# PlanNoa/video_super_resolution

Hardware: AMD Instinct MI355X
Metric: HR frames/sec, 1080p->4K x4 VSR (LR 540x960 -> 2160x3840), VSR.forward end-to-end (higher is better)
Workload: dtype f16

## Files before the change

### __graft_entry__.py

```python
import os

os.environ.setdefault("MIOPEN_FIND_MODE", "2")
os.environ.setdefault("MIOPEN_DEBUG_ENABLE_AI_IMMED_MODE_FALLBACK", "0")
os.environ.setdefault("MIOPEN_LOG_LEVEL", "2")
import subprocess
import sys

ROOT = os.path.dirname(os.path.abspath(__file__))
if ROOT not in sys.path:
    sys.path.insert(0, ROOT)


def build() -> None:
    from video_super_resolution_amd import _lib
    _lib.build(verbose=True)
    subprocess.check_call(["make", "-s", "-C", os.path.join(ROOT, "oracle"), "_build/liboracle_native.so"])
    import video_super_resolution_amd
    missing = [s for s in _lib.declared_symbols() if not hasattr(_lib.load(), s)]
    if missing:
        raise RuntimeError(f"libvsr_hip.so lacks {missing}")
    xmissing = [s for s in _lib.declared_symbols() + _lib.declared_symbols(xcheck=True) if not hasattr(_lib.load_xcheck(), s)]
    if xmissing:
        raise RuntimeError(f"libvsr_hip_xcheck.so lacks {xmissing}")
    s3missing = [s for s in _lib.declared_symbols(s3=True) if not hasattr(_lib.load_s3(), s)]
    if s3missing:
        raise RuntimeError(f"libvsr_hip_s3.so lacks {s3missing}")
    s3tmissing = [s for s in _lib.declared_symbols(s3t=True) if not hasattr(_lib.load_s3t(), s)]
    if s3tmissing:
        raise RuntimeError(f"libvsr_hip_s3t.so lacks {s3tmissing}")
    s3pmissing = [s for s in _lib.declared_symbols(s3p=True) if not hasattr(_lib.load_s3p(), s)]
    if s3pmissing:
        raise RuntimeError(f"libvsr_hip_s3p.so lacks {s3pmissing}")
    s3fmissing = [s for s in _lib.declared_symbols(s3f=True) if not hasattr(_lib.load_s3f(), s)]
    if s3fmissing:
        raise RuntimeError(f"libvsr_hip_s3f.so lacks {s3fmissing}")
    yuvmissing = [s for s in _lib.declared_symbols(yuv=True) if not hasattr(_lib.load_yuv(), s)]
    if yuvmissing:
        raise RuntimeError(f"libvsr_hip_yuv.so lacks {yuvmissing}")
    metricmissing = [s for s in _lib.declared_symbols(metric=True) if not hasattr(_lib.load_metric(), s)]
    if metricmissing:
        raise RuntimeError(f"libvsr_hip_metric.so lacks {metricmissing}")
    optmissing = [s for s in _lib.declared_symbols(opt=True) if not hasattr(_lib.load_opt(), s)]
    if optmissing:
        raise RuntimeError(f"libvsr_hip_opt.so lacks {optmissing}")
    lossmissing = [s for s in _lib.declared_symbols(loss=True) if not hasattr(_lib.load_loss(), s)]
    if lossmissing:
        raise RuntimeError(f"libvsr_hip_loss.so lacks {lossmissing}")
    resizemissing = [s for s in _lib.declared_symbols(resize=True) if not hasattr(_lib.load_resize(), s)]
    if resizemissing:
        raise RuntimeError(f"libvsr_hip_resize.so lacks {resizemissing}")
    warpmissing = [s for s in _lib.declared_symbols(warp=True) if not hasattr(_lib.load_warp(), s)]
    if warpmissing:
        raise RuntimeError(f"libvsr_hip_warp.so lacks {warpmissing}")
    scenemissing = [s for s in _lib.declared_symbols(scene=True) if not hasattr(_lib.load_scene(), s)]
    if scenemissing:
        raise RuntimeError(f"libvsr_hip_scene.so lacks {scenemissing}")
    hgimissing = [s for s in _lib.declared_symbols(hgi=True) if not hasattr(_lib.load_hgi(), s)]
    if hgimissing:
        raise RuntimeError(f"libvsr_hip_hgi.so lacks {hgimissing}")
    msssimmissing = [s for s in _lib.declared_symbols(msssim=True) if not hasattr(_lib.load_msssim(), s)]
    if msssimmissing:
        raise RuntimeError(f"libvsr_hip_msssim.so lacks {msssimmissing}")


def smoke() -> None:
    import numpy as np
    import torch
    from oracle import native, vsr_oracle
    from video_super_resolution_amd import SRProjectionModule, ops
    from video_super_resolution_amd.weights import fill_module_

    assert torch.cuda.is_available(), "smoke() needs cuda:0"
    torch.cuda.set_device(0)
    rs = np.random.RandomState(0)
    img = rs.randn(1, 3, 32, 48).astype(np.float32)
    flow = (rs.randn(1, 2, 32, 48) * 4).astype(np.float32)
    got = ops.resample2d(torch.from_numpy(img).cuda(), torch.from_numpy(flow).cuda()).cpu().numpy()
    assert np.array_equal(got, native.resample2d(img, flow)), "flow warp differs from the oracle"

    sr = fill_module_(SRProjectionModule().eval(), seed=0, prefix="model.")
    x = torch.from_numpy(rs.randint(0, 256, (8, 3, 10, 12)).astype(np.float32))
    with torch.no_grad():
        ref = vsr_oracle.sr_forward({k: v for k, v in sr.state_dict().items()}, x).numpy()
    sr = sr.cuda()
    errs = {}
    for precision, bar in (("fp32", 1e-3), ("fp16", 5e-3)):
        sr.precision = precision
        out = sr(x.cuda()).cpu().numpy()
        errs[precision] = np.abs(out - ref).max() / np.abs(ref).max()
        assert errs[precision] < bar, f"SR forward ({precision}) differs from the oracle: {errs[precision]}"
    print(f"smoke ok: warp bit-exact, SR forward rel err fp32 {errs['fp32']:.2e}, fp16/MFMA {errs['fp16']:.2e}")


if __name__ == "__main__":
    build()
    if len(sys.argv) > 1 and sys.argv[1] == "smoke":
        smoke()
```

### video_super_resolution_amd/_lib.py

```python
from __future__ import annotations

import ctypes
import os
import re
import subprocess

import torch

_PKG = os.path.dirname(os.path.abspath(__file__))
_ROOT = os.path.dirname(_PKG)
LIB_PATH = os.path.join(_PKG, "libvsr_hip.so")
XLIB_PATH = os.path.join(_PKG, "libvsr_hip_xcheck.so")
HEADER_PATH = os.path.join(_ROOT, "include", "vsr_hip.h")
XHEADER_PATH = os.path.join(_ROOT, "include", "vsr_hip_xcheck.h")
_lib = None
_xlib = None


def _side(name: str, prefix: str, abi: int, has_query: bool) -> tuple:
    return (os.path.join(_PKG, f"libvsr_hip_{name}.so"), os.path.join(_ROOT, "include", f"vsr_hip_{name}.h"), prefix, abi, has_query)


_SIDE = {"grad": _side("grad", "vsr_grad", 1, False), "s3": _side("s3", "vsr_s3", 1, True), "s3t": _side("s3t", "vsr_s3t", 1, True),
         "s3p": _side("s3p", "vsr_s3p", 1, True), "s3f": _side("s3f", "vsr_s3f", 1, True), "yuv": _side("yuv", "vsr_yuv", 1, False),
         "metric": _side("metric", "vsr_metric", 1, False), "opt": _side("opt", "vsr_opt", 1, False), "loss": _side("loss", "vsr_loss", 1, False),
         "resize": _side("resize", "vsr_resize", 1, False), "warp": _side("warp", "vsr_warp", 1, False),
         "scene": _side("scene", "vsr_scene", 1, False), "hgi": _side("hgi", "vsr_hgi", 1, False),
         "msssim": _side("msssim", "vsr_msssim", 1, False)}
(GLIB_PATH, GHEADER_PATH), (S3LIB_PATH, S3HEADER_PATH), (S3TLIB_PATH, S3THEADER_PATH), (S3PLIB_PATH, S3PHEADER_PATH), \
    (S3FLIB_PATH, S3FHEADER_PATH), (YUVLIB_PATH, YUVHEADER_PATH), (METRICLIB_PATH, METRICHEADER_PATH), (OPTLIB_PATH, OPTHEADER_PATH), \
    (LOSSLIB_PATH, LOSSHEADER_PATH), (RESIZELIB_PATH, RESIZEHEADER_PATH), (WARPLIB_PATH, WARPHEADER_PATH), (SCENELIB_PATH, SCENEHEADER_PATH), \
    (HGILIB_PATH, HGIHEADER_PATH), (MSSSIMLIB_PATH, MSSSIMHEADER_PATH) = (row[:2] for row in _SIDE.values())
_gradlib = _s3lib = _s3tlib = _s3plib = _s3flib = _yuvlib = _metriclib = _optlib = _losslib = _resizelib = _warplib = _scenelib = _hgilib = _msssimlib = None
_use_x = os.environ.get("VSR_USE_XCHECK", "0") == "1" or bool(os.environ.get("VSR_TUNING", "").strip())


class VsrHipError(RuntimeError):
    pass


def build(verbose: bool = False) -> str:
    cmd = ["make", "-j4", "-C", os.path.join(_PKG, "csrc")]
    if not verbose:
        cmd.insert(1, "-s")
    subprocess.check_call(cmd)
    return LIB_PATH


def declared_symbols(xcheck: bool = False, grad: bool = False, s3: bool = False, s3t: bool = False, s3p: bool = False, s3f: bool = False,
                     yuv: bool = False, metric: bool = False, opt: bool = False, loss: bool = False, resize: bool = False,
                     warp: bool = False, scene: bool = False, hgi: bool = False, msssim: bool = False) -> list:
    side = [name for name, on in (("grad", grad), ("s3", s3), ("s3t", s3t), ("s3p", s3p), ("s3f", s3f), ("yuv", yuv), ("metric", metric),
                                  ("opt", opt), ("loss", loss), ("resize", resize), ("warp", warp), ("scene", scene), ("hgi", hgi),
                                  ("msssim", msssim)) if on]
    with open(_SIDE[side[-1]][1] if side else XHEADER_PATH if xcheck else HEADER_PATH) as f:
        text = re.sub(r"/\*.*?\*/", "", f.read(), flags=re.S)
    return sorted(set(re.findall(r"\b(vsr_[a-z0-9_]+)\s*\(", text)))


def _dlopen(path: str) -> ctypes.CDLL:
    if not os.path.exists(path):
        raise VsrHipError(
            f"{path} is missing: build it with `python -c 'import __graft_entry__ as g; g.build()'` "
            "(there is no CPU fallback for the device path)")
    return ctypes.CDLL(path)


def _open(path: str) -> ctypes.CDLL:
    lib = _dlopen(path)
    lib.vsr_last_error.restype = ctypes.c_char_p
    lib.vsr_last_route.restype = ctypes.c_char_p
    for fn in ("vsr_sr_query", "vsr_train_corr_dw_ws_floats", "vsr_train_prelu_bwd_ws_floats"):
        getattr(lib, fn).restype = ctypes.c_size_t
    if lib.vsr_abi_version() != 3:
        raise VsrHipError(f"{os.path.basename(path)}: ABI version mismatch")
    return lib


def load_xcheck() -> ctypes.CDLL:
    global _xlib
    if _xlib is None:
        lib = _open(XLIB_PATH)
        for t in os.environ.get("VSR_TUNING", "").split(","):
            if t.strip():
                lib.vsr_conv2d_tuning(int(t))
        _xlib = lib
    return _xlib


def _load_side(name: str) -> ctypes.CDLL:
    cache = f"_{name}lib"
    if globals()[cache] is None:
        path, _, prefix, abi, has_query = _SIDE[name]
        lib = _dlopen(path)
        getattr(lib, prefix + "_last_error").restype = ctypes.c_char_p
        lib.vsr_last_error = getattr(lib, prefix + "_last_error")
        if has_query:
            getattr(lib, prefix + "_query").restype = ctypes.c_size_t
        if getattr(lib, prefix + "_abi_version")() != abi:
            raise VsrHipError(f"{os.path.basename(path)}: ABI version mismatch")
        globals()[cache] = lib
    return globals()[cache]


def load_grad() -> ctypes.CDLL:
    return _load_side("grad")


def load_s3() -> ctypes.CDLL:
    return _load_side("s3")


def load_s3t() -> ctypes.CDLL:
    return _load_side("s3t")


def load_s3p() -> ctypes.CDLL:
    return _load_side("s3p")


def load_s3f() -> ctypes.CDLL:
    return _load_side("s3f")


def load_yuv() -> ctypes.CDLL:
    return _load_side("yuv")


def load_metric() -> ctypes.CDLL:
    lib = _load_side("metric")
    lib.vsr_metric_ws_bytes.restype = ctypes.c_size_t
    return lib


class OptTensor(ctypes.Structure):
    _fields_ = [("p", ctypes.c_void_p), ("g", ctypes.c_void_p), ("m", ctypes.c_void_p), ("v", ctypes.c_void_p), ("n", ctypes.c_ulonglong)]


def load_opt() -> ctypes.CDLL:
    lib = _load_side("opt")
    lib.vsr_opt_plan_bytes.restype = lib.vsr_opt_norm_ws_bytes.restype = ctypes.c_size_t
    lib.vsr_opt_plan_bytes.argtypes = [ctypes.c_int, ctypes.POINTER(ctypes.c_ulonglong)]
    lib.vsr_opt_plan_fill.argtypes = [ctypes.c_void_p, ctypes.c_size_t, ctypes.c_int, ctypes.POINTER(OptTensor)]
    lib.vsr_opt_norm_ws_bytes.argtypes = [ctypes.c_void_p]
    lib.vsr_opt_adam_f32.argtypes = [ctypes.c_void_p] * 3 + [ctypes.c_float] * 7 + [ctypes.c_void_p]
    lib.vsr_opt_grad_norm.argtypes = [ctypes.c_void_p, ctypes.c_void_p, ctypes.c_double, ctypes.c_void_p, ctypes.c_void_p, ctypes.c_void_p]
    return lib


def load_loss() -> ctypes.CDLL:
    lib = _load_side("loss")
    lib.vsr_loss_ws_bytes.restype = ctypes.c_size_t
    lib.vsr_loss_ws_bytes.argtypes = [ctypes.c_int, ctypes.c_int]
    lib.vsr_loss_pixel_terms.argtypes = [ctypes.c_void_p] * 3 + [ctypes.c_int] * 2 + [ctypes.c_void_p] * 6
    return lib


def load_resize() -> ctypes.CDLL:
    lib = _load_side("resize")
    lib.vsr_resize_frames.argtypes = [ctypes.c_void_p] * 2 + [ctypes.c_int] * 5 + [ctypes.c_void_p, ctypes.c_void_p, ctypes.c_int] * 2 + \
        [ctypes.c_int, ctypes.c_void_p]
    return lib


def load_warp() -> ctypes.CDLL:
    lib = _load_side("warp")
    lib.vsr_warp_ws_bytes.restype = ctypes.c_size_t
    lib.vsr_warp_ws_bytes.argtypes = [ctypes.c_int] * 4
    lib.vsr_warp_error.argtypes = [ctypes.c_void_p] * 2 + [ctypes.c_int] * 7 + [ctypes.c_void_p] * 2 + [ctypes.c_int] + [ctypes.c_longlong] * 3 + \
        [ctypes.c_int] * 3 + [ctypes.c_void_p] * 5
    return lib


def load_scene() -> ctypes.CDLL:
    lib = _load_side("scene")
    lib.vsr_scene_ws_bytes.restype = ctypes.c_size_t
    lib.vsr_scene_ws_bytes.argtypes = [ctypes.c_int] * 3
    lib.vsr_scene_pair_sums.argtypes = [ctypes.c_void_p] * 2 + [ctypes.c_int] * 3 + [ctypes.c_void_p] * 4
    lib.vsr_scene_decide.argtypes = [ctypes.c_void_p, ctypes.c_int, ctypes.c_void_p, ctypes.c_double, ctypes.c_double, ctypes.c_void_p, ctypes.c_void_p]
    lib.vsr_scene_window.argtypes = [ctypes.c_void_p] * 4 + [ctypes.c_int] * 2 + [ctypes.c_void_p] * 4 + [ctypes.c_int] * 2 + [ctypes.c_void_p]
    return lib


def load_hgi() -> ctypes.CDLL:
    lib = _load_side("hgi")
    lib.vsr_hgi_workgroups.restype = ctypes.c_longlong
    lib.vsr_hgi_inception_f16.argtypes = [ctypes.c_void_p] + [ctypes.c_int] * 3 + [ctypes.c_void_p] * 2 + [ctypes.c_int] * 3 + \
        [ctypes.c_void_p, ctypes.c_void_p, ctypes.c_int] * 3 + [ctypes.c_int, ctypes.c_void_p] + [ctypes.c_int] * 4 + [ctypes.c_void_p]
    return lib


def load_msssim() -> ctypes.CDLL:
    lib = _load_side("msssim")
    lib.vsr_msssim_ws_bytes.restype = ctypes.c_size_t
    lib.vsr_msssim_ws_bytes.argtypes = [ctypes.c_int] * 5
    lib.vsr_msssim_frames.argtypes = [ctypes.c_void_p] * 2 + [ctypes.c_int] * 6 + [ctypes.c_void_p] * 5
    return lib


def load() -> ctypes.CDLL:
    global _lib
    if _use_x:
        return load_xcheck()
    if _lib is None:
        _lib = _open(LIB_PATH)
    return _lib


class xcheck:

    def __enter__(self):
        global _use_x
        self._old, _use_x = _use_x, True
        return load_xcheck()

    def __exit__(self, *exc):
        global _use_x
        _use_x = self._old
        return False


Q_UTD_BLOB_BYTES, Q_UTD_STRIP_WIDTH, Q_UTD_S2_BLOB_BYTES, Q_UTD_S2_STRIP_WIDTH, Q_TAIL_S2_BLOB_BYTES = range(5)
Q_S3_BLOB_BYTES, Q_S3_STRIP_WIDTH = range(2)
Q_S3T_BLOB_BYTES, Q_S3T_BLOB_FOLD_BYTES, Q_S3T_STRIP_WIDTH = range(3)
Q_S3P_BLOB_BYTES, Q_S3P_STRIP_WIDTH = range(2)
Q_S3F_BLOB_BYTES, Q_S3F_STRIP_WIDTH = range(2)


def check(rc: int, what: str = "", lib=None) -> None:
    if rc != 0:
        libs = [lib] if lib is not None else [l for l in (load(), _lib, _xlib) if l is not None]
        msgs = []
        for l in libs:
            m = l.vsr_last_error().decode("utf-8", "replace")
            if m and m not in msgs:
                msgs.append(m)
        raise VsrHipError(f"{what or 'vsr'} failed ({rc}): {' | '.join(msgs)}")


def dptr(t: torch.Tensor, dtype=torch.float32) -> ctypes.c_void_p:
    if not t.is_cuda:
        raise VsrHipError("device path called with a CPU tensor (no CPU fallback exists)")
    if t.dtype != dtype:
        raise VsrHipError(f"expected {dtype}, got {t.dtype}")
    if not t.is_contiguous():
        raise VsrHipError("tensor must be contiguous")
    return ctypes.c_void_p(t.data_ptr())


def optr(t, dtype=torch.float32):
    return ctypes.c_void_p(0) if t is None else dptr(t, dtype)


_raw_stream = getattr(torch._C, "_cuda_getCurrentRawStream", None)


def raw_stream(index=None) -> int:
    if _raw_stream is not None:
        return _raw_stream(torch._C._cuda_getDevice() if index is None else index)
    return torch.cuda.current_stream(index).cuda_stream


def stream() -> ctypes.c_void_p:
    return ctypes.c_void_p(raw_stream())


def _first_cuda_tensor(objs):
    for o in objs:
        if isinstance(o, torch.Tensor):
            if o.is_cuda:
                return o
        elif isinstance(o, (list, tuple)):
            t = _first_cuda_tensor(o)
            if t is not None:
                return t
    return None


def on_device(fn):
    import functools

    @functools.wraps(fn)
    def wrapped(*args, **kwargs):
        t = _first_cuda_tensor(args)
        if t is None:
            t = _first_cuda_tensor(tuple(kwargs.values()))
        if t is None or t.device.index == torch.cuda.current_device():
            return fn(*args, **kwargs)
        with torch.cuda.device(t.device):
            return fn(*args, **kwargs)
    return wrapped


def cf(v: float) -> ctypes.c_float:
    return ctypes.c_float(float(v))


class _ChainStage(ctypes.Structure):
    _fields_ = [("inp", ctypes.c_void_p * 2), ("w", ctypes.c_void_p * 2), ("ldw", ctypes.c_int * 2), ("w_prev", ctypes.c_void_p),
                ("ldw_prev", ctypes.c_int), ("bias", ctypes.c_void_p), ("cmap", ctypes.c_void_p), ("slope", ctypes.c_float),
                ("out", ctypes.c_void_p)]


class Chain1x1(ctypes.Structure):
    _fields_ = [("nstages", ctypes.c_int), ("stage", _ChainStage * 3)]


_ROUTE_BATCH = os.environ.get("VSR_ROUTE_BATCH", "1") != "0"


class route_batch:

    def __init__(self, num: int, den: int):
        self.num, self.den = int(num), int(den)
        self.on = self.den > 0 and self.num > 0 and self.num != self.den and _ROUTE_BATCH

    def __enter__(self):
        if self.on:
            check(load().vsr_conv2d_route_batch(self.num, self.den), "conv2d_route_batch")
        return self

    def __exit__(self, *exc):
        if self.on:
            load().vsr_conv2d_route_batch(0, 0)
        return False


class serial_streams:
    on = False

    def __init__(self, enable: bool = True):
        self.enable = bool(enable)

    def __enter__(self):
        self._old, serial_streams.on = serial_streams.on, serial_streams.on or self.enable
        return self

    def __exit__(self, *exc):
        serial_streams.on = self._old
        return False


class EventTimer:

    def __init__(self):
        self.enabled = False
        self.only = None
        self._pairs = {}

    def reset(self):
        self._pairs = {}

    def start(self, name: str):
        if not self.enabled or (self.only is not None and name not in self.only):
            return None
        a = torch.cuda.Event(enable_timing=True)
        b = torch.cuda.Event(enable_timing=True)
        a.record()
        self._pairs.setdefault(name, []).append((a, b))
        return b

    @staticmethod
    def stop(tok):
        if tok is not None:
            tok.record()

    def summary(self):
        return {k: (len(v), sum(a.elapsed_time(b) for a, b in v) / len(v)) for k, v in self._pairs.items()}


TIMER = EventTimer()


class RouteLog:

    def __init__(self):
        self.enabled = False
        self.calls = []

    def note(self, label: str):
        if self.enabled:
            self.calls.append((label, load().vsr_last_route().decode()))

    def note_as(self, label: str, route: str):
        if self.enabled:
            self.calls.append((label, route))

    def last(self) -> str:
        return load().vsr_last_route().decode()

    def histogram(self):
        h = {}
        for _, r in self.calls:
            h[r] = h.get(r, 0) + 1
        return h


ROUTES = RouteLog()
```

### video_super_resolution_amd/csrc/sr_f16.hip

```cpp
#include "sr_f16_common.h"

namespace {

#if VSR_X
__device__ unsigned long long* g_stamp_ptr = nullptr;

template <int MODE, bool ALLMAX, int DIAG = 0>
__global__ void __launch_bounds__(512, 2)
k_utd(const _Float16* __restrict__ in, const unsigned char* __restrict__ blob, _Float16* __restrict__ out, int h, int w,
      int rows_per_seg) {
    extern __shared__ __attribute__((aligned(16))) unsigned char smem[];
    unsigned char* const ring = smem;
    unsigned char* const part = smem + RING_BYTES;
    unsigned char* const lrr = smem + RING_BYTES + PART_BYTES;
    float* const bias_s = reinterpret_cast<float*>(smem + RING_BYTES + PART_BYTES + LR_BYTES);

    const int tid = threadIdx.x;
    const int lane = tid & 63;
    const int wv = __builtin_amdgcn_readfirstlane(tid >> 6);
    const int l15 = lane & 15, g = lane >> 4;
    const int x0 = blockIdx.x * TX;
    const int n = blockIdx.z;
    const int r0 = blockIdx.y * rows_per_seg;
    const int r1 = min(h, r0 + rows_per_seg);
    if (r0 >= r1) return;

    h8 Aup[2][4][2];
    h8 Adn[2][8];
#pragma unroll
    for (int c = 0; c < 2; ++c)
#pragma unroll
        for (int t = 0; t < 4; ++t)
#pragma unroll
            for (int mt = 0; mt < 2; ++mt)
                Aup[c][t][mt] = *reinterpret_cast<const h8*>(blob + BLOB_UP + ((((wv * 2 + c) * 4 + t) * 2 + mt) * 64 + lane) * 16);
    if (MODE == 0) {
#pragma unroll
        for (int hl = 0; hl < 2; ++hl)
#pragma unroll
            for (int kx = 0; kx < 8; ++kx)
                Adn[hl][kx] = *reinterpret_cast<const h8*>(blob + BLOB_DN + (((wv * 2 + hl) * 8 + kx) * 64 + lane) * 16);
        if (tid < 128) *reinterpret_cast<uint4*>(smem + RING_BYTES + PART_BYTES + LR_BYTES + 256 + tid * 16) =
            *reinterpret_cast<const uint4*>(blob + BLOB_DT + tid * 16);
    }
    const unsigned char* const adt_s = smem + RING_BYTES + PART_BYTES + LR_BYTES + 256 + lane * 16;
    const float* fpar = reinterpret_cast<const float*>(blob + BLOB_F32);
    if (tid < 64) bias_s[tid] = fpar[tid];
    auto bias_up = [&](int mt) __attribute__((always_inline)) { return *reinterpret_cast<const f4*>(bias_s + 16 * mt + 4 * g); };
    auto bias_dt = [&](int mt) __attribute__((always_inline)) { return *reinterpret_cast<const f4*>(bias_s + 32 + 16 * mt + 4 * g); };
    const float a_up = fpar[96], a_dt = fpar[97], a_dn = fpar[98];
    const h2 a_up2 = {(_Float16)a_up, (_Float16)a_up}, a_dt2 = {(_Float16)a_dt, (_Float16)a_dt};
    const bool up_max = ALLMAX || a_up <= 1.0f, dt_max = ALLMAX || a_dt <= 1.0f;
    const bool edge_strip = (x0 == 0) || (4 * (x0 + 32) - 2 >= 4 * w);
    int ring_lo[2], ring_hi[2], lr_b[2][2];
#pragma unroll
    for (int nt = 0; nt < 2; ++nt) {
        const int j = 16 * nt + l15;
        ring_lo[nt] = j * (4 * COL_PITCH) + ((g ^ ((j >> 1) & 3)) << 4);
        ring_hi[nt] = j * (4 * COL_PITCH) + ((g ^ (((j + 1) >> 1) & 3)) << 4);
        lr_b[0][nt] = lr_off(j + 1, g);
        lr_b[1][nt] = lr_off(j, g);
    }
    const int py = wv >> 1, pxb = (wv & 1) * 2;
    const int rr = wv & 3, mth = wv >> 2;
    const int rj = tid >> 4, rcp = tid & 15;
    const float bdn0 = fpar[64 + 2 * rcp], bdn1 = fpar[64 + 2 * rcp + 1];
    const bool red_ok = (rj < TX) && (x0 + rj < w);
    const int part_wr = rr * PART_W_PITCH + l15 * PART_PX_PITCH + (16 * mth + 4 * g) * 4;
    const int part_rd = rj * PART_PX_PITCH + rcp * 8;

    const _Float16* in_n = in + (size_t)n * h * w * NF;
    const bool lr_loader = tid < LR_COLS * 4;
    const int lr_px = tid >> 2, lr_ch = tid & 3, lr_col = x0 - 1 + lr_px;
    const bool lr_col_ok = lr_loader && lr_col >= 0 && lr_col < w;
    const int lr_st = lr_off(lr_px, lr_ch);

    auto fetch_lr = [&](int r) __attribute__((always_inline)) -> uint4 {
        uint4 v = make_uint4(0, 0, 0, 0);
        if (lr_col_ok && r >= 0 && r < h) v = *reinterpret_cast<const uint4*>(in_n + ((size_t)r * w + lr_col) * NF + lr_ch * 8);
        return v;
    };
    auto lr_slot = [&](int r) __attribute__((always_inline)) { return ((r + 1) % 3) * LR_SLOT; };

    f4 carry[2] = {f4{0.0f, 0.0f, 0.0f, 0.0f}, f4{0.0f, 0.0f, 0.0f, 0.0f}};

    auto p1_load = [&](int s_i, int s_i1, h8 (&Bf)[4][2]) __attribute__((always_inline)) {
#pragma unroll
        for (int t = 0; t < 4; ++t) {
            const int dy = t >> 1, dx = t & 1;
            const unsigned char* base = lrr + (dy ? s_i : s_i1);
#pragma unroll
            for (int nt = 0; nt < 2; ++nt) Bf[t][nt] = *reinterpret_cast<const h8*>(base + lr_b[dx][nt]);
        }
    };
    auto phase1 = [&](int i, int s_i, int s_i1, unsigned char* rbase, auto checkc, auto edgec) __attribute__((always_inline)) {
        constexpr bool CHECK = decltype(checkc)::value;
        constexpr bool EDGE = decltype(edgec)::value;
        const int r_hr = 4 * i + 2 + py;
        unsigned char* const rowbase = rbase + py * ROW_PITCH;
        const bool row_ok = !CHECK || ((r_hr >= 0) && (r_hr < 4 * h));
        if (row_ok) {
            h8 Bf[4][2];
            p1_load(s_i, s_i1, Bf);
            f4 acc2c[2][2][2];
#pragma unroll
            for (int c = 0; c < 2; ++c) {
#pragma unroll
                for (int mt = 0; mt < 2; ++mt)
#pragma unroll
                    for (int nt = 0; nt < 2; ++nt) acc2c[c][mt][nt] = bias_up(mt);
#pragma unroll
                for (int t = 0; t < 4; ++t)
#pragma unroll
                    for (int mt = 0; mt < 2; ++mt)
#pragma unroll
                        for (int nt = 0; nt < 2; ++nt) acc2c[c][mt][nt] = mfma16(Aup[c][t][mt], Bf[t][nt], acc2c[c][mt][nt]);
            }
            h8 adt_r[2];
            f4 bdt_r[2];
            if (MODE == 0) {
#pragma unroll
                for (int mt = 0; mt < 2; ++mt) {
                    adt_r[mt] = *reinterpret_cast<const h8*>(adt_s + mt * 1024);
                    bdt_r[mt] = bias_dt(mt);
                }
            }
#pragma unroll
            for (int c = 0; c < 2; ++c) {
                const int px = pxb + c;
                f4 (&acc)[2][2] = acc2c[c];
#pragma unroll
                for (int nt = 0; nt < 2; ++nt) {
                    const h8 hb = act_pack(acc[0][nt], acc[1][nt], a_up2, up_max);
                    const int c_hr = 4 * (x0 + 16 * nt + l15) + px - 2;
                    if (MODE == 0) {
                        f4 a2[2];
#pragma unroll
                        for (int mt = 0; mt < 2; ++mt) a2[mt] = mfma16(adt_r[mt], hb, bdt_r[mt]);
                        h8 ob = act_pack(a2[0], a2[1], a_dt2, dt_max);
                        if (EDGE) {
                            const bool col_ok = (c_hr >= 0) && (c_hr < 4 * w);
#pragma unroll
                            for (int e = 0; e < 8; ++e) ob[e] = col_ok ? ob[e] : (_Float16)0.0f;
                        }
                        *reinterpret_cast<h8*>(rowbase + ring_lo[nt] + px * COL_PITCH) = ob;
                    } else if ((c_hr >= 0) && (c_hr < 4 * w)) {
                        _Float16* dst = out + (((size_t)n * 4 * h + r_hr) * (size_t)(4 * w) + c_hr) * NF;
                        typedef _Float16 h4 __attribute__((ext_vector_type(4)));
                        h4 lo = {hb[0], hb[1], hb[2], hb[3]}, hi = {hb[4], hb[5], hb[6], hb[7]};
                        *reinterpret_cast<h4*>(dst + 4 * g) = lo;
                        *reinterpret_cast<h4*>(dst + 16 + 4 * g) = hi;
                    }
                }
            }
        } else if (MODE == 0) {
            h8 z;
#pragma unroll
            for (int e = 0; e < 8; ++e) z[e] = (_Float16)0.0f;
#pragma unroll
            for (int c = 0; c < 2; ++c)
#pragma unroll
                for (int nt = 0; nt < 2; ++nt) *reinterpret_cast<h8*>(rowbase + ring_lo[nt] + (pxb + c) * COL_PITCH) = z;
        }
    };

    auto phase2 = [&](const unsigned char* rbase, unsigned char* pbase) __attribute__((always_inline)) {
        const unsigned char* const rowbase = rbase + rr * ROW_PITCH;
        f4 acc[2] = {carry[0], carry[1]};
        f4 nc[2] = {f4{0.0f, 0.0f, 0.0f, 0.0f}, f4{0.0f, 0.0f, 0.0f, 0.0f}};
#pragma unroll
        for (int kk = 0; kk < 8; ++kk)
#pragma unroll
            for (int nt = 0; nt < 2; ++nt) {
                const int kx = (kk >> 1) + 4 * (kk & 1);
                const h8 b = *reinterpret_cast<const h8*>(rowbase + (kx < 4 ? ring_lo[nt] : ring_hi[nt]) + kx * COL_PITCH);
                acc[nt] = mfma16(Adn[1][kx], b, acc[nt]);
                nc[nt] = mfma16(Adn[0][kx], b, nc[nt]);
            }
        __builtin_amdgcn_sched_group_barrier(0x100, 8, 0);
#pragma unroll
        for (int k = 0; k < 4; ++k) {
            __builtin_amdgcn_sched_group_barrier(0x008, 4, 0);
            __builtin_amdgcn_sched_group_barrier(0x100, 2, 0);
        }
        __builtin_amdgcn_sched_group_barrier(0x008, 16, 0);
        carry[0] = nc[0];
        carry[1] = nc[1];
#pragma unroll
        for (int nt = 0; nt < 2; ++nt) *reinterpret_cast<f4*>(pbase + part_wr + 16 * nt * PART_PX_PITCH) = acc[nt];
    };

    auto reduce_store = [&](int i, const unsigned char* pbase) __attribute__((always_inline)) {
        f2 s = {0.0f, 0.0f};
#pragma unroll
        for (int k = 0; k < 4; ++k) {
            const f2 v = *reinterpret_cast<const f2*>(pbase + part_rd + k * PART_W_PITCH);
            s[0] += v[0];
            s[1] += v[1];
        }
        const h2 o = {(_Float16)prelu(s[0] + bdn0, a_dn), (_Float16)prelu(s[1] + bdn1, a_dn)};
        if (red_ok) *reinterpret_cast<h2*>(out + (((size_t)n * h + i) * w + x0 + rj) * NF + 2 * rcp) = o;
    };

    if (lr_loader) {
        *reinterpret_cast<uint4*>(lrr + lr_slot(r0 - 1) + lr_st) = fetch_lr(r0 - 1);
        *reinterpret_cast<uint4*>(lrr + lr_slot(r0) + lr_st) = fetch_lr(r0);
        if (MODE == 0) *reinterpret_cast<uint4*>(lrr + lr_slot(r0 + 1) + lr_st) = fetch_lr(r0 + 1);
    }
    __syncthreads();

    if (MODE == 0) {
        phase1(r0 - 1, lr_slot(r0 - 1), lr_slot(r0), ring + ((r0 - 1) & 1) * SLOT_PITCH, BoolC<true>{}, BoolC<true>{});
        __syncthreads();
        __builtin_amdgcn_s_waitcnt(0);
        int s_im1 = lr_slot(r0 - 1), s_i = lr_slot(r0), s_i1 = lr_slot(r0 + 1);
        int ring_cur = (r0 & 1) * SLOT_PITCH, part_cur = (r0 & 1) * PART_BUF;
        unsigned long long stamp[4] = {0, 0, 0, 0};
        const unsigned long long rt0 = DIAG ? __builtin_amdgcn_s_memrealtime() : 0, ct0 = DIAG ? __builtin_amdgcn_s_memtime() : 0;
        auto march = [&](auto edgec) __attribute__((always_inline)) {
            for (int i = r0; i < r1; ++i) {
                uint4 nxt = make_uint4(0, 0, 0, 0);
                if (wv < 3) nxt = fetch_lr(i + 2);
                const unsigned char* ring_prev = ring + (ring_cur ^ SLOT_PITCH);
                unsigned char* part_prev = part + (part_cur ^ PART_BUF);
                if (DIAG) {
                    const unsigned long long t0 = __builtin_amdgcn_s_memtime();
                    phase2(ring_prev, part_prev);
                    const unsigned long long t1 = __builtin_amdgcn_s_memtime();
                    phase1(i, s_i, s_i1, ring + ring_cur, BoolC<true>{}, edgec);
                    const unsigned long long t2 = __builtin_amdgcn_s_memtime();
                    if (i - 2 >= r0) reduce_store(i - 2, part + part_cur);
                    if (wv < 3 && lr_loader) *reinterpret_cast<uint4*>(lrr + s_im1 + lr_st) = nxt;
                    const unsigned long long t3 = __builtin_amdgcn_s_memtime();
                    __syncthreads();
                    const unsigned long long t4 = __builtin_amdgcn_s_memtime();
                    stamp[0] += t1 - t0; stamp[1] += t2 - t1; stamp[2] += t3 - t2; stamp[3] += t4 - t3;
                } else {
                    phase2(ring_prev, part_prev);
                    phase1(i, s_i, s_i1, ring + ring_cur, BoolC<true>{}, edgec);
                    if (i - 2 >= r0) reduce_store(i - 2, part + part_cur);
                    if (wv < 3 && lr_loader) *reinterpret_cast<uint4*>(lrr + s_im1 + lr_st) = nxt;
                    __syncthreads();
                }
                const int t = s_im1; s_im1 = s_i; s_i = s_i1; s_i1 = t;
                ring_cur ^= SLOT_PITCH;
                part_cur ^= PART_BUF;
            }
        };
        if (edge_strip) march(BoolC<true>{}); else march(BoolC<false>{});
        if (DIAG && g_stamp_ptr && (tid & 63) == 0) {
            unsigned long long* d = g_stamp_ptr + ((size_t)((blockIdx.z * gridDim.y + blockIdx.y) * gridDim.x + blockIdx.x) * 8 + wv) * 8;
            for (int k = 0; k < 4; ++k) d[k] = stamp[k];
            d[4] = __builtin_amdgcn_s_memtime() - ct0;
            d[5] = __builtin_amdgcn_s_memrealtime() - rt0;
        }
        phase2(ring + (ring_cur ^ SLOT_PITCH), part + (part_cur ^ PART_BUF));
        if (r1 - 2 >= r0) reduce_store(r1 - 2, part + part_cur);
        __syncthreads();
        reduce_store(r1 - 1, part + (part_cur ^ PART_BUF));
    } else {
        for (int i = r0 - 1; i < r1; ++i) {
            const uint4 nxt = fetch_lr(i + 2);
            const int r_hr = 4 * i + 2 + py;
            if (r_hr >= 4 * r0 && r_hr < 4 * r1) phase1(i, lr_slot(i), lr_slot(i + 1), ring, BoolC<true>{}, BoolC<true>{});
            __syncthreads();
            if (lr_loader) *reinterpret_cast<uint4*>(lrr + lr_slot(i + 2) + lr_st) = nxt;
            __syncthreads();
        }
    }
}

#endif

__global__ void __launch_bounds__(256)
k_conv1x1_h(const _Float16* __restrict__ in0, const float* __restrict__ w0, int ld0, const _Float16* __restrict__ in1,
            const float* __restrict__ w1, int ld1, const _Float16* __restrict__ in2, const float* __restrict__ w2, int ld2,
            const float* __restrict__ bias, const float* __restrict__ cmap, float slope, _Float16* __restrict__ out,
            size_t P, size_t total_px) {
    const int lane = threadIdx.x & 63;
    const int l15 = lane & 15, g = lane >> 4;
    const _Float16* ins[3] = {in0, in1, in2};
    const float* ws[3] = {w0, w1, w2};
    const int lds_[3] = {ld0, ld1, ld2};
    h8 A[3][2];
#pragma unroll
    for (int t = 0; t < 3; ++t)
#pragma unroll
        for (int mt = 0; mt < 2; ++mt) {
            h8 a;
#pragma unroll
            for (int e = 0; e < 8; ++e) a[e] = (_Float16)0.0f;
            if (ins[t]) {
                const float* wr = ws[t] + (size_t)(16 * mt + l15) * lds_[t] + 8 * g;
#pragma unroll
                for (int e = 0; e < 8; ++e) a[e] = (_Float16)wr[e];
            }
            A[t][mt] = a;
        }
    f4 bz[2];
#pragma unroll
    for (int mt = 0; mt < 2; ++mt)
#pragma unroll
        for (int r = 0; r < 4; ++r) bz[mt][r] = bias[16 * mt + 4 * g + r];
    const h2 a2 = {(_Float16)slope, (_Float16)slope};
    const bool use_max = slope <= 1.0f;
    const size_t ntiles = (total_px + 15) / 16;
    const size_t wave0 = (size_t)blockIdx.x * 4 + (threadIdx.x >> 6), nwaves = (size_t)gridDim.x * 4;
    for (size_t tile = wave0; tile < ntiles; tile += nwaves) {
        const size_t px = tile * 16 + l15;
        const size_t pc = px < total_px ? px : total_px - 1;
        f4 acc[2] = {bz[0], bz[1]};
        if (cmap) {
            const size_t pp = pc % P;
#pragma unroll
            for (int mt = 0; mt < 2; ++mt) {
                const f4 c = *reinterpret_cast<const f4*>(cmap + pp * NF + 16 * mt + 4 * g);
                acc[mt] += c;
            }
        }
#pragma unroll
        for (int t = 0; t < 3; ++t) {
            if (!ins[t]) continue;
            const h8 bfrag = *reinterpret_cast<const h8*>(ins[t] + pc * NF + 8 * g);
#pragma unroll
            for (int mt = 0; mt < 2; ++mt) acc[mt] = mfma16(A[t][mt], bfrag, acc[mt]);
        }
        if (px < total_px) {
            typedef float f2v __attribute__((ext_vector_type(2)));
            typedef _Float16 h4 __attribute__((ext_vector_type(4)));
#pragma unroll
            for (int mt = 0; mt < 2; ++mt) {
                const h2 p0 = prelu_h2(__builtin_convertvector(f2v{acc[mt][0], acc[mt][1]}, h2), a2, use_max);
                const h2 p1 = prelu_h2(__builtin_convertvector(f2v{acc[mt][2], acc[mt][3]}, h2), a2, use_max);
                *reinterpret_cast<h4*>(out + px * NF + 16 * mt + 4 * g) = h4{p0[0], p0[1], p1[0], p1[1]};
            }
        }
    }
}

struct ChainStage {
    const _Float16* in[2];
    const float* w[2];
    int ld[2];
    const float* w_prev;
    int ld_prev;
    const float* bias;
    const float* cmap;
    float slope;
    _Float16* out;
};
struct ChainP {
    int nstages;
    ChainStage st[3];
};

__global__ void __launch_bounds__(256)
k_chain1x1_h(const ChainP cp, size_t P, size_t total_px) {
    const int lane = threadIdx.x & 63;
    const int l15 = lane & 15, g = lane >> 4;
    h8 A[3][3][2];
    f4 bz[3][2];
    h2 a2[3];
    bool use_max[3];
#pragma unroll
    for (int s = 0; s < 3; ++s) {
        const ChainStage& st = cp.st[s];
        const bool on = s < cp.nstages;
#pragma unroll
        for (int t = 0; t < 3; ++t)
#pragma unroll
            for (int mt = 0; mt < 2; ++mt) {
                h8 a;
#pragma unroll
                for (int e = 0; e < 8; ++e) a[e] = (_Float16)0.0f;
                const float* wp = !on ? nullptr : (t < 2 ? (st.in[t] ? st.w[t] : nullptr) : st.w_prev);
                if (wp) {
                    const int ld = t < 2 ? st.ld[t] : st.ld_prev;
                    const float* wr = wp + (size_t)(16 * mt + l15) * ld;
#pragma unroll
                    for (int e = 0; e < 8; ++e)
                        a[e] = (_Float16)wr[t < 2 ? 8 * g + e : (e < 4 ? 4 * g + e : 16 + 4 * g + (e - 4))];
                }
                A[s][t][mt] = a;
            }
#pragma unroll
        for (int mt = 0; mt < 2; ++mt)
#pragma unroll
            for (int r = 0; r < 4; ++r) bz[s][mt][r] = on ? st.bias[16 * mt + 4 * g + r] : 0.0f;
        const float sl = on ? st.slope : 1.0f;
        a2[s] = h2{(_Float16)sl, (_Float16)sl};
        use_max[s] = sl <= 1.0f;
    }
    const size_t ntiles = (total_px + 15) / 16;
    const size_t wave0 = (size_t)blockIdx.x * 4 + (threadIdx.x >> 6), nwaves = (size_t)gridDim.x * 4;
    for (size_t tile = wave0; tile < ntiles; tile += nwaves) {
        const size_t px = tile * 16 + l15;
        const size_t pc = px < total_px ? px : total_px - 1;
        h8 prev;
#pragma unroll
        for (int e = 0; e < 8; ++e) prev[e] = (_Float16)0.0f;
#pragma unroll
        for (int s = 0; s < 3; ++s) {
            if (s >= cp.nstages) break;
            const ChainStage& st = cp.st[s];
            f4 acc[2] = {bz[s][0], bz[s][1]};
            if (st.cmap) {
                const size_t pp = pc % P;
#pragma unroll
                for (int mt = 0; mt < 2; ++mt) acc[mt] += *reinterpret_cast<const f4*>(st.cmap + pp * NF + 16 * mt + 4 * g);
            }
#pragma unroll
            for (int t = 0; t < 2; ++t) {
                if (!st.in[t]) continue;
                const h8 bfrag = *reinterpret_cast<const h8*>(st.in[t] + pc * NF + 8 * g);
#pragma unroll
                for (int mt = 0; mt < 2; ++mt) acc[mt] = mfma16(A[s][t][mt], bfrag, acc[mt]);
            }
            if (s > 0 && st.w_prev) {
#pragma unroll
                for (int mt = 0; mt < 2; ++mt) acc[mt] = mfma16(A[s][2][mt], prev, acc[mt]);
            }
            prev = act_pack(acc[0], acc[1], a2[s], use_max[s]);
            if (st.out && px < total_px) {
                typedef _Float16 h4 __attribute__((ext_vector_type(4)));
                *reinterpret_cast<h4*>(st.out + px * NF + 4 * g) = h4{prev[0], prev[1], prev[2], prev[3]};
                *reinterpret_cast<h4*>(st.out + px * NF + 16 + 4 * g) = h4{prev[4], prev[5], prev[6], prev[7]};
            }
        }
    }
}

template <int NS, int MIN, bool CMAP0>
__global__ void __launch_bounds__(256)
k_chain1x1_s(const ChainP cp, unsigned P, unsigned total_px) {
    const int lane = threadIdx.x & 63, wv = threadIdx.x >> 6;
    const int l15 = lane & 15, g = lane >> 4;
    __shared__ __attribute__((aligned(16))) h8 As[NS][3][2][64];
    __shared__ __attribute__((aligned(16))) float bs[NS][32];
    __shared__ __attribute__((aligned(16))) unsigned char ost[4 * 1024];
    for (int q = wv; q < NS * 6; q += 4) {
        const int s = q / 6, t = (q % 6) >> 1, mt = q & 1;
        const ChainStage& st = cp.st[s];
        h8 a;
#pragma unroll
        for (int e = 0; e < 8; ++e) a[e] = (_Float16)0.0f;
        const float* wp = t < 2 ? (st.in[t] ? st.w[t] : nullptr) : st.w_prev;
        if (wp) {
            const int ld = t < 2 ? st.ld[t] : st.ld_prev;
            const float* wr = wp + (size_t)(16 * mt + l15) * ld;
#pragma unroll
            for (int e = 0; e < 8; ++e)
                a[e] = (_Float16)wr[t < 2 ? 8 * g + e : (e < 4 ? 4 * g + e : 16 + 4 * g + (e - 4))];
        }
        As[s][t][mt][lane] = a;
    }
    if (threadIdx.x < NS * 32) bs[threadIdx.x >> 5][threadIdx.x & 31] = cp.st[threadIdx.x >> 5].bias[threadIdx.x & 31];
    __syncthreads();
    h2 a2[NS];
    bool use_max[NS];
#pragma unroll
    for (int s = 0; s < NS; ++s) {
        a2[s] = h2{(_Float16)cp.st[s].slope, (_Float16)cp.st[s].slope};
        use_max[s] = cp.st[s].slope <= 1.0f;
    }
    constexpr int NIN = ((MIN >> 0) & 1) + ((MIN >> 1) & 1) + ((MIN >> 2) & 1) + ((MIN >> 3) & 1) + ((MIN >> 4) & 1) + ((MIN >> 5) & 1);
    struct Ops { h8 in[NIN > 0 ? NIN : 1]; f4 cm[2]; };
    auto fetch = [&](unsigned tile, Ops& o) __attribute__((always_inline)) {
        const unsigned px = tile * 16 + l15;
        const unsigned pc = px < total_px ? px : total_px - 1;
        int k = 0;
#pragma unroll
        for (int q = 0; q < 2 * NS; ++q)
            if ((MIN >> q) & 1) o.in[k++] = *reinterpret_cast<const h8*>(cp.st[q >> 1].in[q & 1] + (size_t)pc * NF + 8 * g);
        if (CMAP0) {
            const unsigned pp = pc - (pc / P) * P;
#pragma unroll
            for (int mt = 0; mt < 2; ++mt) o.cm[mt] = *reinterpret_cast<const f4*>(cp.st[0].cmap + (size_t)pp * NF + 16 * mt + 4 * g);
        }
    };
    const unsigned ntiles = (total_px + 15) / 16;
    const unsigned wave0 = blockIdx.x * 4 + wv, nwaves = gridDim.x * 4;
    if (wave0 >= ntiles) return;
    Ops cur;
    fetch(wave0, cur);
    for (unsigned tile = wave0; tile < ntiles; tile += nwaves) {
        Ops nxt;
        fetch(tile + nwaves < ntiles ? tile + nwaves : tile, nxt);
        unsigned loff = lane * 16, boff = g * 16;
        asm volatile("" : "+v"(loff), "+v"(boff));
        const unsigned char* const ap = reinterpret_cast<const unsigned char*>(&As[0][0][0][0]) + loff;
        const unsigned char* const bp = reinterpret_cast<const unsigned char*>(&bs[0][0]) + boff;
        const unsigned px = tile * 16 + l15;
        h8 prev = cur.in[0];
        int k = 0;
#pragma unroll
        for (int s = 0; s < NS; ++s) {
            f4 acc[2];
#pragma unroll
            for (int mt = 0; mt < 2; ++mt) acc[mt] = *reinterpret_cast<const f4*>(bp + s * 128 + mt * 64);
            if (CMAP0 && s == 0) { acc[0] += cur.cm[0]; acc[1] += cur.cm[1]; }
#pragma unroll
            for (int t = 0; t < 2; ++t) {
                if (!((MIN >> (2 * s + t)) & 1)) continue;
                const h8 bfrag = cur.in[k++];
#pragma unroll
                for (int mt = 0; mt < 2; ++mt)
                    acc[mt] = mfma16(*reinterpret_cast<const h8*>(ap + ((s * 3 + t) * 2 + mt) * 1024), bfrag, acc[mt]);
            }
            if (s > 0) {
#pragma unroll
                for (int mt = 0; mt < 2; ++mt)
                    acc[mt] = mfma16(*reinterpret_cast<const h8*>(ap + ((s * 3 + 2) * 2 + mt) * 1024), prev, acc[mt]);
            }
            prev = act_pack(acc[0], acc[1], a2[s], use_max[s]);
            if (cp.st[s].out) {
                typedef _Float16 h4 __attribute__((ext_vector_type(4)));
                unsigned char* const o = ost + wv * 1024;
                const int sw = (l15 >> 1) & 3;
                *reinterpret_cast<h4*>(o + l15 * 64 + (((g >> 1) ^ sw) << 4) + ((g & 1) << 3)) = h4{prev[0], prev[1], prev[2], prev[3]};
                *reinterpret_cast<h4*>(o + l15 * 64 + (((2 + (g >> 1)) ^ sw) << 4) + ((g & 1) << 3)) = h4{prev[4], prev[5], prev[6], prev[7]};
                asm volatile("" ::: "memory");
                const int opx = lane >> 2, opc = (lane & 3) ^ ((opx >> 1) & 3);
                const h8 ov = *reinterpret_cast<const h8*>(o + lane * 16);
                asm volatile("" ::: "memory");
                const unsigned gpx = tile * 16 + opx;
                if (gpx < total_px) *reinterpret_cast<h8*>(cp.st[s].out + (size_t)gpx * NF + 8 * opc) = ov;
            }
        }
        cur = nxt;
    }
}

__global__ void __launch_bounds__(256, 4)
k_head_h(const float* __restrict__ x, const float* __restrict__ sub_scale, const float* __restrict__ sub_bias,
         const float* __restrict__ w_in, const float* __restrict__ b_in, float slope_in, int nmid,
         const float* __restrict__ w_feat, const float* __restrict__ b_feat, float slope_feat, _Float16* __restrict__ out,
         int N, int h, int w) {
    const int lane = threadIdx.x & 63;
    const int l15 = lane & 15, g = lane >> 4;
    const size_t hw = (size_t)h * w;
    __shared__ __attribute__((aligned(16))) float bias_in[128];
    if (threadIdx.x < 128) bias_in[threadIdx.x] = b_in[threadIdx.x];
    __shared__ __attribute__((aligned(16))) h8 A1s[8][64], A2s[4][2][64];
    {
        const int wv = threadIdx.x >> 6;
#pragma unroll
        for (int q = 0; q < 2; ++q) {
            const int mt = 2 * wv + q;
            h8 a;
#pragma unroll
            for (int j = 0; j < 8; ++j) {
                const int k = 8 * g + j;
                a[j] = k < 27 ? (_Float16)w_in[(16 * mt + l15) * 27 + k] : (_Float16)0.0f;
            }
            A1s[mt][lane] = a;
        }
#pragma unroll
        for (int mt2 = 0; mt2 < 2; ++mt2) {
            h8 a;
#pragma unroll
            for (int j = 0; j < 8; ++j) {
                const int mid = 32 * wv + (j < 4 ? 4 * g + j : 16 + 4 * g + (j - 4));
                a[j] = (_Float16)w_feat[(16 * mt2 + l15) * nmid + mid];
            }
            A2s[wv][mt2][lane] = a;
        }
    }
    __syncthreads();
    const h2 a1 = {(_Float16)slope_in, (_Float16)slope_in}, a2 = {(_Float16)slope_feat, (_Float16)slope_feat};
    const bool max1 = slope_in <= 1.0f, max2 = slope_feat <= 1.0f;
    constexpr int SROW = 20, SCH = 3 * SROW, SWAVE = 3 * SCH;
    __shared__ __attribute__((aligned(16))) float stg[4 * SWAVE];
    __shared__ __attribute__((aligned(16))) unsigned char ost[4 * 1024];
    const int wvi = threadIdx.x >> 6;
    float* const my = stg + wvi * SWAVE;
    int toff[8];
#pragma unroll
    for (int j = 0; j < 8; ++j) {
        const int k = 8 * g + j, kk = k < 27 ? k : 0;
        toff[j] = (kk / 9) * SCH + ((kk % 9) / 3) * SROW + (kk % 3) + l15;
    }
    int ec[3], er[3], ecol[3], eoff[3];
    float es[3], eb[3];
#pragma unroll
    for (int q = 0; q < 3; ++q) {
        const int e0 = lane + 64 * q, ee = e0 < 162 ? e0 : 0;
        ec[q] = ee / 54; er[q] = (ee % 54) / 18; ecol[q] = ee % 18;
        eoff[q] = e0 < 162 ? ec[q] * SCH + er[q] * SROW + ecol[q] : -1;
        es[q] = sub_scale[ec[q]]; eb[q] = sub_bias[ec[q]];
    }
    const unsigned tpr = (unsigned)(w + 15) >> 4;
    const unsigned ntiles = (unsigned)N * (unsigned)h * tpr;
    const unsigned wave0 = __builtin_amdgcn_readfirstlane(blockIdx.x * 4 + (threadIdx.x >> 6)), nwaves = gridDim.x * 4;
    auto fetch = [&](unsigned tile, float (&raw)[3], unsigned& okmask, unsigned& row_out) __attribute__((always_inline)) {
        const unsigned row = tile / tpr, xt = tile - row * tpr;
        const unsigned n = row / (unsigned)h;
        const int y = (int)(row - n * (unsigned)h), x0 = (int)(16 * xt);
        const float* const img = x + (size_t)n * 3 * hw;
        unsigned m = 0;
#pragma unroll
        for (int q = 0; q < 3; ++q) {
            const int yy = y - 1 + er[q], xc = x0 - 1 + ecol[q];
            const bool ok = yy >= 0 && yy < h && xc >= 0 && xc < w;
            const int yc = yy < 0 ? 0 : (yy >= h ? h - 1 : yy), xl = xc < 0 ? 0 : (xc >= w ? w - 1 : xc);
            raw[q] = img[(size_t)ec[q] * hw + (size_t)yc * w + xl];
            m |= ok ? (1u << q) : 0u;
        }
        okmask = m;
        row_out = row;
    };
    float cur[3];
    unsigned curm = 0, cur_row = 0;
    if (wave0 < ntiles) fetch(wave0, cur, curm, cur_row);
    for (unsigned tile = wave0; tile < ntiles; tile += nwaves) {
        float nxr[3];
        unsigned nxm, nx_row;
        const unsigned tnext = tile + nwaves < ntiles ? tile + nwaves : tile;
        fetch(tnext, nxr, nxm, nx_row);
        const unsigned xt = tile - cur_row * tpr;
        const int xx = (int)(16 * xt) + l15;
#pragma unroll
        for (int q = 0; q < 3; ++q) {
            const float t = cur[q] * es[q] + eb[q];
            if (eoff[q] >= 0) my[eoff[q]] = (curm >> q) & 1u ? t : 0.0f;
        }
        asm volatile("" ::: "memory");
        h8 bfrag;
#pragma unroll
        for (int j = 0; j < 8; ++j) bfrag[j] = (_Float16)my[toff[j]];
        asm volatile("" ::: "memory");
        unsigned loff = lane * 16, boff = g * 16;
        asm volatile("" : "+v"(loff), "+v"(boff));
        const unsigned char* const a1p = reinterpret_cast<const unsigned char*>(&A1s[0][0]) + loff;
        const unsigned char* const a2p = reinterpret_cast<const unsigned char*>(&A2s[0][0][0]) + loff;
        const unsigned char* const bp = reinterpret_cast<const unsigned char*>(&bias_in[0]) + boff;
        f4 acc1[8];
#pragma unroll
        for (int mt = 0; mt < 8; ++mt)
            acc1[mt] = mfma16(*reinterpret_cast<const h8*>(a1p + mt * 1024), bfrag, *reinterpret_cast<const f4*>(bp + mt * 64));
        f4 acc2[2];
#pragma unroll
        for (int mt2 = 0; mt2 < 2; ++mt2)
#pragma unroll
            for (int r = 0; r < 4; ++r) acc2[mt2][r] = b_feat[16 * mt2 + 4 * g + r];
#pragma unroll
        for (int s4 = 0; s4 < 4; ++s4) {
            const h8 mid = act_pack(acc1[2 * s4], acc1[2 * s4 + 1], a1, max1);
#pragma unroll
            for (int mt2 = 0; mt2 < 2; ++mt2) acc2[mt2] = mfma16(*reinterpret_cast<const h8*>(a2p + (2 * s4 + mt2) * 1024), mid, acc2[mt2]);
        }
        {
            typedef float f2v __attribute__((ext_vector_type(2)));
            typedef _Float16 h4 __attribute__((ext_vector_type(4)));
            unsigned char* const o = ost + wvi * 1024;
            const int sw = (l15 >> 1) & 3;
#pragma unroll
            for (int mt2 = 0; mt2 < 2; ++mt2) {
                const h2 p0 = prelu_h2(__builtin_convertvector(f2v{acc2[mt2][0], acc2[mt2][1]}, h2), a2, max2);
                const h2 p1 = prelu_h2(__builtin_convertvector(f2v{acc2[mt2][2], acc2[mt2][3]}, h2), a2, max2);
                *reinterpret_cast<h4*>(o + l15 * 64 + (((2 * mt2 + (g >> 1)) ^ sw) << 4) + ((g & 1) << 3)) = h4{p0[0], p0[1], p1[0], p1[1]};
            }
            asm volatile("" ::: "memory");
            const int opx = lane >> 2, opc = (lane & 3) ^ ((opx >> 1) & 3);
            const h8 ov = *reinterpret_cast<const h8*>(o + lane * 16);
            asm volatile("" ::: "memory");
            const int ox = (int)(16 * xt) + opx;
            if (ox < w) *reinterpret_cast<h8*>(out + ((size_t)cur_row * w + ox) * NF + 8 * opc) = ov;
        }
        (void)xx;
#pragma unroll
        for (int q = 0; q < 3; ++q) cur[q] = nxr[q];
        curm = nxm;
        cur_row = nx_row;
    }
}

#if VSR_X
template <bool ALLMAX>
__global__ void __launch_bounds__(512, 2)
k_utd2(const _Float16* __restrict__ in, const unsigned char* __restrict__ blob, _Float16* __restrict__ out, int h, int w,
       int rows_per_seg) {
    extern __shared__ __attribute__((aligned(16))) unsigned char smem[];
    unsigned char* const ring = smem;
    unsigned char* const part = smem + RING_BYTES;
    unsigned char* const lrr = smem + RING_BYTES + PART_BYTES;
    float* const bias_s = reinterpret_cast<float*>(smem + RING_BYTES + PART_BYTES + LR_BYTES);
    const unsigned char* const adt_base = smem + RING_BYTES + PART_BYTES + LR_BYTES + 256;

    const int tid = threadIdx.x;
    const int lane = tid & 63;
    const int wv = __builtin_amdgcn_readfirstlane(tid >> 6);
    const int l15 = lane & 15, g = lane >> 4;
    const int x0 = blockIdx.x * TX;
    const int n = blockIdx.z;
    const int r0 = blockIdx.y * rows_per_seg;
    const int r1 = min(h, r0 + rows_per_seg);
    if (r0 >= r1) return;

    const float* fpar = reinterpret_cast<const float*>(blob + BLOB_F32);
    if (tid < 64) bias_s[tid] = fpar[tid];
    if (tid >= 64 && tid < 192) *reinterpret_cast<uint4*>(smem + RING_BYTES + PART_BYTES + LR_BYTES + 256 + (tid - 64) * 16) =
        *reinterpret_cast<const uint4*>(blob + BLOB_DT + (tid - 64) * 16);
    const float a_up = fpar[96], a_dt = fpar[97], a_dn = fpar[98];
    int ring_lo[2], ring_hi[2];
#pragma unroll
    for (int nt = 0; nt < 2; ++nt) {
        const int j = 16 * nt + l15;
        ring_lo[nt] = j * (4 * COL_PITCH) + ((g ^ ((j >> 1) & 3)) << 4);
        ring_hi[nt] = j * (4 * COL_PITCH) + ((g ^ (((j + 1) >> 1) & 3)) << 4);
    }
    const int t_first = r0 - 1, t_last = r1 + 1;

    if (wv < 4) {
        const int py = wv;
        h8 Aup[4][4][2];
#pragma unroll
        for (int c = 0; c < 4; ++c)
#pragma unroll
            for (int t = 0; t < 4; ++t)
#pragma unroll
                for (int mt = 0; mt < 2; ++mt)
                    Aup[c][t][mt] = *reinterpret_cast<const h8*>(blob + BLOB_UP + ((((py * 4 + c) * 4 + t) * 2 + mt) * 64 + lane) * 16);
        const h2 a_up2 = {(_Float16)a_up, (_Float16)a_up}, a_dt2 = {(_Float16)a_dt, (_Float16)a_dt};
        const bool up_max = ALLMAX || a_up <= 1.0f, dt_max = ALLMAX || a_dt <= 1.0f;
        const bool edge_strip = (x0 == 0) || (4 * (x0 + 32) - 2 >= 4 * w);
        int lr_b[2][2];
#pragma unroll
        for (int nt = 0; nt < 2; ++nt) {
            lr_b[0][nt] = lr_off(16 * nt + l15 + 1, g);
            lr_b[1][nt] = lr_off(16 * nt + l15, g);
        }
        const unsigned char* const adt_s = adt_base + lane * 16;
        const _Float16* in_n = in + (size_t)n * h * w * NF;
        const bool lr_loader = tid < LR_COLS * 4;
        const int lr_px = tid >> 2, lr_ch = tid & 3, lr_col = x0 - 1 + lr_px;
        const bool lr_col_ok = lr_loader && lr_col >= 0 && lr_col < w;
        const int lr_st = lr_off(lr_px, lr_ch);
        auto fetch_lr = [&](int r) __attribute__((always_inline)) -> uint4 {
            uint4 v = make_uint4(0, 0, 0, 0);
            if (lr_col_ok && r >= 0 && r < h) v = *reinterpret_cast<const uint4*>(in_n + ((size_t)r * w + lr_col) * NF + lr_ch * 8);
            return v;
        };
        auto lr_slot = [&](int r) __attribute__((always_inline)) { return ((r + 1) % 3) * LR_SLOT; };
        if (lr_loader) {
            *reinterpret_cast<uint4*>(lrr + lr_slot(r0 - 1) + lr_st) = fetch_lr(r0 - 1);
            *reinterpret_cast<uint4*>(lrr + lr_slot(r0) + lr_st) = fetch_lr(r0);
        }
        __syncthreads();
        for (int t = t_first; t <= t_last; ++t) {
            if (t <= r1 - 1) {
                uint4 nxt = make_uint4(0, 0, 0, 0);
                if (wv < 3) nxt = fetch_lr(t + 2);
                const int r_hr = 4 * t + 2 + py;
                unsigned char* const rowbase = ring + (t & 1) * SLOT_PITCH + py * ROW_PITCH;
                if (r_hr >= 0 && r_hr < 4 * h) {
                    h8 Bf[4][2];
#pragma unroll
                    for (int tp = 0; tp < 4; ++tp) {
                        const int dy = tp >> 1, dx = tp & 1;
                        const unsigned char* base = lrr + lr_slot(t + 1 - dy);
#pragma unroll
                        for (int nt = 0; nt < 2; ++nt) Bf[tp][nt] = *reinterpret_cast<const h8*>(base + lr_b[dx][nt]);
                    }
#pragma unroll
                    for (int c = 0; c < 4; ++c) {
                        f4 acc[2][2];
#pragma unroll
                        for (int mt = 0; mt < 2; ++mt)
#pragma unroll
                            for (int nt = 0; nt < 2; ++nt) acc[mt][nt] = *reinterpret_cast<const f4*>(bias_s + 16 * mt + 4 * g);
#pragma unroll
                        for (int tp = 0; tp < 4; ++tp)
#pragma unroll
                            for (int mt = 0; mt < 2; ++mt)
#pragma unroll
                                for (int nt = 0; nt < 2; ++nt) acc[mt][nt] = mfma16(Aup[c][tp][mt], Bf[tp][nt], acc[mt][nt]);
#pragma unroll
                        for (int nt = 0; nt < 2; ++nt) {
                            const h8 hb = act_pack(acc[0][nt], acc[1][nt], a_up2, up_max);
                            f4 a2[2] = {*reinterpret_cast<const f4*>(bias_s + 32 + 4 * g), *reinterpret_cast<const f4*>(bias_s + 48 + 4 * g)};
#pragma unroll
                            for (int mt = 0; mt < 2; ++mt) a2[mt] = mfma16(*reinterpret_cast<const h8*>(adt_s + mt * 1024), hb, a2[mt]);
                            h8 ob = act_pack(a2[0], a2[1], a_dt2, dt_max);
                            if (edge_strip) {
                                const int c_hr = 4 * (x0 + 16 * nt + l15) + c - 2;
                                const bool col_ok = (c_hr >= 0) && (c_hr < 4 * w);
#pragma unroll
                                for (int e = 0; e < 8; ++e) ob[e] = col_ok ? ob[e] : (_Float16)0.0f;
                            }
                            *reinterpret_cast<h8*>(rowbase + ring_lo[nt] + c * COL_PITCH) = ob;
                        }
                    }
                } else {
                    h8 z;
#pragma unroll
                    for (int e = 0; e < 8; ++e) z[e] = (_Float16)0.0f;
#pragma unroll
                    for (int c = 0; c < 4; ++c)
#pragma unroll
                        for (int nt = 0; nt < 2; ++nt) *reinterpret_cast<h8*>(rowbase + ring_lo[nt] + c * COL_PITCH) = z;
                }
                if (wv < 3 && lr_loader) *reinterpret_cast<uint4*>(lrr + lr_slot(t + 2) + lr_st) = nxt;
            }
            __syncthreads();
        }
    } else {
        const int q = wv - 4;
        h8 Adn[2][8][2];
#pragma unroll
        for (int hl = 0; hl < 2; ++hl)
#pragma unroll
            for (int kx = 0; kx < 8; ++kx)
#pragma unroll
                for (int mt = 0; mt < 2; ++mt)
                    Adn[hl][kx][mt] = *reinterpret_cast<const h8*>(blob + BLOB_DN + ((((q * 2 + hl) * 8 + kx) * 2 + mt) * 64 + lane) * 16);
        const int ctid = tid - 256;
        const int rj = ctid >> 3, rc4 = ctid & 7;
        const f4 bdn = *reinterpret_cast<const f4*>(fpar + 64 + 4 * rc4);
        const bool red_ok = (rj < TX) && (x0 + rj < w);
        f4 carry[2][2];
#pragma unroll
        for (int mt = 0; mt < 2; ++mt)
#pragma unroll
            for (int nt = 0; nt < 2; ++nt) carry[mt][nt] = f4{0.0f, 0.0f, 0.0f, 0.0f};
        __syncthreads();
        for (int t = t_first; t <= t_last; ++t) {
            if (t >= r0 && t <= r1) {
                const unsigned char* const rowbase = ring + ((t - 1) & 1) * SLOT_PITCH + q * ROW_PITCH;
                f4 acc[2][2], nc[2][2];
#pragma unroll
                for (int mt = 0; mt < 2; ++mt)
#pragma unroll
                    for (int nt = 0; nt < 2; ++nt) {
                        acc[mt][nt] = carry[mt][nt];
                        nc[mt][nt] = f4{0.0f, 0.0f, 0.0f, 0.0f};
                    }
#pragma unroll
                for (int kx = 0; kx < 8; ++kx)
#pragma unroll
                    for (int nt = 0; nt < 2; ++nt) {
                        const h8 b = *reinterpret_cast<const h8*>(rowbase + (kx < 4 ? ring_lo[nt] : ring_hi[nt]) + kx * COL_PITCH);
#pragma unroll
                        for (int mt = 0; mt < 2; ++mt) {
                            acc[mt][nt] = mfma16(Adn[1][kx][mt], b, acc[mt][nt]);
                            nc[mt][nt] = mfma16(Adn[0][kx][mt], b, nc[mt][nt]);
                        }
                    }
#pragma unroll
                for (int mt = 0; mt < 2; ++mt)
#pragma unroll
                    for (int nt = 0; nt < 2; ++nt) {
                        carry[mt][nt] = nc[mt][nt];
                        *reinterpret_cast<f4*>(part + ((t - 1) & 1) * PART_BUF + q * PART_W_PITCH + (16 * nt + l15) * PART_PX_PITCH +
                                               (16 * mt + 4 * g) * 4) = acc[mt][nt];
                    }
            }
            if (t - 2 >= r0 && t - 2 <= r1 - 1) {
                const unsigned char* pb = part + ((t - 2) & 1) * PART_BUF + rj * PART_PX_PITCH + rc4 * 16;
                f4 s4 = bdn;
#pragma unroll
                for (int k = 0; k < 4; ++k) s4 += *reinterpret_cast<const f4*>(pb + k * PART_W_PITCH);
                typedef _Float16 h4 __attribute__((ext_vector_type(4)));
                const h4 o = {(_Float16)prelu(s4[0], a_dn), (_Float16)prelu(s4[1], a_dn), (_Float16)prelu(s4[2], a_dn),
                              (_Float16)prelu(s4[3], a_dn)};
                if (red_ok) *reinterpret_cast<h4*>(out + (((size_t)n * h + (t - 2)) * w + x0 + rj) * NF + 4 * rc4) = o;
            }
            __syncthreads();
        }
    }
}


template <bool ALLMAX, bool DEC = false>
__global__ void __launch_bounds__(512, 2)
k_tail(const _Float16* __restrict__ in, const unsigned char* __restrict__ blob, const unsigned char* __restrict__ acv,
       const float* __restrict__ tpar, const float* __restrict__ x, float* __restrict__ prefc, int h, int w, int rows_per_seg) {
    extern __shared__ __attribute__((aligned(16))) unsigned char smem[];
    constexpr int RING3 = 3 * SLOT_PITCH;
    unsigned char* const ring = smem;
    unsigned char* const lrr = smem + RING3;
    float* const bias_s = reinterpret_cast<float*>(smem + RING3 + LR_BYTES);

    const int tid = threadIdx.x;
    const int lane = tid & 63;
    const int wv = __builtin_amdgcn_readfirstlane(tid >> 6);
    const int l15 = lane & 15, g = lane >> 4;
    const int x0 = blockIdx.x * TX;
    const int n = blockIdx.z;
    const int r0 = blockIdx.y * rows_per_seg;
    const int r1 = min(h, r0 + rows_per_seg);
    if (r0 >= r1) return;
    const int H = 4 * h, W = 4 * w;

    h8 Aup[2][4][2];
#pragma unroll
    for (int c = 0; c < 2; ++c)
#pragma unroll
        for (int t = 0; t < 4; ++t)
#pragma unroll
            for (int mt = 0; mt < 2; ++mt)
                Aup[c][t][mt] = *reinterpret_cast<const h8*>(blob + BLOB_UP + ((((wv * 2 + c) * 4 + t) * 2 + mt) * 64 + lane) * 16);
    h8 Acv[9];
#pragma unroll
    for (int t = 0; t < 9; ++t) Acv[t] = *reinterpret_cast<const h8*>(acv + (t * 64 + lane) * 16);
    const float* fpar = reinterpret_cast<const float*>(blob + BLOB_F32);
    if (tid < 32) bias_s[tid] = fpar[tid];
    auto bias_up = [&](int mt) __attribute__((always_inline)) { return *reinterpret_cast<const f4*>(bias_s + 16 * mt + 4 * g); };
    const float a_up = fpar[96];
    const h2 a_up2 = {(_Float16)a_up, (_Float16)a_up};
    const bool up_max = ALLMAX || a_up <= 1.0f;
    const int ch = g < 3 ? g : 0;
    const float b_out = tpar[ch], sub_s = tpar[3 + ch], sub_b = tpar[6 + ch], add_s = tpar[9 + ch], add_b = tpar[12 + ch];

    int ring_lo[2], lr_b[2][2];
#pragma unroll
    for (int nt = 0; nt < 2; ++nt) {
        const int j = 16 * nt + l15;
        ring_lo[nt] = j * (4 * COL_PITCH) + ((g ^ ((j >> 1) & 3)) << 4);
        lr_b[0][nt] = lr_off(j + 1, g);
        lr_b[1][nt] = lr_off(j, g);
    }
    const int py = wv >> 1, pxb = (wv & 1) * 2;
    const _Float16* in_n = in + (size_t)n * h * w * NF;
    const bool lr_loader = tid < LR_COLS * 4;
    const int lr_px = tid >> 2, lr_ch = tid & 3, lr_col = x0 - 1 + lr_px;
    const bool lr_col_ok = lr_loader && lr_col >= 0 && lr_col < w;
    const int lr_st = lr_off(lr_px, lr_ch);
    const __amdgpu_buffer_rsrc_t in_rsrc = __builtin_amdgcn_make_buffer_rsrc(const_cast<_Float16*>(in), 0, (int)((size_t)gridDim.z * h * w * NF * 2), 0x00020000);
    typedef unsigned int u4b __attribute__((ext_vector_type(4)));
    auto fetch_lr = [&](int r) __attribute__((always_inline)) -> u4b {
        const unsigned off = (lr_col_ok && r >= 0 && r < h) ? (unsigned)(((((size_t)n * h + r) * w + lr_col) * NF + lr_ch * 8) * 2) : 0xFFFFFFFFu;
        return __builtin_amdgcn_raw_buffer_load_b128(in_rsrc, off, 0, 0);
    };
    auto lr_slot = [&](int r) __attribute__((always_inline)) { return ((r + 1) % 3) * LR_SLOT; };
    auto ring_slot = [&](int gi) __attribute__((always_inline)) { return ring + ((gi + 3) % 3) * SLOT_PITCH; };

    auto phase1 = [&](int i) __attribute__((always_inline)) {
        const int r_hr = 4 * i + 2 + py;
        unsigned char* const rowbase = ring_slot(i) + py * ROW_PITCH;
        if (r_hr >= 0 && r_hr < H) {
            h8 Bf[4][2];
#pragma unroll
            for (int t = 0; t < 4; ++t) {
                const int dy = t >> 1, dx = t & 1;
                const unsigned char* base = lrr + lr_slot(i + 1 - dy);
#pragma unroll
                for (int nt = 0; nt < 2; ++nt) Bf[t][nt] = *reinterpret_cast<const h8*>(base + lr_b[dx][nt]);
            }
#pragma unroll
            for (int c = 0; c < 2; ++c) {
                const int px = pxb + c;
                f4 acc[2][2];
#pragma unroll
                for (int mt = 0; mt < 2; ++mt)
#pragma unroll
                    for (int nt = 0; nt < 2; ++nt) acc[mt][nt] = bias_up(mt);
#pragma unroll
                for (int t = 0; t < 4; ++t)
#pragma unroll
                    for (int mt = 0; mt < 2; ++mt)
#pragma unroll
                        for (int nt = 0; nt < 2; ++nt) acc[mt][nt] = mfma16(Aup[c][t][mt], Bf[t][nt], acc[mt][nt]);
#pragma unroll
                for (int nt = 0; nt < 2; ++nt) {
                    h8 hb = act_pack(acc[0][nt], acc[1][nt], a_up2, up_max);
                    const int c_hr = 4 * (x0 + 16 * nt + l15) + px - 2;
                    const bool col_ok = (c_hr >= 0) && (c_hr < W);
#pragma unroll
                    for (int e = 0; e < 8; ++e) hb[e] = col_ok ? hb[e] : (_Float16)0.0f;
                    *reinterpret_cast<h8*>(rowbase + ring_lo[nt] + px * COL_PITCH) = hb;
                }
            }
        } else {
            h8 z;
#pragma unroll
            for (int e = 0; e < 8; ++e) z[e] = (_Float16)0.0f;
#pragma unroll
            for (int c = 0; c < 2; ++c)
#pragma unroll
// ... 45 lines not shown
        }
    };

    if (lr_loader) {
        *reinterpret_cast<u4b*>(lrr + lr_slot(r0 - 1) + lr_st) = fetch_lr(r0 - 1);
        *reinterpret_cast<u4b*>(lrr + lr_slot(r0) + lr_st) = fetch_lr(r0);
        *reinterpret_cast<u4b*>(lrr + lr_slot(r0 + 1) + lr_st) = fetch_lr(r0 + 1);
    }
    __syncthreads();
    phase1(r0 - 1);
    __syncthreads();
    __builtin_amdgcn_s_waitcnt(0);
    for (int i = r0; i <= r1 + 1; ++i) {
        const bool produce = i <= r1 - 1;
        const u4b nxt = fetch_lr(i + 2);
        if (produce) phase1(i);
        if (i >= r0 + 1) phase3(i);
        if (produce && wv < 3 && lr_loader) *reinterpret_cast<u4b*>(lrr + lr_slot(i + 2) + lr_st) = nxt;
        __syncthreads();
    }
}

#endif

#if VSR_X
template <int NPL, int HID>
__global__ void __launch_bounds__(256)
k_fc_planes(const float* __restrict__ prefc, const float* __restrict__ w1, const float* __restrict__ b1,
            const float* __restrict__ w2, const float* __restrict__ b2, float* __restrict__ out, size_t P, int nhwc) {
    const int c = blockIdx.y;
    const size_t p = (size_t)blockIdx.x * 256 + threadIdx.x;
    if (p >= P) return;
    float v[NPL];
#pragma unroll
    for (int i = 0; i < NPL; ++i) v[i] = prefc[((size_t)i * 3 + c) * P + p];
    float o = b2[0];
#pragma unroll
    for (int j = 0; j < HID; ++j) {
        float hs = b1[j];
#pragma unroll
        for (int i = 0; i < NPL; ++i) hs += w1[j * NPL + i] * v[i];
        o += w2[j] * fmaxf(hs, 0.0f);
    }
    o = fmaxf(o, 0.0f);
    if (nhwc) out[p * 3 + c] = o; else out[(size_t)c * P + p] = o;
}

#pragma clang fp contract(off)
#endif

template <int NPL, int HID>
__global__ void __launch_bounds__(256)
k_fc_planes_skip(const float* __restrict__ raw, const float* __restrict__ x, const float* __restrict__ tpar,
                 const float* __restrict__ w1, const float* __restrict__ b1, const float* __restrict__ w2,
                 const float* __restrict__ b2, float* __restrict__ out, int h, int w, int dec) {
    const int c = blockIdx.y;
    const int Wo = dec ? w : 4 * w, Ho = dec ? h : 4 * h;
    const size_t P = (size_t)Ho * Wo;
    const size_t p = (size_t)blockIdx.x * 256 + threadIdx.x;
    if (p >= P) return;
    const int yo = (int)(p / Wo), xo = (int)(p - (size_t)yo * Wo);
    int y0, y1, x0i, x1i;
    float ly, lx;
    bil4(dec ? 4 * yo : yo, h, y0, y1, ly);
    bil4(dec ? 4 * xo : xo, w, x0i, x1i, lx);
    const float sub_s = tpar[3 + c], sub_b = tpar[6 + c], add_s = tpar[9 + c], add_b = tpar[12 + c];
    float v[NPL];
#pragma unroll
    for (int i = 0; i < NPL; ++i) {
        const float* xp = x + ((size_t)i * 3 + c) * (size_t)h * w;
        const float v00 = __builtin_fmaf(xp[(size_t)y0 * w + x0i], sub_s, sub_b), v01 = __builtin_fmaf(xp[(size_t)y0 * w + x1i], sub_s, sub_b);
        const float v10 = __builtin_fmaf(xp[(size_t)y1 * w + x0i], sub_s, sub_b), v11 = __builtin_fmaf(xp[(size_t)y1 * w + x1i], sub_s, sub_b);
        v[i] = __builtin_fmaf(lerp4(v00, v01, v10, v11, lx, ly) + raw[((size_t)i * 3 + c) * P + p], add_s, add_b);
    }
    float o = b2[0];
#pragma unroll
    for (int j = 0; j < HID; ++j) {
        float hs = b1[j];
#pragma unroll
        for (int i = 0; i < NPL; ++i) hs = __builtin_fmaf(w1[j * NPL + i], v[i], hs);
        o = __builtin_fmaf(w2[j], fmaxf(hs, 0.0f), o);
    }
    out[(size_t)c * P + p] = fmaxf(o, 0.0f);
}

template <int NPL, int HID>
__global__ void __launch_bounds__(256)
k_fc_planes_skip4(const float* __restrict__ raw, const float* __restrict__ x, const float* __restrict__ tpar,
                  const float* __restrict__ w1, const float* __restrict__ b1, const float* __restrict__ w2,
                  const float* __restrict__ b2, float* __restrict__ out, int h, int w) {
    typedef float f2 __attribute__((ext_vector_type(2)));
    const int c = blockIdx.y;
    const int Ho = 4 * h;
    const size_t P = (size_t)Ho * 4 * w;
    const size_t t = (size_t)blockIdx.x * 256 + threadIdx.x;
    if (t >= (size_t)Ho * w) return;
    const int yo = (int)(t / w), q = (int)(t - (size_t)yo * w);
    int y0, y1;
    float ly;
    bil4(yo, h, y0, y1, ly);
    int xa[4], xb[4];
    float lx[4];
#pragma unroll
    for (int j = 0; j < 4; ++j) bil4(4 * q + j, w, xa[j], xb[j], lx[j]);
    const int cm = q > 0 ? q - 1 : 0, cp = q < w - 1 ? q + 1 : q;
    const float sub_s = tpar[3 + c], sub_b = tpar[6 + c], add_s = tpar[9 + c], add_b = tpar[12 + c];
    const size_t p = (size_t)yo * 4 * w + 4 * q;
    float v[NPL][4];
#pragma unroll
    for (int i = 0; i < NPL; ++i) {
        const float* xp = x + ((size_t)i * 3 + c) * (size_t)h * w;
        const float* r0 = xp + (size_t)y0 * w;
        const float* r1 = xp + (size_t)y1 * w;
        const float a0 = __builtin_fmaf(r0[cm], sub_s, sub_b), a1 = __builtin_fmaf(r0[q], sub_s, sub_b), a2 = __builtin_fmaf(r0[cp], sub_s, sub_b);
        const float c0 = __builtin_fmaf(r1[cm], sub_s, sub_b), c1 = __builtin_fmaf(r1[q], sub_s, sub_b), c2 = __builtin_fmaf(r1[cp], sub_s, sub_b);
        const f4 rw = *reinterpret_cast<const f4*>(raw + ((size_t)i * 3 + c) * P + p);
#pragma unroll
        for (int j = 0; j < 4; ++j) {
            const float v00 = xa[j] == q ? a1 : (xa[j] == cm ? a0 : a2), v01 = xb[j] == q ? a1 : (xb[j] == cm ? a0 : a2);
            const float v10 = xa[j] == q ? c1 : (xa[j] == cm ? c0 : c2), v11 = xb[j] == q ? c1 : (xb[j] == cm ? c0 : c2);
            v[i][j] = __builtin_fmaf(lerp4(v00, v01, v10, v11, lx[j], ly) + rw[j], add_s, add_b);
        }
    }
    f2 o[2] = {f2{b2[0], b2[0]}, f2{b2[0], b2[0]}};
#pragma unroll
    for (int j = 0; j < HID; ++j) {
        f2 hs[2] = {f2{b1[j], b1[j]}, f2{b1[j], b1[j]}};
#pragma unroll
        for (int i = 0; i < NPL; ++i) {
            const float wv = w1[j * NPL + i];
            hs[0] = __builtin_elementwise_fma(f2{wv, wv}, f2{v[i][0], v[i][1]}, hs[0]);
            hs[1] = __builtin_elementwise_fma(f2{wv, wv}, f2{v[i][2], v[i][3]}, hs[1]);
        }
        const float w2j = w2[j];
        o[0] = __builtin_elementwise_fma(f2{w2j, w2j}, __builtin_elementwise_max(hs[0], f2{0.0f, 0.0f}), o[0]);
        o[1] = __builtin_elementwise_fma(f2{w2j, w2j}, __builtin_elementwise_max(hs[1], f2{0.0f, 0.0f}), o[1]);
    }
    *reinterpret_cast<f4*>(out + (size_t)c * P + p) = f4{fmaxf(o[0][0], 0.0f), fmaxf(o[0][1], 0.0f), fmaxf(o[1][0], 0.0f), fmaxf(o[1][1], 0.0f)};
}
#pragma clang fp contract(fast)

}

[[maybe_unused]] VSR_TUNABLE g_utd_variant = 0;

namespace vsr {
int launch_utd3(const void* in, const void* blob, void* out, int N, int h, int w, int rows_per_seg, int slopes_le_one,
                int diag, hipStream_t stream, void* out2 = nullptr);
int utd3_set_stamps(void* buf);
int tail3_set_stamps(void* buf, int totals_only);
size_t utd_s2_blob_bytes();
int utd_s2_strip_width();
size_t tail_s2_blob_bytes();
int launch_tail3(const void* hid_nhwc, const void* blob, const void* conv3_frags, const float* tail_params, float* prefc, int N,
                 int h, int w, int rows_per_seg, int slopes_le_one, int dec, hipStream_t stream, const void* in2 = nullptr,
                 const float* cmap = nullptr);
}

VSR_TUNABLE g_fc_one_pixel = 0;
VSR_TUNABLE g_chain_generic = 0;

extern "C" {

#if VSR_X
int vsr_sr_chain_variant(int generic) {
    const int old = g_chain_generic | (g_fc_one_pixel << 1);
    g_chain_generic = generic & 1;
    g_fc_one_pixel = (generic >> 1) & 1;
    return old;
}


int vsr_sr_utd_variant(int v) {
    VSR_REQUIRE(v >= 0 && v <= 4, "sr_utd_variant: 0 one wave per SIMD, 1 two waves per SIMD, 2 / 3 their stamped diagnostic builds, 4 build 0 with loop totals only");
    g_utd_variant = v;
    return VSR_OK;
}

int vsr_sr_tail_stamp_buffer(void* buf, int totals_only) { return vsr::tail3_set_stamps(buf, totals_only); }

int vsr_sr_utd_stamp_buffer(void* buf) {
    vsr::utd3_set_stamps(buf);
    return (int)hipMemcpyToSymbol(HIP_SYMBOL(g_stamp_ptr), &buf, sizeof(buf));
}

#endif

size_t vsr_sr_query(int what) {
    switch (what) {
        case VSR_Q_UTD_BLOB_BYTES: return BLOB_BYTES;
        case VSR_Q_UTD_STRIP_WIDTH: return TX;
        case VSR_Q_UTD_S2_BLOB_BYTES: return vsr::utd_s2_blob_bytes();
        case VSR_Q_UTD_S2_STRIP_WIDTH: return (size_t)vsr::utd_s2_strip_width();
        case VSR_Q_TAIL_S2_BLOB_BYTES: return vsr::tail_s2_blob_bytes();
        default: return 0;
    }
}

int vsr_sr_utd_f16(const void* in, const void* blob, void* out, int N, int h, int w, int rows_per_seg, int deconv_only,
                   int slopes_le_one, vsr_stream_t stream) {
    VSR_REQUIRE(in && blob && out, "sr_utd: null pointer");
    VSR_REQUIRE(N > 0 && h > 0 && w > 0 && rows_per_seg != 0 && rows_per_seg >= -65535 && N <= 65535, "sr_utd: bad shape");
    VSR_REQUIRE((reinterpret_cast<uintptr_t>(in) & 15) == 0 && (reinterpret_cast<uintptr_t>(blob) & 15) == 0 &&
                    (reinterpret_cast<uintptr_t>(out) & 15) == 0, "sr_utd: pointers must be 16-byte aligned");
#if !VSR_X
    if (deconv_only) return vsr::fail(VSR_E_UNSUPPORTED, "sr_utd: the deconv-only mode lives in the cross-check library (libvsr_hip_xcheck.so)");
    return vsr::launch_utd3(in, blob, out, N, h, w, rows_per_seg, slopes_le_one, 0, vsr::S(stream));
#else
    const bool one_wave_build = !deconv_only && (g_utd_variant == 0 || g_utd_variant == 2 || g_utd_variant == 4);
    if (rows_per_seg < 0 && !one_wave_build) rows_per_seg = h;
    const unsigned strips = vsr::cdiv(w, TX), segs = rows_per_seg > 0 ? vsr::cdiv(h, rows_per_seg) : 1;
    VSR_REQUIRE(segs <= 65535, "sr_utd: too many row segments");
    typedef void (*kern_t)(const _Float16*, const unsigned char*, _Float16*, int, int, int);
    static const kern_t kerns[4] = {k_utd<0, false>, k_utd<0, true>, k_utd<1, false>, k_utd<1, true>};
    static unsigned long long attr_devs = 0;
    if (!vsr::raise_lds_limit(attr_devs, kerns, 4, UTD_LDS)) return vsr::fail(VSR_E_LAUNCH, "sr_utd: cannot reserve %d bytes of LDS", UTD_LDS);
    if (!deconv_only && (g_utd_variant == 0 || g_utd_variant == 2 || g_utd_variant == 4))
        return vsr::launch_utd3(in, blob, out, N, h, w, rows_per_seg, slopes_le_one, g_utd_variant / 2, vsr::S(stream));
    kern_t k = kerns[(deconv_only ? 2 : 0) + (slopes_le_one ? 1 : 0)];
    if (!deconv_only && g_utd_variant == 3) {
        k = k_utd<0, true, 1>;
        (void)hipFuncSetAttribute(reinterpret_cast<const void*>(k), hipFuncAttributeMaxDynamicSharedMemorySize, UTD_LDS);
    }
    hipLaunchKernelGGL(k, dim3(strips, segs, N), dim3(512), UTD_LDS, vsr::S(stream), (const _Float16*)in,
                       (const unsigned char*)blob, (_Float16*)out, h, w, rows_per_seg);
    return vsr::launched("sr_utd");
#endif
}

int vsr_sr_utd_post_f16(const void* in, const void* blob, void* out, void* out_post, int N, int h, int w, int rows_per_seg, int slopes_le_one,
                        vsr_stream_t stream) {
    VSR_REQUIRE(in && blob && out && out_post, "sr_utd_post: null pointer");
    VSR_REQUIRE(N > 0 && h > 0 && w > 0 && rows_per_seg != 0 && rows_per_seg >= -65535 && N <= 65535, "sr_utd_post: bad shape");
    VSR_REQUIRE((reinterpret_cast<uintptr_t>(in) & 15) == 0 && (reinterpret_cast<uintptr_t>(blob) & 15) == 0 &&
                    (reinterpret_cast<uintptr_t>(out) & 15) == 0 && (reinterpret_cast<uintptr_t>(out_post) & 15) == 0,
                "sr_utd_post: pointers must be 16-byte aligned");
    VSR_REQUIRE(out_post != out && out_post != in, "sr_utd_post: out_post must be a tensor of its own");
    return vsr::launch_utd3(in, blob, out, N, h, w, rows_per_seg, slopes_le_one, 0, vsr::S(stream), out_post);
}

int vsr_sr_conv1x1_f16(const void* in0, const float* w0, int ldw0, const void* in1, const float* w1, int ldw1,
                       const void* in2, const float* w2, int ldw2, const float* bias, const float* cmap_nhwc, float slope,
                       void* out, int N, int P, vsr_stream_t stream) {
    VSR_REQUIRE(in0 && w0 && bias && out, "sr_conv1x1_f16: null pointer");
    VSR_REQUIRE((in1 == nullptr) == (w1 == nullptr) && (in2 == nullptr) == (w2 == nullptr), "sr_conv1x1_f16: input/weight mismatch");
    VSR_REQUIRE(N > 0 && P > 0 && N <= 65535, "sr_conv1x1_f16: bad shape");
    const size_t total = (size_t)N * P;
    const size_t tiles = (total + 15) / 16;
    const unsigned grid = (unsigned)(tiles / 4 + 1 < 2048 ? tiles / 4 + 1 : 2048);
    hipLaunchKernelGGL(k_conv1x1_h, dim3(grid), dim3(256), 0, vsr::S(stream), (const _Float16*)in0, w0, ldw0,
                       (const _Float16*)in1, w1, ldw1, (const _Float16*)in2, w2, ldw2, bias, cmap_nhwc, slope,
                       (_Float16*)out, (size_t)P, total);
    return vsr::launched("sr_conv1x1_f16");
}

int vsr_sr_chain1x1_f16(const vsr_chain1x1_t* chain, int N, int P, vsr_stream_t stream) {
    VSR_REQUIRE(chain && chain->nstages >= 1 && chain->nstages <= 3, "sr_chain1x1_f16: 1..3 stages");
    VSR_REQUIRE(N > 0 && P > 0 && N <= 65535, "sr_chain1x1_f16: bad shape");
    ChainP cp;
    cp.nstages = chain->nstages;
    for (int s = 0; s < 3; ++s) {
        ChainStage& d = cp.st[s];
        d = ChainStage{};
        if (s >= chain->nstages) continue;
        const auto& c = chain->stage[s];
        VSR_REQUIRE(c.bias, "sr_chain1x1_f16: stage %d has no bias", s);
        VSR_REQUIRE(c.in[0] || (s > 0 && c.w_prev), "sr_chain1x1_f16: stage %d has no input", s);
        VSR_REQUIRE(s > 0 || !c.w_prev, "sr_chain1x1_f16: the first stage has no previous stage");
        for (int t = 0; t < 2; ++t) {
            VSR_REQUIRE((c.in[t] == nullptr) == (c.w[t] == nullptr), "sr_chain1x1_f16: stage %d input/weight mismatch", s);
            d.in[t] = (const _Float16*)c.in[t]; d.w[t] = c.w[t]; d.ld[t] = c.ldw[t];
        }
        d.w_prev = c.w_prev; d.ld_prev = c.ldw_prev; d.bias = c.bias; d.cmap = c.cmap_nhwc; d.slope = c.slope;
        d.out = (_Float16*)c.out;
    }
    VSR_REQUIRE(cp.st[chain->nstages - 1].out, "sr_chain1x1_f16: the last stage must have an output");
    const size_t total = (size_t)N * P;
    const size_t tiles = (total + 15) / 16;
    const unsigned grid = (unsigned)(tiles / 4 + 1 < 2048 ? tiles / 4 + 1 : 2048);
    int min_mask = 0, cmap_late = 0, cmap0 = cp.st[0].cmap != nullptr;
    for (int s = 0; s < chain->nstages; ++s) {
        for (int t = 0; t < 2; ++t) min_mask |= cp.st[s].in[t] ? 1 << (2 * s + t) : 0;
        if (s > 0 && cp.st[s].cmap) cmap_late = 1;
    }
    const int key = g_chain_generic != 0 || cmap_late || total >= (1ull << 26) ? -1 : chain->nstages * 1000 + min_mask * 10 + cmap0;
#define VSR_CHAIN_CASE(NS_, MIN_, CM_)                                                                                   \
    case NS_ * 1000 + MIN_ * 10 + CM_:                                                                                   \
        hipLaunchKernelGGL((k_chain1x1_s<NS_, MIN_, (CM_ != 0)>), dim3(grid), dim3(256), 0, vsr::S(stream), cp, (unsigned)P, \
                           (unsigned)total);                                                                             \
        break;
    switch (key) {
        VSR_CHAIN_CASE(1, 1, 0) VSR_CHAIN_CASE(1, 3, 0) VSR_CHAIN_CASE(1, 1, 1) VSR_CHAIN_CASE(1, 3, 1)
        VSR_CHAIN_CASE(2, 3, 0) VSR_CHAIN_CASE(2, 1, 0) VSR_CHAIN_CASE(3, 7, 1) VSR_CHAIN_CASE(3, 5, 1) VSR_CHAIN_CASE(3, 7, 0)
        default: hipLaunchKernelGGL(k_chain1x1_h, dim3(grid), dim3(256), 0, vsr::S(stream), cp, (size_t)P, total);
    }
#undef VSR_CHAIN_CASE
    return vsr::launched("sr_chain1x1_f16");
}

int vsr_sr_head_f16(const float* x, const float* sub_scale3, const float* sub_bias3, const float* w_in, const float* b_in,
                    float slope_in, int nmid, const float* w_feat, const float* b_feat, float slope_feat, void* out_nhwc,
                    int N, int h, int w, vsr_stream_t stream) {
    VSR_REQUIRE(x && sub_scale3 && sub_bias3 && w_in && b_in && w_feat && b_feat && out_nhwc, "sr_head_f16: null pointer");
    VSR_REQUIRE(N > 0 && h > 0 && w > 0, "sr_head_f16: bad shape");
    if (nmid != 128) return vsr::fail(VSR_E_UNSUPPORTED, "sr_head_f16: %d mid channels (the reference has 4 x 32)", nmid);
    VSR_REQUIRE((long long)N * h * ((w + 15) / 16) < (1ll << 31), "sr_head_f16: too many pixels");
    const size_t tiles = (size_t)N * h * ((w + 15) / 16);
    const unsigned grid = (unsigned)(tiles / 4 + 1 < 2048 ? tiles / 4 + 1 : 2048);
    hipLaunchKernelGGL(k_head_h, dim3(grid), dim3(256), 0, vsr::S(stream), x, sub_scale3, sub_bias3, w_in, b_in, slope_in,
                       nmid, w_feat, b_feat, slope_feat, (_Float16*)out_nhwc, N, h, w);
    return vsr::launched("sr_head_f16");
}

#if VSR_X
int vsr_sr_utd2_f16(const void* in, const void* blob_v2, void* out, int N, int h, int w, int rows_per_seg, int slopes_le_one,
                    vsr_stream_t stream) {
    VSR_REQUIRE(in && blob_v2 && out, "sr_utd2: null pointer");
    VSR_REQUIRE(N > 0 && h > 0 && w > 0 && rows_per_seg > 0 && N <= 65535, "sr_utd2: bad shape");
    VSR_REQUIRE((reinterpret_cast<uintptr_t>(in) & 15) == 0 && (reinterpret_cast<uintptr_t>(blob_v2) & 15) == 0 &&
                    (reinterpret_cast<uintptr_t>(out) & 15) == 0, "sr_utd2: pointers must be 16-byte aligned");
    const unsigned strips = vsr::cdiv(w, TX), segs = vsr::cdiv(h, rows_per_seg);
    VSR_REQUIRE(segs <= 65535, "sr_utd2: too many row segments");
    typedef void (*kern_t)(const _Float16*, const unsigned char*, _Float16*, int, int, int);
    static const kern_t kerns[2] = {k_utd2<false>, k_utd2<true>};
    static unsigned long long attr_devs = 0;
    if (!vsr::raise_lds_limit(attr_devs, kerns, 2, UTD_LDS)) return vsr::fail(VSR_E_LAUNCH, "sr_utd2: cannot reserve %d bytes of LDS", UTD_LDS);
    if (slopes_le_one)
        hipLaunchKernelGGL(k_utd2<true>, dim3(strips, segs, N), dim3(512), UTD_LDS, vsr::S(stream), (const _Float16*)in,
                           (const unsigned char*)blob_v2, (_Float16*)out, h, w, rows_per_seg);
    else
        hipLaunchKernelGGL(k_utd2<false>, dim3(strips, segs, N), dim3(512), UTD_LDS, vsr::S(stream), (const _Float16*)in,
                           (const unsigned char*)blob_v2, (_Float16*)out, h, w, rows_per_seg);
    return vsr::launched("sr_utd2");
}

static int tail_launch(const void* hid_nhwc, const void* blob, const void* conv_out_frags, const float* tail_params,
                       const float* x, float* prefc, int N, int h, int w, int rows_per_seg, int slopes_le_one, bool dec,
                       vsr_stream_t stream) {
    VSR_REQUIRE(hid_nhwc && blob && conv_out_frags && tail_params && x && prefc, "sr_tail_f16: null pointer");
    VSR_REQUIRE(N > 0 && h > 0 && w > 0 && rows_per_seg > 0 && N <= 65535, "sr_tail_f16: bad shape");
    constexpr int LDS = 3 * SLOT_PITCH + LR_BYTES + 256;
    static_assert(LDS <= 160 * 1024, "LDS budget");
    const unsigned strips = vsr::cdiv(w, TX), segs = vsr::cdiv(h, rows_per_seg);
    VSR_REQUIRE(segs <= 65535, "sr_tail_f16: too many row segments");
    typedef void (*kern_t)(const _Float16*, const unsigned char*, const unsigned char*, const float*, const float*, float*, int, int, int);
    static const kern_t kerns[4] = {k_tail<false, false>, k_tail<true, false>, k_tail<false, true>, k_tail<true, true>};
    static unsigned long long attr_devs = 0;
    if (!vsr::raise_lds_limit(attr_devs, kerns, 4, LDS)) return vsr::fail(VSR_E_LAUNCH, "sr_tail_f16: cannot reserve %d bytes of LDS", LDS);
    hipLaunchKernelGGL(kerns[(dec ? 2 : 0) + (slopes_le_one ? 1 : 0)], dim3(strips, segs, N), dim3(512), LDS, vsr::S(stream),
                       (const _Float16*)hid_nhwc, (const unsigned char*)blob, (const unsigned char*)conv_out_frags, tail_params, x,
                       prefc, h, w, rows_per_seg);
    return vsr::launched("sr_tail_f16");
}

int vsr_sr_tail_f16(const void* hid_nhwc, const void* blob, const void* conv_out_frags, const float* tail_params,
                    const float* x, float* prefc, int N, int h, int w, int rows_per_seg, int slopes_le_one,
                    vsr_stream_t stream) {
    return tail_launch(hid_nhwc, blob, conv_out_frags, tail_params, x, prefc, N, h, w, rows_per_seg, slopes_le_one, false, stream);
}

int vsr_sr_tail_dec_f16(const void* hid_nhwc, const void* blob, const void* conv_out_frags, const float* tail_params,
                        const float* x, float* prefc_dec, int N, int h, int w, int rows_per_seg, int slopes_le_one,
                        vsr_stream_t stream) {
    return tail_launch(hid_nhwc, blob, conv_out_frags, tail_params, x, prefc_dec, N, h, w, rows_per_seg, slopes_le_one, true, stream);
}

#endif

int vsr_sr_tail3_f16(const void* hid_nhwc, const void* blob, const void* conv3_frags, const float* tail_params, float* raw,
                     int N, int h, int w, int rows_per_seg, int slopes_le_one, int decimate, vsr_stream_t stream) {
    VSR_REQUIRE(hid_nhwc && blob && conv3_frags && tail_params && raw, "sr_tail3_f16: null pointer");
    VSR_REQUIRE(N > 0 && h > 0 && w > 0 && rows_per_seg > 0 && N <= 65535, "sr_tail3_f16: bad shape");
    VSR_REQUIRE(vsr::cdiv(h, rows_per_seg) <= 65535, "sr_tail3_f16: too many row segments");
    return vsr::launch_tail3(hid_nhwc, blob, conv3_frags, tail_params, raw, N, h, w, rows_per_seg, slopes_le_one, decimate,
                             vsr::S(stream));
}

int vsr_sr_tail3_fold_f16(const void* lr_a, const void* lr_b, const float* cmap_nhwc, const void* blob_fold, const void* conv3_frags,
                          const float* tail_params, float* raw, int N, int h, int w, int rows_per_seg, int slopes_le_one, int decimate,
                          vsr_stream_t stream) {
    VSR_REQUIRE(lr_a && lr_b && cmap_nhwc && blob_fold && conv3_frags && tail_params && raw, "sr_tail3_fold_f16: null pointer");
    VSR_REQUIRE(N > 0 && h > 0 && w > 0 && rows_per_seg > 0 && N <= 65535, "sr_tail3_fold_f16: bad shape");
    VSR_REQUIRE(vsr::cdiv(h, rows_per_seg) <= 65535, "sr_tail3_fold_f16: too many row segments");
    return vsr::launch_tail3(lr_a, blob_fold, conv3_frags, tail_params, raw, N, h, w, rows_per_seg, slopes_le_one, decimate,
                             vsr::S(stream), lr_b, cmap_nhwc);
}

int vsr_sr_fc_planes_skip_f32(const float* raw, const float* x, const float* tail_params, const float* w1, const float* b1,
                              const float* w2, const float* b2, int nplanes, int hidden, float* out, int h, int w, int decimate,
                              vsr_stream_t stream) {
    VSR_REQUIRE(raw && x && tail_params && w1 && b1 && w2 && b2 && out, "sr_fc_planes_skip: null pointer");
    VSR_REQUIRE(h > 0 && w > 0, "sr_fc_planes_skip: bad shape");
    if (nplanes != 8 || hidden != 32)
        return vsr::fail(VSR_E_UNSUPPORTED, "sr_fc_planes_skip: %d planes / %d hidden units (the reference fuses 8 through 32)", nplanes, hidden);
    const size_t P = decimate ? (size_t)h * w : (size_t)16 * h * w;
    if (decimate != 0 || g_fc_one_pixel != 0)
        hipLaunchKernelGGL((k_fc_planes_skip<8, 32>), dim3(vsr::cdiv(P, 256), 3), dim3(256), 0, vsr::S(stream), raw, x, tail_params, w1, b1,
                           w2, b2, out, h, w, decimate);
    else
        hipLaunchKernelGGL((k_fc_planes_skip4<8, 32>), dim3(vsr::cdiv(P / 4, 256), 3), dim3(256), 0, vsr::S(stream), raw, x, tail_params,
                           w1, b1, w2, b2, out, h, w);
    return vsr::launched("sr_fc_planes_skip");
}

#if VSR_X
int vsr_sr_fc_planes_f32(const float* prefc, const float* w1, const float* b1, const float* w2, const float* b2,
                         int nplanes, int hidden, float* out, int P, int out_nhwc, vsr_stream_t stream) {
    VSR_REQUIRE(prefc && w1 && b1 && w2 && b2 && out, "sr_fc_planes: null pointer");
    VSR_REQUIRE(P > 0, "sr_fc_planes: bad shape");
    if (nplanes != 8 || hidden != 32)
        return vsr::fail(VSR_E_UNSUPPORTED, "sr_fc_planes: %d planes / %d hidden units (the reference fuses 8 through 32)", nplanes, hidden);
    hipLaunchKernelGGL((k_fc_planes<8, 32>), dim3(vsr::cdiv(P, 256), 3), dim3(256), 0, vsr::S(stream), prefc, w1, b1, w2, b2, out,
                       (size_t)P, out_nhwc);
    return vsr::launched("sr_fc_planes");
}
#endif

}
```

### video_super_resolution_amd/graph.py

```python
from __future__ import annotations

import os

import torch

from . import _lib
from .vsr import VSR

_RUNTIME_GRAPH_STREAMS = 4


def _hw_queue_limit() -> int:
    try:
        return int(os.environ.get("GPU_MAX_HW_QUEUES") or _RUNTIME_GRAPH_STREAMS)
    except ValueError:
        return _RUNTIME_GRAPH_STREAMS


class GraphedVSR:
    def __init__(self, model: VSR, clone_output: bool = True):
        self.model = model
        self.clone_output = clone_output
        self._graphs = {}

    def reset(self):
        self._graphs = {}

    def _key(self, data, est):
        m = self.model
        weights = (m.model._weights_key(), m._flow_exec.key(), m._depth_exec.key(), m._vos_exec.key())
        return (tuple(data.shape), data.dtype, data.device.index, None if est is None else (tuple(est.shape), est.dtype),
                m.precision, m.upscale_factor, m.share_planes, m.share_tail, m.overlap_shared, m.early_planes, m.depth_est_late, tuple(m.early_scales),
                m.model.fuse_uptran, m.model.fold_chain, tuple(m.model.fold_chain_modes), m.model.fold_tail, m.model.utd_build, m.model.tail_build, weights)

    def _capture(self, data, est):
        m = self.model
        sd = data.detach().clone()
        se = None if est is None else est.detach().clone()
        single = _hw_queue_limit() < _RUNTIME_GRAPH_STREAMS
        s = torch.cuda.Stream(device=data.device)
        s.wait_stream(torch.cuda.current_stream(data.device))
        with _lib.serial_streams(single):
            with torch.cuda.stream(s), torch.no_grad():
                want, _ = m(sd, None, None, se, train=False)
            torch.cuda.current_stream(data.device).wait_stream(s)
            torch.cuda.synchronize(data.device)
            g = torch.cuda.CUDAGraph()
            with torch.cuda.graph(g, stream=s if single else None), torch.no_grad():
                so, _ = m(sd, None, None, se, train=False)
        if single:
            g.replay()
            if not torch.equal(so, want):
                raise RuntimeError("GraphedVSR: the replayed graph does not reproduce the eager call's frame.  With fewer than four hardware "
                                   "queues (GPU_MAX_HW_QUEUES) the HIP runtime must run with DEBUG_CLR_GRAPH_PACKET_CAPTURE=0, set before its "
                                   "first call (importing this package first does it): graph.py")
        return g, sd, se, so

    def __call__(self, data, target, high_frames, estimated_image, train=False):
        m = self.model
        if train or target is not None or torch.is_grad_enabled() and m.training:
            raise ValueError("GraphedVSR replays inference calls only (train=False, target=None, under no_grad or in eval mode): "
                             "call the module itself for a training step")
        if m.temporal_cache:
            raise ValueError("VSR.temporal_cache keys on the identity of the frame tensors: not usable with the static buffers of a graph")
        if not data.is_cuda:
            raise RuntimeError("VSR runs on the GPU through hand-written HIP kernels; there is no CPU fallback")
        with torch.cuda.device(data.device):
            key = self._key(data, estimated_image)
            ent = self._graphs.get(key)
            if ent is None:
                if len(self._graphs) >= 8:
                    self._graphs.pop(next(iter(self._graphs)))
                ent = self._graphs[key] = self._capture(data, estimated_image)
            g, sd, se, so = ent
            sd.copy_(data)
            if se is not None:
                se.copy_(estimated_image)
            g.replay()
            out = so.clone() if self.clone_output else so
            if high_frames is not None:
                high_frames[1] = out.detach()
        return out, None
```

### video_super_resolution_amd/sr.py

```python
from __future__ import annotations

import ctypes
import os
from typing import Dict, List, Optional, Tuple

import torch
import torch.nn as nn

from . import _lib as L
from .sr_pack import (_append_post_s3, pack_conv_out_frags, pack_conv_out_frags3, pack_dt_frags, pack_tail_s2_blob, pack_tail_s3_blob,
                      pack_utd_blob, pack_utd_s2_blob, pack_utd_s3_blob, pack_utd_s3_pre_blob)

_NF = 32


def sr_geometry(upscale_factor: int):
    try:
        return {2: (6, 2, 2), 3: (7, 3, 2), 4: (8, 4, 2)}[int(upscale_factor)]
    except KeyError:
        raise NotImplementedError(f"upscale_factor {upscale_factor}: 4 (the reference's geometry), 2 or 3") from None


class MeanShift(nn.Conv2d):

    def __init__(self, rgb_mean, rgb_std, sign=-1):
        super().__init__(3, 3, kernel_size=1)
        std = torch.tensor(rgb_std, dtype=torch.float32)
        self.weight.data = torch.eye(3).view(3, 3, 1, 1) / std.view(3, 1, 1, 1)
        self.bias.data = sign * 255.0 * torch.tensor(rgb_mean, dtype=torch.float32) / std
        for p in self.parameters():
            p.requires_grad = False


def _conv_act(cin, cout, k, stride=1, padding=0, act=True) -> nn.Sequential:
    layers: List[nn.Module] = [nn.Conv2d(cin, cout, k, stride=stride, padding=padding)]
    if act:
        layers.append(nn.PReLU(num_parameters=1, init=0.2))
    return nn.Sequential(*layers)


def _deconv_act(cin, cout, k, stride, padding) -> nn.Sequential:
    return nn.Sequential(nn.ConvTranspose2d(cin, cout, k, stride, padding), nn.PReLU(num_parameters=1, init=0.2))


class FeedbackBlock(nn.Module):

    def __init__(self, num_features, num_groups, act_type="prelu", norm_type=None, upscale_factor=4):
        super().__init__()
        nf = num_features
        k, st, pd = sr_geometry(upscale_factor)
        self.num_groups = num_groups
        self.num_features = nf
        self.compress_in = _conv_act(2 * nf, nf, 1)
        self.upBlocks = nn.ModuleList()
        self.downBlocks = nn.ModuleList()
        self.uptranBlocks = nn.ModuleList()
        self.downtranBlocks = nn.ModuleList()
        for idx in range(num_groups):
            self.upBlocks.append(_deconv_act(nf, nf, k, st, pd))
            self.downBlocks.append(_conv_act(nf, nf, k, stride=st, padding=pd))
            if idx > 0:
                self.uptranBlocks.append(_conv_act(nf * (idx + 1), nf, 1))
                self.downtranBlocks.append(_conv_act(nf * (idx + 1), nf, 1))
        self.compress_out = _conv_act(num_groups * nf, nf, 1)

    def forward(self, x):
        raise RuntimeError("FeedbackBlock is a parameter container; call SRProjectionModule.forward")


class SRProjectionModule(nn.Module):
    def __init__(self, in_channels=3, out_channels=3, num_features=32, upscale_factor=4, num_steps=3, num_groups=6,
                 act_type="prelu", norm_type=None):
        super().__init__()
        if (in_channels, out_channels, num_features) != (3, 3, _NF):
            raise NotImplementedError("the gfx950 kernels implement the reference's widths: 3->3 channels, 32 features")
        k, st, pd = sr_geometry(upscale_factor)
        if not 3 <= num_groups <= 9:
            raise NotImplementedError("3 <= num_groups <= 9 (compress_out takes at most three live inputs per launch)")
        if act_type != "prelu" or norm_type is not None:
            raise NotImplementedError("only the reference configuration (PReLU, no norm) is implemented")
        self.num_steps = num_steps
        self.num_features = num_features
        self.upscale_factor = upscale_factor
        rgb_mean, rgb_std = (0.4488, 0.4371, 0.4040), (1.0, 1.0, 1.0)
        self.sub_mean = MeanShift(rgb_mean, rgb_std)
        self.conv_in = _conv_act(in_channels, 4 * num_features, 3, padding=1)
        self.feat_in = _conv_act(4 * num_features, num_features, 1)
        self.block = FeedbackBlock(num_features, num_groups, act_type, norm_type, upscale_factor)
        self.out = _deconv_act(num_features, num_features, k, st, pd)
        self.conv_out = _conv_act(num_features, out_channels, 3, padding=1, act=False)
        self.add_mean = MeanShift(rgb_mean, rgb_std, 1)
        self.fc = nn.Sequential(nn.Linear(8, 32), nn.ReLU(), nn.Linear(32, 1), nn.ReLU())
        self.precision = "fp16"
        self.tail_build = 3
        self.precompute_cus = int(os.environ.get("VSR_PRECOMPUTE_CUS", "128"))
        self.utd_flat_split = True
        self._pack: Optional[dict] = None
        self._pack_key = None
        self._const: Dict[Tuple[int, int], torch.Tensor] = {}
        self._const_nhwc: Dict[Tuple[int, int], torch.Tensor] = {}

    def _weights_key(self):
        mods = self.__dict__.get("_key_mods")
        if mods is None:
            mods = self.__dict__["_key_mods"] = [m for m in self.modules() if m._parameters or m._buffers]
        return tuple((t.data_ptr(), t._version) for m in mods for d in (m._parameters, m._buffers) for t in d.values() if t is not None)

    @staticmethod
    def _diag(ms: MeanShift):
        w = ms.weight.detach().reshape(3, 3)
        if torch.count_nonzero(w - torch.diag(torch.diagonal(w))):
            raise NotImplementedError("MeanShift weight must be diagonal (it is frozen to identity/std in the reference)")
        return torch.diagonal(w).contiguous().float(), ms.bias.detach().contiguous().float()

    def _packed(self) -> dict:
        key = self._weights_key()
        if self._pack is not None and key == self._pack_key:
            return self._pack
        b = self.block
        f = lambda t: t.detach().float().contiguous()
        P = {}
        P["sub_s"], P["sub_b"] = self._diag(self.sub_mean)
        P["add_s"], P["add_b"] = self._diag(self.add_mean)
        P["w_in"], P["b_in"], P["a_in"] = f(self.conv_in[0].weight), f(self.conv_in[0].bias), float(self.conv_in[1].weight.detach())
        P["w_feat"] = f(self.feat_in[0].weight.reshape(_NF, -1))
        P["b_feat"], P["a_feat"] = f(self.feat_in[0].bias), float(self.feat_in[1].weight.detach())
        wci = f(b.compress_in[0].weight.reshape(_NF, 2 * _NF))
        P["ci_w"], P["ci_b"], P["ci_a"] = wci, f(b.compress_in[0].bias), float(b.compress_in[1].weight.detach())
        P["up_w"] = [f(m[0].weight.permute(2, 3, 0, 1)) for m in b.upBlocks]
        P["up_b"] = [f(m[0].bias) for m in b.upBlocks]
        P["up_a"] = [float(m[1].weight.detach()) for m in b.upBlocks]
        P["dn_w"] = [f(m[0].weight.permute(2, 3, 1, 0)) for m in b.downBlocks]
        P["dn_b"] = [f(m[0].bias) for m in b.downBlocks]
        P["dn_a"] = [float(m[1].weight.detach()) for m in b.downBlocks]
        P["ut_w"] = [f(m[0].weight.reshape(_NF, -1)) for m in b.uptranBlocks]
        P["ut_b"] = [f(m[0].bias) for m in b.uptranBlocks]
        P["ut_a"] = [float(m[1].weight.detach()) for m in b.uptranBlocks]
        P["dt_w"] = [f(m[0].weight.reshape(_NF, -1)) for m in b.downtranBlocks]
        P["dt_b"] = [f(m[0].bias) for m in b.downtranBlocks]
        P["dt_a"] = [float(m[1].weight.detach()) for m in b.downtranBlocks]
        P["co_w"] = f(b.compress_out[0].weight.reshape(_NF, -1))
        P["co_b"], P["co_a"] = f(b.compress_out[0].bias), float(b.compress_out[1].weight.detach())
        P["out_w"] = f(self.out[0].weight.permute(2, 3, 0, 1))
        P["out_b"], P["out_a"] = f(self.out[0].bias), float(self.out[1].weight.detach())
        P["cv_w"], P["cv_b"] = f(self.conv_out[0].weight), f(self.conv_out[0].bias)
        P["fc_w1"], P["fc_b1"] = f(self.fc[0].weight), f(self.fc[0].bias)
        P["fc_w2"], P["fc_b2"] = f(self.fc[2].weight.reshape(-1)), f(self.fc[2].bias)
        P["zero_b"] = torch.zeros(_NF, dtype=torch.float32, device=wci.device)
        G = b.num_groups
        P["slopes_le_one"] = all(a <= 1.0 for a in P["up_a"] + P["dn_a"] + P["dt_a"] + [P["out_a"]])
        P["tail_par"] = torch.cat((P["cv_b"], P["sub_s"], P["sub_b"], P["add_s"], P["add_b"])).contiguous()
        post = {j: (P["ut_w"][j + 3], _NF * (j + 4), P["ut_b"][j + 3], P["ut_a"][j + 3]) for j in range(0, G - 5, 3)}
        fold_co = (P["co_w"], (_NF * 2, _NF * 5), P["co_b"], P["co_a"]) if G == 6 else None
        if self.upscale_factor != 4:
            def stage(j):
                args = (b.upBlocks[j + 1], P["dt_w"][j + 1], _NF * (j + 2), P["dt_b"][j + 1], P["dt_a"][j + 1], b.downBlocks[j + 2])
                if self.upscale_factor == 2 and self.fused_s2:
                    return _FusedStageS2(*args, slopes_le_one=P["slopes_le_one"], rows_fn=self._rows_per_segment, wide=self.utd_s2_build == 2, post=post.get(j))
                if self.upscale_factor == 3 and self.fused_s3:
                    return _FusedStageS3(*args, slopes_le_one=P["slopes_le_one"], rows_fn=self._rows_per_segment)
                return _UnfusedStage(*args, self.upscale_factor)
            P["stage"] = {j: stage(j) for j in range(0, G - 2, 3)}
            if self.upscale_factor == 3 and self.fused_s3:
                P["stage_post"] = {j: _FusedStageS3Post(P["stage"][j], post[j], rows_fn=self._rows_per_segment) for j in post}
                if G == 6:
                    P["stage_pre"] = {0: _FusedStageS3Pre(P["stage_post"][0], fold_co, (P["ci_w"], P["ci_b"], P["ci_a"]),
                                                          (P["ut_w"][0], _NF, P["ut_b"][0], P["ut_a"][0]), rows_fn=self._rows_per_segment)}
            P["out_deconv"] = _PhaseDeconv(self.out[0].weight, self.out[0].bias, P["out_a"], self.upscale_factor)
            if self.upscale_factor == 2 and self.fused_s2:
                P["tail_s2"] = pack_tail_s2_blob(self.out[0].weight, self.out[0].bias, P["out_a"], self.conv_out[0].weight,
                                                 self.conv_out[0].bias, fold_co=fold_co)
                P["tail_s2_fold"] = fold_co is not None
            if self.upscale_factor == 3 and self.fused_tail_s3:
                P["tail_s3"] = pack_tail_s3_blob(self.out[0].weight, self.out[0].bias, P["out_a"], self.conv_out[0].weight,
                                                 self.conv_out[0].bias, fold_co=fold_co)
                P["tail_s3_fold"] = fold_co is not None
            self._pack, self._pack_key = P, key
            self._const.clear()
            self._const_nhwc.clear()
            return P
        P["utd"], P["utd2"], P["utd_post"], P["utd4"] = {}, {}, {}, {}
        for j in range(0, G - 2, 3):
            args = (b.upBlocks[j + 1][0].weight, b.upBlocks[j + 1][0].bias, P["up_a"][j + 1], P["dt_w"][j + 1], _NF * (j + 2),
                    P["dt_b"][j + 1], P["dt_a"][j + 1], b.downBlocks[j + 2][0].weight, b.downBlocks[j + 2][0].bias, P["dn_a"][j + 2])
            P["utd"][j] = pack_utd_blob(*args)
            P["utd2"][j] = pack_utd_blob(*args, layout=2)
            P["utd4"][j] = pack_utd_blob(*args, layout=4, post=post.get(j))
            if j in post:
                P["utd_post"][j] = pack_utd_blob(*args, post=post[j])
        P["post_slopes_le_one"] = P["slopes_le_one"] and all(a <= 1.0 for a in P["ut_a"])
        P["utd_out"] = pack_utd_blob(self.out[0].weight, self.out[0].bias, P["out_a"], None, 0, None, 1.0, None, None, 1.0)
        if fold_co is not None:
            P["utd_out_fold"] = pack_utd_blob(self.out[0].weight, self.out[0].bias, P["out_a"], None, 0, None, 1.0, None, None, 1.0, fold_co=fold_co)
        P["cv_frags"] = pack_conv_out_frags(self.conv_out[0].weight)
        P["cv_frags3"] = pack_conv_out_frags3(self.conv_out[0].weight)
        self._pack, self._pack_key = P, key
        self._const.clear()
        self._const_nhwc.clear()
        return P

    @staticmethod
    def _c1(ins, bias, slope, N, P, cmap=None):
        lib = L.load()
        out = torch.empty((N, _NF, P), dtype=torch.float32, device=bias.device)
        args = []
        keep = []
        for k in range(3):
            if k < len(ins):
                t, w, col = ins[k]
                ws = w[:, col:col + _NF]
                keep.append(ws)
                args += [L.dptr(t), ctypes_ptr(ws), w.shape[1]]
            else:
                args += [L.optr(None), L.optr(None), 0]
        L.check(lib.vsr_sr_conv1x1_f32(*args, L.dptr(bias), L.optr(cmap), L.cf(slope), L.dptr(out), N, P, L.stream()),
                "sr_conv1x1")
        return out

    def _up(self, x, w, b, a, N, h, w_, dt=None):
        S = self.upscale_factor
        out = torch.empty((N, _NF, S * h, S * w_), dtype=torch.float32, device=x.device)
        tok = L.TIMER.start((("sr_deconv8s4_f32" if S == 4 else "sr_deconv_f32") if dt is None else "sr_deconv_dt_f32") + ("" if N == 8 else f"_p{N}"))
        fr, fb, fa = dt if dt is not None else (None, None, 0.0)
        L.check(L.load().vsr_sr_deconv_f32(L.dptr(x), L.dptr(w), L.dptr(b), L.cf(a), L.dptr(out), N, h, w_, S, L.optr(fr), L.optr(fb), L.cf(fa),
                                           L.stream()), "sr_deconv")
        L.TIMER.stop(tok)
        return out

    def _down(self, x, w, b, a, N, h, w_):
        S = self.upscale_factor
        out = torch.empty((N, _NF, h, w_), dtype=torch.float32, device=x.device)
        tok = L.TIMER.start(("sr_conv8s4_f32" if S == 4 else "sr_conv_f32") + ("" if N == 8 else f"_p{N}"))
        L.check(L.load().vsr_sr_conv_f32(L.dptr(x), L.dptr(w), L.dptr(b), L.cf(a), L.dptr(out), N, h, w_, S, L.stream()),
                "sr_conv")
        L.TIMER.stop(tok)
        return out

    def _hr_from(self, P, i, lr_prev, N, h, w, dt_for=None):
        a = self._c1([(lr_prev.view(N, _NF, h * w), P["ut_w"][i - 1], _NF * i)], P["ut_b"][i - 1], P["ut_a"][i - 1], N, h * w)
        dt = None
        if dt_for is not None:
            fr = P.setdefault("dt_frags", {})
            if dt_for not in fr:
                fr[dt_for] = pack_dt_frags(P["dt_w"][dt_for - 1], _NF * dt_for)
            dt = (fr[dt_for], P["dt_b"][dt_for - 1], P["dt_a"][dt_for - 1])
        return self._up(a.view(N, _NF, h, w), P["up_w"][i], P["up_b"][i], P["up_a"][i], N, h, w, dt=dt)

    def _lr_from(self, P, i, hr_prev, N, h, w, dt_done=False):
        S = self.upscale_factor
        b = hr_prev if dt_done else self._c1([(hr_prev.view(N, _NF, S * S * h * w), P["dt_w"][i - 1], _NF * i)], P["dt_b"][i - 1],
                                             P["dt_a"][i - 1], N, S * S * h * w)
        return self._down(b.view(N, _NF, S * h, S * w), P["dn_w"][i], P["dn_b"][i], P["dn_a"][i], N, h, w)

    def _const_map(self, P, h, w, dev) -> torch.Tensor:
        if (h, w) in self._const:
            return self._const[(h, w)]
        G = self.block.num_groups
        lr: Dict[int, torch.Tensor] = {}
        hr: Dict[int, torch.Tensor] = {}
        z = torch.zeros((1, _NF, h, w), dtype=torch.float32, device=dev)
        Z = torch.zeros((1, _NF, self.upscale_factor * h, self.upscale_factor * w), dtype=torch.float32, device=dev)
        hr[0] = self._up(z, P["up_w"][0], P["up_b"][0], P["up_a"][0], 1, h, w)
        lr[1] = self._down(Z, P["dn_w"][0], P["dn_b"][0], P["dn_a"][0], 1, h, w)
        del z, Z
        for i in range(1, G):
            if (i - 1) % 3 != 0 and i < G - 1:
                hr[i] = self._hr_from(P, i, lr[i - 1], 1, h, w)
            if (i + 1) % 3 != 0:
                lr[i + 1] = self._lr_from(P, i, hr[i - 1], 1, h, w)
            hr.pop(i - 2, None)
        cmap = None
        for j in sorted(lr):
            cmap = self._c1([(lr[j].view(1, _NF, h * w), P["co_w"], _NF * (j - 1))], P["zero_b"], 1.0, 1, h * w,
                            cmap=cmap).view(_NF, h * w)
        if cmap is None:
            cmap = torch.zeros((_NF, h * w), dtype=torch.float32, device=dev)
        self._const[(h, w)] = cmap
        return cmap

    def forward(self, x: torch.Tensor, taps: Optional[dict] = None, decimate: bool = False, shared: Optional[dict] = None) -> torch.Tensor:
        if torch.is_grad_enabled() and self.training and any(p.requires_grad for p in self.parameters()):
            if not getattr(self, "_warned_autograd", False):
                import warnings
                warnings.warn("SRProjectionModule: training mode with autograd enabled -> this call runs the differentiable "
                              "float32 train-step kernels (csrc/sr_train.hip; the train step of main.py:205-210), not the inference "
                              "kernels; call .eval() or wrap the call in torch.no_grad() for inference", stacklevel=2)
                self._warned_autograd = True
            from .sr_train import forward_train
            out = forward_train(self, x)
            S = self.upscale_factor
            return out[..., ::S, ::S] if decimate else out
        return self._forward_kernels(x, taps, decimate, shared)

    @L.on_device
    @torch.no_grad()
    def precompute_shared(self, x_first: torch.Tensor, shared: dict, live: dict) -> None:
        if self.precision == "fp32":
            n, _, h, w = x_first.shape
            if n != int(shared.get("n", 0)) or n <= 0:
                raise ValueError(f"precompute_shared: {n} planes given, shared['n'] = {shared.get('n')}")
            x = x_first.detach().float().contiguous()
            P = self._packed()
            S = self.upscale_factor
            kept = torch.empty((n, 3, S * h, S * w), dtype=torch.float32, device=x.device)
            self._f32_planes(x, P, self._const_map(P, h, w, x.device), None, kept)
            shared["prefc_f32"], shared["key_f32"] = kept, (self._pack_key, h, w, self.fc[0].in_features, S, n)
            return
        if self.precision != "fp16" or self.block.num_groups != 6:
            raise ValueError("precompute_shared: the fp16 configuration with six groups only (or the float32 configuration)")
        n, _, h, w = x_first.shape
        total = live[3].shape[0]
        if n != int(shared.get("n", 0)) or not 0 < n < total:
            raise ValueError(f"precompute_shared: {n} planes given, shared['n'] = {shared.get('n')}, {total} in all")
        x = x_first.detach().float().contiguous()
        P = self._packed()
        cmap = self._const_map(P, h, w, x.device)
        self._utd_cus, self._utd_side = int(getattr(self, "precompute_cus", 256)), True
        try:
            self._forward_f16(x, P, cmap, None, False, shared, precompute=live)
        finally:
            self._utd_cus, self._utd_side = 256, False

    @L.on_device
    @torch.no_grad()
    def precompute_rows(self, x_rows: torch.Tensor, live: dict, row0: int) -> None:
        if self.precision != "fp16" or self.block.num_groups != 6:
            raise ValueError("precompute_rows: the fp16 configuration with six groups only")
        n, _, h, w = x_rows.shape
        if not (0 <= row0 and row0 + n <= live[3].shape[0]):
            raise ValueError(f"precompute_rows: rows [{row0}, {row0 + n}) outside the {live[3].shape[0]} planes of the buffers")
        x = x_rows.detach().float().contiguous()
        P = self._packed()
        cmap = self._const_map(P, h, w, x.device)
        self._utd_cus, self._utd_side = int(getattr(self, "precompute_cus", 256)), True
        try:
            self._forward_f16(x, P, cmap, None, False, {}, precompute={k: live[k][row0:row0 + n] for k in (3, 6)})
        finally:
            self._utd_cus, self._utd_side = 256, False

    def _forward_autograd(self, x: torch.Tensor) -> torch.Tensor:
        import torch.nn.functional as F
        k, st, pd = sr_geometry(self.upscale_factor)
        b = self.block
        nf = self.num_features
        G = b.num_groups
        x = self.sub_mean(x.float())
        inter_res = F.interpolate(x, scale_factor=self.upscale_factor, mode="bilinear", align_corners=False)
        x = self.feat_in(self.conv_in(x))
        last = x
        h = None

        def tran(block, src, idx):
            conv, act = block[0], block[1]
            return act(F.conv2d(src, conv.weight[:, nf * idx:nf * (idx + 1)], conv.bias))

        for _ in range(self.num_steps):
            lr = [b.compress_in(torch.cat((x, last), 1))]
            hr = []
            for idx in range(G):
                if idx == 0:
                    ld_l = torch.zeros_like(lr[0])
                else:
                    ld_l = tran(b.uptranBlocks[idx - 1], lr[idx - 1], idx)
                hr.append(b.upBlocks[idx](ld_l))
                if idx == 0:
                    ld_h = torch.zeros_like(hr[0])
                else:
                    ld_h = tran(b.downtranBlocks[idx - 1], hr[idx - 1], idx)
                lr.append(b.downBlocks[idx](ld_h))
            last = b.compress_out(torch.cat(lr[1:], 1))
            h = self.add_mean(inter_res + self.conv_out(self.out(last)))
        v = self.fc(h.permute(1, 2, 3, 0))
        return v.permute(3, 0, 1, 2)

    @L.on_device
    @torch.no_grad()
    def _forward_kernels(self, x: torch.Tensor, taps: Optional[dict] = None, decimate: bool = False,
                         shared: Optional[dict] = None) -> torch.Tensor:
        if x.dim() != 4 or x.shape[1] != 3:
            raise ValueError(f"expected [planes,3,h,w], got {tuple(x.shape)}")
        N, _, h, w = x.shape
        if N != self.fc[0].in_features:
            raise ValueError(f"the fusion MLP is defined over {self.fc[0].in_features} planes, got {N}")
        lib = L.load()
        x = x.detach().float().contiguous()
        P = self._packed()
        dev = x.device
        G = self.block.num_groups
        cmap = self._const_map(P, h, w, dev)
        if self.precision == "fp16":
            return self._forward_f16(x, P, cmap, taps, decimate, shared)
        if self.precision != "fp32":
            raise ValueError(f"precision must be 'fp16' or 'fp32', got {self.precision!r}")
        S = self.upscale_factor
        n_sh = int(shared.get("n", 0)) if (shared is not None and taps is None) else 0
        skey32 = (self._pack_key, h, w, N, S, n_sh)
        kept = shared.get("prefc_f32") if (n_sh and shared.get("key_f32") == skey32) else None
        reuse = kept is not None and 0 < n_sh < N and tuple(kept.shape) == (n_sh, 3, S * h, S * w) and kept.device == dev
        prefc = torch.empty((N, 3, S * h, S * w), dtype=torch.float32, device=dev)
        if reuse:
            prefc[:n_sh].copy_(kept)
            self._f32_planes(x[n_sh:].contiguous(), P, cmap, None, prefc[n_sh:])
        else:
            self._f32_planes(x, P, cmap, taps, prefc)
            if 0 < n_sh < N:
                shared["prefc_f32"], shared["key_f32"] = prefc[:n_sh].clone(), skey32
        if taps is not None:
            taps[f"prefc{self.num_steps - 1}"] = prefc
        out = torch.empty((1, 3, S * h, S * w), dtype=torch.float32, device=dev)
        L.check(lib.vsr_sr_fc_fuse_f32(L.dptr(prefc), L.dptr(P["fc_w1"]), L.dptr(P["fc_b1"]), L.dptr(P["fc_w2"]),
                                       L.dptr(P["fc_b2"]), N, P["fc_w1"].shape[0], L.dptr(out), S * S * h * w, 0, L.stream()),
                "sr_fc_fuse")
        return out[..., ::S, ::S].contiguous() if decimate else out

    def _f32_planes(self, x, P, cmap, taps, prefc_out):
        lib = L.load()
        N, _, h, w = x.shape
        dev = x.device
        G = self.block.num_groups
        S = self.upscale_factor
        nmid = P["w_in"].shape[0]
        feat = torch.empty((N, _NF, h, w), dtype=torch.float32, device=dev)
        L.check(lib.vsr_sr_head_f32(L.dptr(x), L.dptr(P["sub_s"]), L.dptr(P["sub_b"]), L.dptr(P["w_in"]), L.dptr(P["b_in"]),
                                    L.cf(P["a_in"]), nmid, L.dptr(P["w_feat"]), L.dptr(P["b_feat"]), L.cf(P["a_feat"]),
                                    L.dptr(feat), N, h, w, L.stream()), "sr_head")
        if taps is not None:
            taps["feat_in"] = feat
        hp = h * w
        last = feat
        hid = None
        for step in range(self.num_steps):
            lr0 = self._c1([(feat.view(N, _NF, hp), P["ci_w"], 0), (last.view(N, _NF, hp), P["ci_w"], _NF)], P["ci_b"],
                           P["ci_a"], N, hp)
            live = {0: lr0.view(N, _NF, h, w)}
            j = 0
            while j + 3 <= G:
                fuse = bool(getattr(self, "fuse_dt_f32", True)) and taps is None
                hr = self._hr_from(P, j + 1, live[j], N, h, w, dt_for=j + 2 if fuse else None)
                live[j + 3] = self._lr_from(P, j + 2, hr, N, h, w, dt_done=fuse)
                del hr
                j += 3
            ins = [(live[k].view(N, _NF, hp), P["co_w"], _NF * (k - 1)) for k in sorted(live) if k > 0]
            if not ins:
                raise NotImplementedError("num_groups < 3 leaves compress_out without a live input")
            hid = self._c1(ins, P["co_b"], P["co_a"], N, hp, cmap=cmap)
            last = hid
            if taps is not None:
                taps[f"block{step}"] = hid.view(N, _NF, h, w)
                if step == self.num_steps - 1:
                    for k, v in live.items():
                        taps[f"lr{k}"] = v
        up = self._up(hid.view(N, _NF, h, w), P["out_w"], P["out_b"], P["out_a"], N, h, w)
        if bool(getattr(self, "tail_conv_mfma_f32", True)):
            from . import trunk_f32
            if "cv_wp" not in P:
                P["cv_wp"] = trunk_f32._pack(P["cv_w"].view(3, _NF, 3, 3).contiguous())
            trunk_f32.conv2d_fused(up, P["cv_wp"], None, P["cv_b"], False, 0.0, 3, 3, 3, 1, 1, 1, trunk_f32.SPATIAL_K, out=prefc_out)
            L.check(lib.vsr_sr_tail_scale_f32(L.optr(None), L.optr(None), L.optr(None), L.dptr(x), L.dptr(P["sub_s"]), L.dptr(P["sub_b"]),
                                              L.dptr(P["add_s"]), L.dptr(P["add_b"]), L.dptr(prefc_out), N, h, w, S, L.stream()), "sr_tail_skip")
            return
        L.check(lib.vsr_sr_tail_scale_f32(L.dptr(up), L.dptr(P["cv_w"]), L.dptr(P["cv_b"]), L.dptr(x), L.dptr(P["sub_s"]),
                                          L.dptr(P["sub_b"]), L.dptr(P["add_s"]), L.dptr(P["add_b"]), L.dptr(prefc_out), N, h, w, S,
                                          L.stream()), "sr_tail")

    @staticmethod
    def _c1h(ins, bias, slope, N, P, cmap=None):
        out = torch.empty((N, P, _NF), dtype=torch.float16, device=bias.device)
        args = []
        keep = []
        for k in range(3):
            if k < len(ins):
                t, w, col = ins[k]
                ws = w[:, col:col + _NF]
                keep.append(ws)
                args += [L.dptr(t, torch.float16), ctypes_ptr(ws), w.shape[1]]
            else:
                args += [L.optr(None), L.optr(None), 0]
        L.check(L.load().vsr_sr_conv1x1_f16(*args, L.dptr(bias), L.optr(cmap), L.cf(slope), L.dptr(out, torch.float16), N, P,
                                            L.stream()), "sr_conv1x1_f16")
        return out

    @staticmethod
    def _chain(stages, N, P, keep, outs=None):
        dev = stages[0]["bias"].device
        c = L.Chain1x1()
        c.nstages = len(stages)
        given, outs, hold = outs, [], []
        for s, st in enumerate(stages):
            d = c.stage[s]
            for t, (ten, wm, col) in enumerate(st["ins"]):
                ws = wm[:, col:col + _NF]
                hold.append(ws)
                d.inp[t] = L.dptr(ten, torch.float16).value
                d.w[t] = ctypes_ptr(ws).value
                d.ldw[t] = wm.shape[1]
            if st.get("prev") is not None:
                wm, col = st["prev"]
                ws = wm[:, col:col + _NF]
                hold.append(ws)
                d.w_prev = ctypes_ptr(ws).value
                d.ldw_prev = wm.shape[1]
            d.bias = L.dptr(st["bias"]).value
            if st.get("cmap") is not None:
                d.cmap = L.dptr(st["cmap"]).value
            d.slope = float(st["slope"])
            o = (given[s] if given is not None and given[s] is not None else
                 torch.empty((N, P, _NF), dtype=torch.float16, device=dev)) if keep[s] else None
            d.out = L.dptr(o, torch.float16).value if o is not None else None
            outs.append(o)
        tok = L.TIMER.start(f"sr_chain1x1_f16 x{len(stages)}") if L.TIMER.enabled else None
        L.check(L.load().vsr_sr_chain1x1_f16(ctypes.byref(c), N, P, L.stream()), "sr_chain1x1_f16")
        L.TIMER.stop(tok)
        return outs

    @staticmethod
    def _rows_per_segment(N, h, w, cus=256, strip=None, flat_ok=False):
        strips = -(-w // (strip or L.load().vsr_sr_query(L.Q_UTD_STRIP_WIDTH)))
        wgs = strips * N
        best, best_cost = 1, None
        for segs in range(1, max(1, min(-(-h // 8), 32)) + 1):
            rows = -(-h // segs)
            cost = -(-(wgs * (-(-h // rows))) // cus) * (rows + 6)
            if best_cost is None or cost < best_cost * 0.97:
                best, best_cost = segs, cost
        if flat_ok and wgs * h > cus:
            per = -(-(wgs * h) // cus)
            flat_cost = per + 6 * (2 if per < h else -(-per // h) + 1)
            if flat_cost < best_cost * 0.97:
                return -cus
        return -(-h // best)

    def _utd2(self, a, blob_v2, N, h, w):
        out = torch.empty((N, h, w, _NF), dtype=torch.float16, device=a.device)
        tok = L.TIMER.start("sr_utd2_f16")
        L.check(L.load_xcheck().vsr_sr_utd2_f16(L.dptr(a, torch.float16), L.dptr(blob_v2, torch.uint8), L.dptr(out, torch.float16), N, h, w,
                                         self._rows_per_segment(N, h, w), int(self._pack["slopes_le_one"]), L.stream()),
                "sr_utd2_f16")
        L.TIMER.stop(tok)
        return out

    fold_tail = os.environ.get("VSR_FOLD_TAIL", "1") != "0"
    fused_s2 = True
    fused_s3 = True
    fused_tail_s3 = True

    utd_s2_build = int(os.environ.get("VSR_UTD_S2_BUILD", "1"))
    fuse_uptran = os.environ.get("VSR_UTD_POST", "1") != "0"

    fold_chain = os.environ.get("VSR_FOLD_CHAIN", "0") != "0"
    fold_chain_modes = (2, 3)

    def _utd_timer_name(self, N):
        return ("sr_utd_f16" if N == 8 else f"sr_utd_f16_p{N}") + ("_side" if getattr(self, "_utd_side", False) else "")

    utd_build = int(os.environ.get("VSR_UTD_BUILD", "4"))

    def _utd4(self, a, blob, N, h, w, out=None, post=False, entry="vsr_sr_utd4_f16"):
        if out is None:
            out = torch.empty((N, h, w, _NF), dtype=torch.float16, device=a.device)
        out_post = torch.empty((N, h, w, _NF), dtype=torch.float16, device=a.device) if post else None
        tok = L.TIMER.start(self._utd_timer_name(N))
        L.check(getattr(L.load(), entry)(L.dptr(a, torch.float16), L.dptr(blob, torch.uint8), L.dptr(out, torch.float16), L.optr(out_post, torch.float16),
                                         N, h, w, self._rows_per_segment(N, h, w, cus=getattr(self, "_utd_cus", 256), flat_ok=getattr(self, "utd_flat_split", True)),
                                         int(self._pack["post_slopes_le_one"] if post else self._pack["slopes_le_one"]), L.stream()), entry[4:])
        L.TIMER.stop(tok)
        return (out, out_post) if post else out

    def _utd_post(self, a, blob, N, h, w, out=None):
        return self._utd4(a, blob, N, h, w, out=out, post=True, entry="vsr_sr_utd_post_f16")

    def _utd(self, a, blob, N, h, w, deconv_only=False, out=None):
        if out is None:
            out = torch.empty((N, 4 * h, 4 * w, _NF) if deconv_only else (N, h, w, _NF), dtype=torch.float16, device=a.device)
        tok = L.TIMER.start("sr_utd_f16_deconv" if deconv_only else self._utd_timer_name(N))
        L.check((L.load_xcheck() if deconv_only else L.load()).vsr_sr_utd_f16(L.dptr(a, torch.float16), L.dptr(blob, torch.uint8), L.dptr(out, torch.float16), N, h, w,
                                        self._rows_per_segment(N, h, w, cus=getattr(self, "_utd_cus", 256), flat_ok=not deconv_only and getattr(self, "utd_flat_split", True)),
                                        int(deconv_only), int(self._pack["slopes_le_one"]),
                                        L.stream()), "sr_utd_f16")
        L.TIMER.stop(tok)
        return out

    def _share_plan(self, N_all, h, w, taps, shared, precompute):
        if precompute is not None:
            return (self._pack_key, h, w, precompute[3].shape[0], self.upscale_factor), False, 0, 0, 0
        skey = (self._pack_key, h, w, N_all, self.upscale_factor)
        share_ok = shared is not None and taps is None and self.block.num_groups == 6 and 0 < int(shared.get("n", 0)) < N_all
        n0 = n_sh = m_done = 0
        if share_ok and shared.get("live") is not None and shared.get("key") == skey:
            n0 = n_sh = int(shared["n"])
            m_done = max(0, min(int(shared.get("done_last", 0)), N_all - n0))
            if shared.get("todo") is not None:
                a_, b_ = shared["todo"]
                if not (n0 <= a_ <= b_ <= N_all):
                    raise ValueError(f"shared['todo'] = {shared['todo']} outside the unshared planes [{n0}, {N_all})")
                n0, m_done = int(a_), N_all - int(b_)
        return skey, share_ok, n_sh, n0, m_done

    def _forward_f16(self, x, P, cmap, taps, decimate=False, shared=None, precompute=None):
        N_all, _, h, w = x.shape
        skey, share_ok, n_sh, n0, m_done = self._share_plan(N_all, h, w, taps, shared, precompute)
        N = N_all - n0 - m_done
        if (h, w) not in self._const_nhwc:
            self._const_nhwc[(h, w)] = cmap.t().contiguous()
        cmap_nhwc = self._const_nhwc[(h, w)]
        into = precompute if precompute is not None else shared["live"] if n0 else None
        dst = {k: into[k][n0:n0 + N].view(N, h, w, _NF) for k in (3, 6)} if into is not None else {}
        live = self._steps_f16(x[n0:N_all - m_done] if (n0 or m_done) else x, P, cmap_nhwc, taps, dst)
        if precompute is not None:
            shared.update(live={k: precompute[k] for k in (3, 6)}, key=skey)
            self._tail_ahead(P, precompute, shared, live, N, h, w, cmap_nhwc)
            return None
        if n_sh:
            live = {k: shared["live"][k] for k in (3, 6)}
        elif share_ok:
            shared.pop("prefc_all", None)
            shared.update(live={k: live[k] for k in (3, 6)}, key=skey)
        kept = shared is not None and shared.get("key") == skey and taps is None
        return self._tail_f16(x, live, P, cmap_nhwc, taps, decimate, shared.get("prefc_all") if (n_sh and kept) else None, n_sh)

    def _co(self, P, live, cmap_nhwc):
        return dict(ins=[(live[k], P["co_w"], _NF * (k - 1)) for k in sorted(live) if k > 0], bias=P["co_b"], slope=P["co_a"], cmap=cmap_nhwc)

    def _hid(self, P, live, N, hp, cmap_nhwc):
        co = self._co(P, live, cmap_nhwc)
        return self._chain([co], N, hp, keep=[True])[0] if len(co["ins"]) <= 2 else self._c1h(co["ins"], P["co_b"], P["co_a"], N, hp, cmap=cmap_nhwc)

    def _steps_f16(self, x, P, cmap_nhwc, taps, dst):
        lib = L.load()
        N, _, h, w = x.shape
        dev = x.device
        G = self.block.num_groups
        S = self.upscale_factor
        hp = h * w
        side = getattr(self, "_utd_side", False)
        feat = torch.empty((N, hp, _NF), dtype=torch.float16, device=dev)
        if N:
            x = x.contiguous()
            tok = L.TIMER.start("sr_head_f16") if L.TIMER.enabled else None
            L.check(lib.vsr_sr_head_f16(L.dptr(x), L.dptr(P["sub_s"]), L.dptr(P["sub_b"]), L.dptr(P["w_in"]), L.dptr(P["b_in"]),
                                        L.cf(P["a_in"]), P["w_in"].shape[0], L.dptr(P["w_feat"]), L.dptr(P["b_feat"]),
                                        L.cf(P["a_feat"]), L.dptr(feat, torch.float16), N, h, w, L.stream()), "sr_head_f16")
            L.TIMER.stop(tok)
        nchw = lambda t: t.view(N, h, w, _NF).permute(0, 3, 1, 2).float()
        v4 = lambda t: None if t is None else t.view(N, h, w, _NF)
        if taps is not None:
            taps["feat_in"] = nchw(feat)
        if G < 3:
            raise NotImplementedError("num_groups < 3 leaves compress_out without a live input")
        want_lr0 = taps is not None
        ci = lambda last: dict(ins=[(feat, P["ci_w"], 0), (last, P["ci_w"], _NF)], bias=P["ci_b"], slope=P["ci_a"])
        ut = lambda j, src=None: dict(ins=[] if src is None else [(src, P["ut_w"][j], _NF * (j + 1))],
                                      prev=None if src is not None else (P["ut_w"][j], _NF * (j + 1)), bias=P["ut_b"][j], slope=P["ut_a"][j])
        live = {}
        stage_post, utd_post = P.get("stage_post", ()), P.get("utd_post", ())
        for step in range(self.num_steps if N else 0):
            last_step = step == self.num_steps - 1
            fold = (self.fold_chain and S == 3 and G == 6 and taps is None and not L._use_x and 0 in P.get("stage_pre", {})
                    and (step == 0 or sorted(live) == [3, 6]) and (3 if step > 0 else 2) in self.fold_chain_modes)
            if fold:
                prev = (live[3], live[6], cmap_nhwc) if step > 0 else (None, None, None)
                outs = [None, None]
            elif step > 0 and len(self._co(P, live, cmap_nhwc)["ins"]) > 2:
                hid = self._hid(P, live, N, hp, cmap_nhwc)
                outs = [hid] + self._chain([ci(hid), ut(0)], N, hp, keep=[want_lr0, True])
            elif step > 0:
                ci_chained = dict(ins=[(feat, P["ci_w"], 0)], prev=(P["ci_w"], _NF), bias=P["ci_b"], slope=P["ci_a"])
                outs = self._chain([self._co(P, live, cmap_nhwc), ci_chained, ut(0)], N, hp, keep=[taps is not None, want_lr0, True])
            else:
                outs = self._chain([ci(feat), ut(0)], N, hp, keep=[want_lr0, True])
            if taps is not None and step > 0:
                taps[f"block{step - 1}"] = nchw(outs[0])
            live = {0: outs[-2]} if want_lr0 else {}
            a = outs[-1]
            a_next = None
            for j in range(0, G - 2, 3):
                if j > 0:
                    a = a_next if a_next is not None else self._chain([ut(j, live[j])], N, hp, keep=[True])[0]
                out = dst.get(j + 3) if last_step else None
                build, post = _stage_route(S, j, G, fold, self.fuse_uptran, self.utd_build, L._use_x,
                                           S != 4 and getattr(P["stage"][j], "has_post", False), j in stage_post, j in utd_post)
                if build == "pre":
                    r = P["stage_pre"][0](v4(feat), v4(prev[0]), v4(prev[1]), prev[2], out=out, side=side, post=post)
                elif S == 4:
                    r = getattr(self, "_" + build)(a, P[build][j], N, h, w, out=out, **({"post": True} if build == "utd4" and post else {}))
                else:
                    r = P[build][j](v4(a), self._chain, out=out, side=side, **({"post": True} if post else {}))
                o, a_next = r if post else (r, None)
                live[j + 3], a_next = o.view(N, hp, _NF), (None if a_next is None else a_next.view(N, hp, _NF))
            if taps is not None and last_step:
                for k, v in live.items():
                    taps[f"lr{k}"] = nchw(v)
        return live

    @staticmethod
    def _planes_ahead(pre, nt, N, S, h, w, n_live, dev):
        return nt if (pre is not None and tuple(pre.shape) == (N, 3, S * h, S * w) and pre.device == dev and n_live <= 2) else 0

    @staticmethod
    def _planes_buffer(pre, nt, N, S, ho, wo, decimate, dev):
        if nt and not decimate:
            return pre
        buf = torch.empty((N, 3, ho, wo), dtype=torch.float32, device=dev)
        if nt:
            buf[:nt].copy_(pre[:nt, :, ::S, ::S])
        return buf

    def _fuse_planes(self, raw, x, P, decimate):
        N, _, h, w = x.shape
        S = self.upscale_factor
        lib = L.load()
        out = torch.empty((1,) + tuple(raw.shape[1:]), dtype=torch.float32, device=raw.device)
        what = "sr_fc_planes_skip" if S == 4 else "sr_fc_planes_skip_scale"
        tok = L.TIMER.start(what + ("_dec" if decimate and S == 4 else "")) if L.TIMER.enabled else None
        fn, scale = (lib.vsr_sr_fc_planes_skip_f32, ()) if S == 4 else (lib.vsr_sr_fc_planes_skip_scale_f32, (S,))
        L.check(fn(L.dptr(raw), L.dptr(x), L.dptr(P["tail_par"]), L.dptr(P["fc_w1"]), L.dptr(P["fc_b1"]), L.dptr(P["fc_w2"]), L.dptr(P["fc_b2"]),
                   N, P["fc_w1"].shape[0], L.dptr(out), h, w, *scale, int(decimate), L.stream()), what)
        L.TIMER.stop(tok)
        return out

    def _tail3_fold(self, lr3, lr6, cmap_nhwc, P, prefc, N, h, w, cus, decimate, name):
        tok = L.TIMER.start(name)
        L.check(L.load().vsr_sr_tail3_fold_f16(L.dptr(lr3, torch.float16), L.dptr(lr6, torch.float16), L.dptr(cmap_nhwc),
                                               L.dptr(P["utd_out_fold"], torch.uint8), L.dptr(P["cv_frags3"], torch.float16),
                                               L.dptr(P["tail_par"]), L.dptr(prefc), N, h, w, self._rows_per_segment(N, h, w, cus=cus),
                                               int(P["slopes_le_one"]), int(decimate), L.stream()), "sr_tail3_fold_f16")
        L.TIMER.stop(tok)

    def _tail_ahead(self, P, precompute, shared, live, N, h, w, cmap_nhwc):
        S = self.upscale_factor
        pre = precompute.get("prefc")
        if pre is None or tuple(pre.shape) != (precompute[3].shape[0], 3, S * h, S * w):
            return
        cus = getattr(self, "_utd_cus", 256)
        if S == 4 and self.fold_tail and self.tail_build == 3 and "utd_out_fold" in P:
            self._tail3_fold(precompute[3], precompute[6], cmap_nhwc, P, pre, N, h, w, cus, False, "sr_tail_f16_p%d" % N)
        elif S != 4 and self._tail_key(P) and sum(k > 0 for k in live) <= 2:
            fold = self._fold_tail(P, live, N, h, w, cmap_nhwc)
            hid = fold[0] if fold else self._hid(P, live, N, h * w, cmap_nhwc).view(N, h, w, _NF)
            self._tail_raw(hid, P, False, pre[:N], cus=2 * cus, fold=fold)
        else:
            return
        shared["prefc_all"] = pre

    def _tail_f16(self, x, live, P, cmap_nhwc, taps, decimate, pre, n_sh):
        N, _, h, w = x.shape
        dev = x.device
        hp = h * w
        S = self.upscale_factor
        ho, wo = (h, w) if decimate else (S * h, S * w)
        nchw = lambda t: t.view(N, h, w, _NF).permute(0, 3, 1, 2).float()
        n_live = sum(k > 0 for k in live)
        if S != 4:
            nt = self._planes_ahead(pre, n_sh, N, S, h, w, n_live, dev)
            if nt:
                live = {k: v[nt:] for k, v in live.items()}
            fold = self._fold_tail(P, live, N - nt, h, w, cmap_nhwc) if taps is None else None
            hid = fold[0] if fold else self._hid(P, live, N - nt, hp, cmap_nhwc).view(N - nt, h, w, _NF)
            if taps is not None:
                taps[f"block{self.num_steps - 1}"] = nchw(hid)
            return self._tail_unfused(x, hid, P, decimate, taps, pre=pre, fold=fold)
        if self.fold_tail and taps is None and self.tail_build == 3 and "utd_out_fold" in P and sorted(k for k in live if k > 0) == [3, 6]:
            nt = self._planes_ahead(pre, n_sh, N, S, h, w, n_live, dev)
            prefc = self._planes_buffer(pre, nt, N, S, ho, wo, decimate, dev)
            self._tail3_fold(live[3][nt:], live[6][nt:], cmap_nhwc, P, prefc[nt:], N - nt, h, w, 256, decimate,
                             ("sr_tail_dec_f16" if decimate else "sr_tail_f16") + (f"_p{N - nt}" if nt else ""))
            return self._fuse_planes(prefc, x, P, decimate)
        hid = self._hid(P, live, N, hp, cmap_nhwc)
        if taps is not None:
            taps[f"block{self.num_steps - 1}"] = nchw(hid)
        prefc = torch.empty((N, 3, ho, wo), dtype=torch.float32, device=dev)
        tok = L.TIMER.start("sr_tail_dec_f16" if decimate else "sr_tail_f16")
        if self.tail_build == 3 and taps is None:
            L.check(L.load().vsr_sr_tail3_f16(L.dptr(hid, torch.float16), L.dptr(P["utd_out"], torch.uint8), L.dptr(P["cv_frags3"], torch.float16),
                                              L.dptr(P["tail_par"]), L.dptr(prefc), N, h, w, self._rows_per_segment(N, h, w),
                                              int(P["slopes_le_one"]), int(decimate), L.stream()), "sr_tail3_f16")
            L.TIMER.stop(tok)
            return self._fuse_planes(prefc, x, P, decimate)
        lib = L.load_xcheck()
        out = torch.empty((1, 3, ho, wo), dtype=torch.float32, device=dev)
        tail = lib.vsr_sr_tail_dec_f16 if decimate else lib.vsr_sr_tail_f16
        L.check(tail(L.dptr(hid, torch.float16), L.dptr(P["utd_out"], torch.uint8), L.dptr(P["cv_frags"], torch.float16),
                     L.dptr(P["tail_par"]), L.dptr(x), L.dptr(prefc), N, h, w, self._rows_per_segment(N, h, w),
                     int(P["slopes_le_one"]), L.stream()), "sr_tail_f16")
        L.TIMER.stop(tok)
        L.check(lib.vsr_sr_fc_planes_f32(L.dptr(prefc), L.dptr(P["fc_w1"]), L.dptr(P["fc_b1"]), L.dptr(P["fc_w2"]), L.dptr(P["fc_b2"]),
                                         N, P["fc_w1"].shape[0], L.dptr(out), ho * wo, 0, L.stream()), "sr_fc_planes")
        if taps is not None:
            taps[f"prefc{self.num_steps - 1}"] = prefc
        return out

    def _tail_key(self, P):
        key = {2: "tail_s2", 3: "tail_s3"}.get(self.upscale_factor)
        return key if key in P else None

    def _fold_tail(self, P, live, N, h, w, cmap_nhwc):
        key = self._tail_key(P)
        if not (self.fold_tail and key and P.get(key + "_fold") and sorted(k for k in live if k > 0) == [3, 6]) or L._use_x:
            return None
        return live[3].view(N, h, w, _NF), live[6].view(N, h, w, _NF), cmap_nhwc

    def _tail_raw(self, hid, P, decimate, raw, cus=512, fold=None):
        lib = L.load()
        N, h, w, _ = hid.shape
        S = self.upscale_factor
        key = self._tail_key(P)
        if key:
            own, entry = (L.load_s3t(), "vsr_s3t_sr_tail") if S == 3 else (None, "vsr_sr_tail_s2")
            fn = getattr(own or lib, entry + ("_fold_f16" if fold else "_f16"))
            blob, flags = L.dptr(P[key], torch.uint8), (int(P["slopes_le_one"]), int(decimate), L.stream())
            if fold:
                launch = lambda n0, n, rows: fn(L.dptr(fold[0][n0:n0 + n], torch.float16), L.dptr(fold[1][n0:n0 + n], torch.float16), L.dptr(fold[2]),
                                                blob, L.dptr(raw[n0:n0 + n]), n, h, w, rows, *flags)
            else:
                launch = lambda n0, n, rows: fn(L.dptr(hid[n0:n0 + n], torch.float16), blob, L.dptr(raw[n0:n0 + n]), n, h, w, rows, *flags)
            _launch_chunks(f"sr_tail_s{S}" + ("_dec_f16" if decimate else "_f16"), N, h, w, self._rows_per_segment, cus, 30, launch,
                           f"sr_tail_s{S}" + ("_fold_f16" if fold else "_f16"), lib=own, planes_in_name=False)
            return
        nb = _planes_per_chunk(N, S * h, S * w)
        for n0 in range(0, N, nb):
            hr = P["out_deconv"](hid[n0:n0 + nb])
            tok = L.TIMER.start("sr_convout_planes_f16") if L.TIMER.enabled else None
            L.check(lib.vsr_sr_convout_planes_f16(L.dptr(hr, torch.float16), L.dptr(P["cv_w"]), L.dptr(P["cv_b"]), L.dptr(raw[n0:n0 + nb]),
                                                  hr.shape[0], S * h, S * w, S if decimate else 1, L.stream()), "sr_convout_planes")
            L.TIMER.stop(tok)
            del hr

    def _tail_unfused(self, x, hid, P, decimate, taps, pre=None, fold=None):
        N = x.shape[0]
        Nh, h, w, _ = hid.shape
        nt = N - Nh
        S = self.upscale_factor
        ho, wo = (h, w) if decimate else (S * h, S * w)
        raw = self._planes_buffer(pre, nt, N, S, ho, wo, decimate, hid.device)
        self._tail_raw(hid, P, decimate, raw[nt:], fold=fold)
        return self._fuse_planes(raw, x, P, decimate)

    def _reset_state(self):
        return None


def _stage_route(scale, j, G, fold, fuse_uptran, utd_build, use_x, has_post, in_stage_post, in_utd_post):
    if fold and j == 0:
        return "pre", bool(fuse_uptran)
    plain = "utd" if scale == 4 else "stage"
    if use_x:
        return plain, False
    if scale == 4 and utd_build == 4:
        return "utd4", bool(fuse_uptran and j + 6 <= G)
    if not fuse_uptran:
        return plain, False
    if scale == 4:
        return ("utd_post", True) if in_utd_post else (plain, False)
    if has_post:
        return "stage", True
    return ("stage_post", True) if scale == 3 and in_stage_post else (plain, False)


def _plane_chunks(N, h, w):
    nb = max(1, min(N, ((1 << 32) - 32) // (h * w * _NF * 2)))
    return [(n0, min(nb, N - n0)) for n0 in range(0, N, nb)]


def _launch_chunks(name, N, h, w, rows_fn, cus, strip, launch, what, lib=None, side=False, planes_in_name=True):
    for n0, n in _plane_chunks(N, h, w):
        tok = L.TIMER.start((name if n == 8 or not planes_in_name else f"{name}_p{n}") + ("_side" if side else "")) if L.TIMER.enabled else None
        L.check(launch(n0, n, rows_fn(n, h, w, cus=cus, strip=strip)), what, lib=lib)
        L.TIMER.stop(tok)


def _planes_per_chunk(N, H, W):
    per = H * W * _NF * 2
    if per >= (1 << 31):
        raise L.VsrHipError(f"one {H}x{W}x32 fp16 feature map exceeds 2 GiB")
    return max(1, min(N, ((1 << 31) - 1) // per))


class _PhaseDeconv:

    def __init__(self, weight, bias, slope, S):
        from .igemm import ACT_LEAKY, HConv
        w = weight.detach().float()
        K = w.shape[2]
        T = -(-K // S)
        self.S = S
        self.phases = []
        for ry in range(S):
            for rx in range(S):
                wk = torch.zeros((w.shape[1], w.shape[0], T, T), dtype=torch.float32, device=w.device)
                for a in range(T):
                    ky = (ry + 2) % S + S * (T - 1 - a)
                    for bb in range(T):
                        kx = (rx + 2) % S + S * (T - 1 - bb)
                        if ky < K and kx < K:
                            wk[:, :, a, bb] = w[:, :, ky, kx].t()
                c = HConv(wk, bias, stride=1, pad=0, act=ACT_LEAKY, slope=float(slope))
                c.pad_y, c.pad_x = T - 1 - (ry + 2) // S, T - 1 - (rx + 2) // S
                c.oy, c.ox = (S, ry), (S, rx)
                self.phases.append(c)

    def __call__(self, x):
        N, h, w, _ = x.shape
        out = torch.empty((N, self.S * h, self.S * w, _NF), dtype=torch.float16, device=x.device)
        for c in self.phases:
            c(x, out=out, out_hw=(h, w))
        return out


class _FusedStageS2:

    def __init__(self, up, dt_w, dt_col, dt_b, dt_a, dn, slopes_le_one, rows_fn, wide=True, post=None):
        self.wide = bool(wide)
        self.has_post = post is not None and not self.wide
        self.blob = pack_utd_s2_blob(up[0].weight, up[0].bias, float(up[1].weight.detach()), dt_w, dt_col, dt_b, dt_a,
                                     dn[0].weight, dn[0].bias, float(dn[1].weight.detach()), layout=4 if self.wide else 1,
                                     post=post if self.has_post else None)
        self.slopes_le_one = bool(slopes_le_one)
        self.post_slopes_le_one = self.slopes_le_one and (post is None or float(post[3]) <= 1.0)
        self.rows_fn = rows_fn
        self.strip = int(L.load().vsr_sr_query(L.Q_UTD_S2_STRIP_WIDTH))

    def __call__(self, a, chain, out=None, side=False, post=False):
        N, h, w, _ = a.shape
        if out is None:
            out = torch.empty((N, h, w, _NF), dtype=torch.float16, device=a.device)
        lib = L.load()
        if post:
            assert self.has_post
            out2 = torch.empty((N, h, w, _NF), dtype=torch.float16, device=a.device)
            launch = lambda n0, n, rows: lib.vsr_sr_utd_s2_post_f16(
                L.dptr(a[n0:n0 + n], torch.float16), L.dptr(self.blob, torch.uint8), L.dptr(out[n0:n0 + n], torch.float16),
                L.dptr(out2[n0:n0 + n], torch.float16), n, h, w, rows, int(self.post_slopes_le_one), L.stream())
        else:
            fn = lib.vsr_sr_utd_s2w_f16 if self.wide else lib.vsr_sr_utd_s2_f16
            launch = lambda n0, n, rows: fn(L.dptr(a[n0:n0 + n], torch.float16), L.dptr(self.blob, torch.uint8), L.dptr(out[n0:n0 + n], torch.float16),
                                            n, h, w, rows, int(self.slopes_le_one), L.stream())
        _launch_chunks("sr_utd_s2_f16", N, h, w, self.rows_fn, 256 if self.wide and not post else 512, self.strip, launch,
                       "sr_utd_s2_post_f16" if post else "sr_utd_s2_f16", side=side)
        return (out, out2) if post else out


class _FusedStageS3:

    has_post = False

    def __init__(self, up, dt_w, dt_col, dt_b, dt_a, dn, slopes_le_one, rows_fn):
        self.blob = pack_utd_s3_blob(up[0].weight, up[0].bias, float(up[1].weight.detach()), dt_w, dt_col, dt_b, dt_a,
                                     dn[0].weight, dn[0].bias, float(dn[1].weight.detach()))
        self.slopes_le_one = bool(slopes_le_one)
        self.rows_fn = rows_fn
        self.strip = int(L.load_s3().vsr_s3_query(L.Q_S3_STRIP_WIDTH))

    def __call__(self, a, chain, out=None, side=False, post=False):
        assert not post
        N, h, w, _ = a.shape
        if out is None:
            out = torch.empty((N, h, w, _NF), dtype=torch.float16, device=a.device)
        lib = L.load_s3()
        _launch_chunks("sr_utd_s3_f16", N, h, w, self.rows_fn, 256, self.strip,
                       lambda n0, n, rows: lib.vsr_s3_sr_utd_f16(L.dptr(a[n0:n0 + n], torch.float16), L.dptr(self.blob, torch.uint8),
                                                                 L.dptr(out[n0:n0 + n], torch.float16), n, h, w, rows, int(self.slopes_le_one), L.stream()),
                       "sr_utd_s3_f16", lib=lib, side=side)
        return out


# ... 92 lines not shown
```

### video_super_resolution_amd/sr_pack.py

```python
from __future__ import annotations

import torch

from . import _lib as L

_NF = 32


def _chunk_channel_order(device):
    g = torch.arange(4, device=device).view(4, 1)
    j = torch.arange(8, device=device).view(1, 8)
    return torch.where(j < 4, 4 * g + j, 16 + 4 * g + (j - 4))


def _lane_j(device):
    return torch.arange(64, device=device).view(64, 1), torch.arange(8, device=device).view(1, 8)


def _k16_natural(device):
    lane, j = _lane_j(device)
    return 8 * (lane >> 4) + j


def _k16_acc(device):
    return _chunk_channel_order(device)[torch.arange(64, device=device) >> 4]


def _k32_natural(device):
    lane, e = _lane_j(device)
    return 16 * torch.arange(2, device=device).view(2, 1, 1) + 8 * (lane >> 5) + e


def _k32_acc(device):
    lane, e = _lane_j(device)
    return 16 * torch.arange(2, device=device).view(2, 1, 1) + 8 * (e >> 2) + 4 * (lane >> 5) + (e & 3)


def _rows(k):
    lane = torch.arange(64, device=k.device).view(64, 1)
    return 16 * torch.arange(2, device=k.device).view(2, 1, 1) + (lane & 15) if k.dim() == 2 else lane & 31


def _f32(t):
    return t.detach().float()


def _frags(w, transposed, row, k, ky, kx):
    return (w[k, row, ky, kx] if transposed else w[row, k, ky, kx]).to(torch.float16)


def _frag_1x1(w, col0, order):
    k = order(w.device)
    return _f32(w)[_rows(k), col0 + k].to(torch.float16)


def _param_block(biases, slopes, n, device):
    par = torch.zeros(n, dtype=torch.float32, device=device)
    for i, b in enumerate(biases):
        if b is not None:
            par[32 * i:32 * i + b.numel()] = _f32(b)
    for i, a in enumerate(slopes):
        par[n - 32 + i] = float(a)
    return par.view(torch.uint8)


def _put(blob, off, t, nbytes):
    raw = t.contiguous().view(torch.uint8).reshape(-1)
    assert raw.numel() == nbytes, (raw.numel(), nbytes)
    blob[off:off + nbytes] = raw
    return off + nbytes


def _lead3(device, a, b, c):
    return (torch.arange(a, device=device).view(a, 1, 1, 1, 1, 1), torch.arange(b, device=device).view(b, 1, 1, 1, 1),
            torch.arange(c, device=device).view(c, 1, 1, 1))


def _conv_out_frags9(cv_w):
    dev = cv_w.device
    k = _k16_acc(dev)
    row = torch.arange(64, device=dev) & 15
    live = row < 3
    cv = torch.zeros((3, 3, 64, 8), dtype=torch.float32, device=dev)
    cv[:, :, live] = _f32(cv_w)[row[live].unsqueeze(1), k[live]].permute(2, 3, 0, 1)
    return cv.to(torch.float16)


def _fold_co_section(blob, off, fold_co):
    co_w, cols, co_b, co_a = fold_co
    off = _put(blob, off, torch.stack([_frag_1x1(co_w, c, _k16_natural) for c in cols]), 4096)
    return _put(blob, off, _param_block([co_b], [co_a], 64, blob.device), 256)


def _post_section(blob, off, post, gap=0):
    pw, pcol, pb, pa = post
    off = _put(blob, off, _frag_1x1(pw, pcol, _k16_natural), 2048)
    return _put(blob, off + gap, _param_block([pb], [pa], 64, blob.device), 256)


def pack_dt_frags(dt_w: torch.Tensor, col: int) -> torch.Tensor:
    w = _f32(dt_w[:, col:col + _NF])
    r = torch.arange(16).view(16, 1)
    l = torch.arange(64).view(1, 64)
    ci = 8 * (r // 4) + 4 * (l // 32) + r % 4
    co = (l % 32).expand(16, 64)
    return w[co.to(w.device), ci.to(w.device)].contiguous()


def pack_utd_blob(up_w, up_b, up_a, tr_w, tr_col0, tr_b, tr_a, dn_w, dn_b, dn_a, layout: int = 1, fold_co=None, post=None) -> torch.Tensor:
    dev = up_w.device
    nbytes = int(L.load().vsr_sr_query(L.Q_UTD_BLOB_BYTES))
    if layout == 4:
        k_up, k_acc = _k32_natural(dev), _k32_acc(dev)
    else:
        k_up, k_acc = (_k16_natural if fold_co is None else _k16_acc)(dev), _k16_acc(dev)
    if layout == 1:
        W, C, T = _lead3(dev, 8, 2, 4)
        ky, kx = (W >> 1) + 4 * (T >> 1), 2 * (W & 1) + C + 4 * (T & 1)
    else:
        P, C, T = _lead3(dev, 4, 4, 4)
        ky, kx = P + 4 * (T >> 1), C + 4 * (T & 1)
    blob = torch.zeros(nbytes, dtype=torch.uint8, device=dev)
    off = _put(blob, 0, _frags(_f32(up_w), True, _rows(k_up), k_up, ky, kx), 128 * 1024)
    if dn_w is None:
        off += 128 * 1024 + 2048
        off = _put(blob, off, _param_block([up_b], [up_a], 128, dev), 512)
    else:
        Q, HL, KX = _lead3(dev, 4, 2, 8)
        dn_frag = _frags(_f32(dn_w), False, _rows(k_acc), k_acc, Q + 4 * HL, KX)
        if layout == 1:
            dn_frag = dn_frag.permute(3, 0, 1, 2, 4, 5)
        off = _put(blob, off, dn_frag, 128 * 1024)
        off = _put(blob, off, _frag_1x1(tr_w, tr_col0, _k32_acc if layout == 4 else _k16_acc), 2048)
        off = _put(blob, off, _param_block([up_b, tr_b, dn_b], [up_a, tr_a, dn_a], 128, dev), 512)
    if fold_co is not None:
        _fold_co_section(blob, off, fold_co)
    if post is not None:
        assert fold_co is None
        _post_section(blob, off, post, gap=2048)
    return blob


def pack_conv_out_frags3(weight) -> torch.Tensor:
    dev = weight.device
    w = _f32(weight)
    m = torch.arange(64, device=dev) & 15
    dy, co = m >> 2, m & 3
    live = (dy < 3) & (co < 3)
    ci = _k16_acc(dev)[live]
    frags = torch.zeros((3, 64, 8), dtype=torch.float32, device=dev)
    for dx in range(3):
        frags[dx, live] = w[co[live].unsqueeze(1), ci, dy[live].unsqueeze(1), dx]
    return frags.to(torch.float16).contiguous()


def pack_conv_out_frags(weight) -> torch.Tensor:
    dev = weight.device
    w = _f32(weight)
    m = torch.arange(64, device=dev) & 15
    k = _k16_acc(dev)
    frags = torch.zeros((9, 64, 8), dtype=torch.float32, device=dev)
    for c in range(3):
        sel = m == 4 * c
        ci = k[sel]
        for t in range(9):
            frags[t, sel] = w[c, ci, t // 3, t % 3]
    return frags.to(torch.float16).contiguous()


def _s2_taps(device):
    W, A, B = _lead3(device, 4, 3, 3)
    return (W >> 1) + 2 * A, (W & 1) + 2 * B


def pack_utd_s2_blob(up_w, up_b, up_a, tr_w, tr_col0, tr_b, tr_a, dn_w, dn_b, dn_a, layout: int = 1, post=None) -> torch.Tensor:
    dev = up_w.device
    nbytes = int(L.load().vsr_sr_query(L.Q_UTD_S2_BLOB_BYTES))
    nat, acc = (_k32_natural, _k32_acc) if layout == 4 else (_k16_natural, _k16_acc)
    k_nat, k_acc = nat(dev), acc(dev)
    ky, kx = _s2_taps(dev)
    blob = torch.zeros(nbytes, dtype=torch.uint8, device=dev)
    off = _put(blob, 0, _frags(_f32(up_w), True, _rows(k_nat), k_nat, ky, kx), 72 * 1024)
    off = _put(blob, off, _frags(_f32(dn_w), False, _rows(k_acc), k_acc, ky, kx), 72 * 1024)
    off = _put(blob, off, _frag_1x1(tr_w, tr_col0, acc), 2048)
    off = _put(blob, off, _param_block([up_b, tr_b, dn_b], [up_a, tr_a, dn_a], 128, dev), 512)
    if post is not None:
        _post_section(blob, off, post)
    return blob


def pack_tail_s2_blob(out_w, out_b, out_a, cv_w, cv_b, fold_co=None) -> torch.Tensor:
    dev = out_w.device
    nbytes = int(L.load().vsr_sr_query(L.Q_TAIL_S2_BLOB_BYTES))
    k = _k16_natural(dev)
    blob = torch.zeros(nbytes, dtype=torch.uint8, device=dev)
    off = _put(blob, 0, _frags(_f32(out_w), True, _rows(k), k, *_s2_taps(dev)), 72 * 1024)
    off = _put(blob, off, _conv_out_frags9(cv_w), 9 * 1024)
    off = _put(blob, off, _param_block([out_b, cv_b], [out_a], 128, dev), 512)
    if fold_co is not None:
        _fold_co_section(blob, off, fold_co)
    return blob


_S3_PHASES = (((1, 1), (0, 0)), ((0, 1), (2, 1)), ((1, 0), (1, 2)), ((0, 2), (2, 0), (2, 2)))
_S3_SLOTS = 13
_S3_FRAG_BYTES = 4 * _S3_SLOTS * 2 * 1024


def _s3_taps(x):
    return [x + 2 - 3 * d for d in (1, 0, -1) if 0 <= x + 2 - 3 * d <= 6]


def _s3_slots():
    for wv, phases in enumerate(_S3_PHASES):
        taps = [(ky, kx) for r, c in phases for ky in _s3_taps(r) for kx in _s3_taps(c)]
        assert len(taps) <= _S3_SLOTS
        for t, (ky, kx) in enumerate(taps):
            yield wv, t, ky, kx


def _s3_frags(w, transposed, k):
    w, row = _f32(w), _rows(k)
    out = torch.zeros((4, _S3_SLOTS, 2, 64, 8), dtype=torch.float16, device=w.device)
    for wv, t, ky, kx in _s3_slots():
        out[wv, t] = _frags(w, transposed, row, k, ky, kx)
    return out


def pack_utd_s3_blob(up_w, up_b, up_a, tr_w, tr_col0, tr_b, tr_a, dn_w, dn_b, dn_a, layout: int = 1, post=None) -> torch.Tensor:
    if layout != 1 or post is not None:
        raise NotImplementedError("k_utd_s3 has one fragment layout and no in-launch uptran slice")
    dev = up_w.device
    nbytes = int(L.load_s3().vsr_s3_query(L.Q_S3_BLOB_BYTES))
    assert nbytes == 2 * _S3_FRAG_BYTES + 2048 + 512
    blob = torch.zeros(nbytes, dtype=torch.uint8, device=dev)
    off = _put(blob, 0, _s3_frags(up_w, True, _k16_natural(dev)), _S3_FRAG_BYTES)
    off = _put(blob, off, _s3_frags(dn_w, False, _k16_acc(dev)), _S3_FRAG_BYTES)
    off = _put(blob, off, _frag_1x1(tr_w, tr_col0, _k16_acc), 2048)
    _put(blob, off, _param_block([up_b, tr_b, dn_b], [up_a, tr_a, dn_a], 128, dev), 512)
    return blob


def pack_tail_s3_blob(out_w, out_b, out_a, cv_w, cv_b, fold_co=None) -> torch.Tensor:
    dev = out_w.device
    lib = L.load_s3t()
    nplain = int(lib.vsr_s3t_query(L.Q_S3T_BLOB_BYTES))
    nbytes = nplain if fold_co is None else int(lib.vsr_s3t_query(L.Q_S3T_BLOB_FOLD_BYTES))
    assert nplain == _S3_FRAG_BYTES + 9 * 1024 + 512
    blob = torch.zeros(nbytes, dtype=torch.uint8, device=dev)
    off = _put(blob, 0, _s3_frags(out_w, True, _k16_natural(dev)), _S3_FRAG_BYTES)
    off = _put(blob, off, _conv_out_frags9(cv_w), 9 * 1024)
    off = _put(blob, off, _param_block([out_b, cv_b], [out_a], 128, dev), 512)
    if fold_co is not None:
        off = _fold_co_section(blob, off, fold_co)
        assert off == nbytes
    return blob


def _append_post_s3(stage_blob, post) -> torch.Tensor:
    nbytes = int(L.load_s3p().vsr_s3p_query(L.Q_S3P_BLOB_BYTES))
    blob = torch.zeros(nbytes, dtype=torch.uint8, device=stage_blob.device)
    off = _put(blob, 0, stage_blob, stage_blob.numel())
    off = _post_section(blob, off, post)
    assert off == nbytes
    return blob


def pack_utd_s3_post_blob(up_w, up_b, up_a, tr_w, tr_col0, tr_b, tr_a, dn_w, dn_b, dn_a, post) -> torch.Tensor:
    return _append_post_s3(pack_utd_s3_blob(up_w, up_b, up_a, tr_w, tr_col0, tr_b, tr_a, dn_w, dn_b, dn_a), post)


PRE_SECTION_BYTES = 12 * 1024 + 512


def pack_utd_s3_pre_blob(post_blob, co, ci, ut0) -> torch.Tensor:
    nbytes = int(L.load_s3f().vsr_s3f_query(L.Q_S3F_BLOB_BYTES))
    assert nbytes == post_blob.numel() + PRE_SECTION_BYTES
    co_w, (col_a, col_b), co_b, co_a = co
    ci_w, ci_b, ci_a = ci
    ut_w, ut_col, ut_b, ut_a = ut0
    frags = torch.stack((_frag_1x1(co_w, col_a, _k16_natural), _frag_1x1(co_w, col_b, _k16_natural), _frag_1x1(ci_w, 0, _k16_natural),
                         _frag_1x1(ci_w, _NF, _k16_acc), _frag_1x1(ut_w, ut_col, _k16_acc), _frag_1x1(ci_w, _NF, _k16_natural)))
    blob = torch.zeros(nbytes, dtype=torch.uint8, device=post_blob.device)
    off = _put(blob, 0, post_blob, post_blob.numel())
    off = _put(blob, off, frags, 12 * 1024)
    _put(blob, off, _param_block([co_b, ci_b, ut_b], [co_a, ci_a, ut_a], 128, blob.device), 512)
    return blob
```

Baseline: 44.12.

## Fuse step-0 conv_in and first up-transform 1x1 into SR head kernel for x4

Templates the SR head kernel so that, for x4 upscaling, it also applies the step-0 channel-input 1x1 conv and the first up-transform 1x1 conv while the head features are still in registers, writing both feat and the chained activation. This is meant to remove a separate chain launch and a full re-read of the feature map at low resolution. The new path is on by default for scale 4 when VSR_FOLD_CHAIN is unset. It adds a new side library and packed weight blob, increases LDS use and register pressure in the head kernel, and may change rounding slightly.

```diff
diff --git a/__graft_entry__.py b/__graft_entry__.py
--- a/__graft_entry__.py
+++ b/__graft_entry__.py
@@ -61,6 +61,9 @@
     msssimmissing = [s for s in _lib.declared_symbols(msssim=True) if not hasattr(_lib.load_msssim(), s)]
     if msssimmissing:
         raise RuntimeError(f"libvsr_hip_msssim.so lacks {msssimmissing}")
+    x4fmissing = [s for s in _lib.declared_symbols(x4f=True) if not hasattr(_lib.load_x4f(), s)]
+    if x4fmissing:
+        raise RuntimeError(f"libvsr_hip_x4f.so lacks {x4fmissing}")
 
 
 def smoke() -> None:
diff --git a/include/vsr_hip_x4f.h b/include/vsr_hip_x4f.h
--- /dev/null
+++ b/include/vsr_hip_x4f.h
@@ -0,0 +1,28 @@
+#ifndef VSR_HIP_X4F_H
+#define VSR_HIP_X4F_H
+
+#include <stddef.h>
+
+#include "vsr_hip.h"
+
+#ifdef __cplusplus
+extern "C" {
+#endif
+
+#define VSR_X4F_ABI_VERSION 1
+
+int vsr_x4f_abi_version(void);
+const char* vsr_x4f_last_error(void);
+
+#define VSR_X4F_Q_HEAD_CHAIN_BLOB_BYTES 0
+size_t vsr_x4f_query(int what);
+
+int vsr_x4f_sr_head_chain_f16(const float* x, const float* sub_scale3, const float* sub_bias3, const float* w_in, const float* b_in,
+                              float slope_in, int nmid, const float* w_feat, const float* b_feat, float slope_feat, const void* chain_blob,
+                              void* feat_nhwc, void* a_nhwc, int N, int h, int w, vsr_stream_t stream);
+
+#ifdef __cplusplus
+}
+#endif
+
+#endif
diff --git a/video_super_resolution_amd/_lib.py b/video_super_resolution_amd/_lib.py
--- a/video_super_resolution_amd/_lib.py
+++ b/video_super_resolution_amd/_lib.py
@@ -26,12 +26,12 @@
          "metric": _side("metric", "vsr_metric", 1, False), "opt": _side("opt", "vsr_opt", 1, False), "loss": _side("loss", "vsr_loss", 1, False),
          "resize": _side("resize", "vsr_resize", 1, False), "warp": _side("warp", "vsr_warp", 1, False),
          "scene": _side("scene", "vsr_scene", 1, False), "hgi": _side("hgi", "vsr_hgi", 1, False),
-         "msssim": _side("msssim", "vsr_msssim", 1, False)}
+         "msssim": _side("msssim", "vsr_msssim", 1, False), "x4f": _side("x4f", "vsr_x4f", 1, True)}
 (GLIB_PATH, GHEADER_PATH), (S3LIB_PATH, S3HEADER_PATH), (S3TLIB_PATH, S3THEADER_PATH), (S3PLIB_PATH, S3PHEADER_PATH), \
     (S3FLIB_PATH, S3FHEADER_PATH), (YUVLIB_PATH, YUVHEADER_PATH), (METRICLIB_PATH, METRICHEADER_PATH), (OPTLIB_PATH, OPTHEADER_PATH), \
     (LOSSLIB_PATH, LOSSHEADER_PATH), (RESIZELIB_PATH, RESIZEHEADER_PATH), (WARPLIB_PATH, WARPHEADER_PATH), (SCENELIB_PATH, SCENEHEADER_PATH), \
-    (HGILIB_PATH, HGIHEADER_PATH), (MSSSIMLIB_PATH, MSSSIMHEADER_PATH) = (row[:2] for row in _SIDE.values())
-_gradlib = _s3lib = _s3tlib = _s3plib = _s3flib = _yuvlib = _metriclib = _optlib = _losslib = _resizelib = _warplib = _scenelib = _hgilib = _msssimlib = None
+    (HGILIB_PATH, HGIHEADER_PATH), (MSSSIMLIB_PATH, MSSSIMHEADER_PATH), (X4FLIB_PATH, X4FHEADER_PATH) = (row[:2] for row in _SIDE.values())
+_gradlib = _x4flib = _s3lib = _s3tlib = _s3plib = _s3flib = _yuvlib = _metriclib = _optlib = _losslib = _resizelib = _warplib = _scenelib = _hgilib = _msssimlib = None
 _use_x = os.environ.get("VSR_USE_XCHECK", "0") == "1" or bool(os.environ.get("VSR_TUNING", "").strip())
 
 
@@ -49,10 +49,10 @@
 
 def declared_symbols(xcheck: bool = False, grad: bool = False, s3: bool = False, s3t: bool = False, s3p: bool = False, s3f: bool = False,
                      yuv: bool = False, metric: bool = False, opt: bool = False, loss: bool = False, resize: bool = False,
-                     warp: bool = False, scene: bool = False, hgi: bool = False, msssim: bool = False) -> list:
+                     warp: bool = False, scene: bool = False, hgi: bool = False, msssim: bool = False, x4f: bool = False) -> list:
     side = [name for name, on in (("grad", grad), ("s3", s3), ("s3t", s3t), ("s3p", s3p), ("s3f", s3f), ("yuv", yuv), ("metric", metric),
                                   ("opt", opt), ("loss", loss), ("resize", resize), ("warp", warp), ("scene", scene), ("hgi", hgi),
-                                  ("msssim", msssim)) if on]
+                                  ("msssim", msssim), ("x4f", x4f)) if on]
     with open(_SIDE[side[-1]][1] if side else XHEADER_PATH if xcheck else HEADER_PATH) as f:
         text = re.sub(r"/\*.*?\*/", "", f.read(), flags=re.S)
     return sorted(set(re.findall(r"\b(vsr_[a-z0-9_]+)\s*\(", text)))
@@ -198,6 +198,10 @@
     return lib
 
 
+def load_x4f() -> ctypes.CDLL:
+    return _load_side("x4f")
+
+
 def load() -> ctypes.CDLL:
     global _lib
     if _use_x:
@@ -225,6 +229,7 @@
 Q_S3T_BLOB_BYTES, Q_S3T_BLOB_FOLD_BYTES, Q_S3T_STRIP_WIDTH = range(3)
 Q_S3P_BLOB_BYTES, Q_S3P_STRIP_WIDTH = range(2)
 Q_S3F_BLOB_BYTES, Q_S3F_STRIP_WIDTH = range(2)
+Q_X4F_HEAD_CHAIN_BLOB_BYTES = 0
 
 
 def check(rc: int, what: str = "", lib=None) -> None:
diff --git a/video_super_resolution_amd/csrc/sr_f16.hip b/video_super_resolution_amd/csrc/sr_f16.hip
--- a/video_super_resolution_amd/csrc/sr_f16.hip
+++ b/video_super_resolution_amd/csrc/sr_f16.hip
@@ -1,4 +1,5 @@
 #include "sr_f16_common.h"
+#include "sr_head.h"
 
 namespace {
 
@@ -531,150 +532,6 @@
     }
 }
 
-__global__ void __launch_bounds__(256, 4)
-k_head_h(const float* __restrict__ x, const float* __restrict__ sub_scale, const float* __restrict__ sub_bias,
-         const float* __restrict__ w_in, const float* __restrict__ b_in, float slope_in, int nmid,
-         const float* __restrict__ w_feat, const float* __restrict__ b_feat, float slope_feat, _Float16* __restrict__ out,
-         int N, int h, int w) {
-    const int lane = threadIdx.x & 63;
-    const int l15 = lane & 15, g = lane >> 4;
-    const size_t hw = (size_t)h * w;
-    __shared__ __attribute__((aligned(16))) float bias_in[128];
-    if (threadIdx.x < 128) bias_in[threadIdx.x] = b_in[threadIdx.x];
-    __shared__ __attribute__((aligned(16))) h8 A1s[8][64], A2s[4][2][64];
-    {
-        const int wv = threadIdx.x >> 6;
-#pragma unroll
-        for (int q = 0; q < 2; ++q) {
-            const int mt = 2 * wv + q;
-            h8 a;
-#pragma unroll
-            for (int j = 0; j < 8; ++j) {
-                const int k = 8 * g + j;
-                a[j] = k < 27 ? (_Float16)w_in[(16 * mt + l15) * 27 + k] : (_Float16)0.0f;
-            }
-            A1s[mt][lane] = a;
-        }
-#pragma unroll
-        for (int mt2 = 0; mt2 < 2; ++mt2) {
-            h8 a;
-#pragma unroll
-            for (int j = 0; j < 8; ++j) {
-                const int mid = 32 * wv + (j < 4 ? 4 * g + j : 16 + 4 * g + (j - 4));
-                a[j] = (_Float16)w_feat[(16 * mt2 + l15) * nmid + mid];
-            }
-            A2s[wv][mt2][lane] = a;
-        }
-    }
-    __syncthreads();
-    const h2 a1 = {(_Float16)slope_in, (_Float16)slope_in}, a2 = {(_Float16)slope_feat, (_Float16)slope_feat};
-    const bool max1 = slope_in <= 1.0f, max2 = slope_feat <= 1.0f;
-    constexpr int SROW = 20, SCH = 3 * SROW, SWAVE = 3 * SCH;
-    __shared__ __attribute__((aligned(16))) float stg[4 * SWAVE];
-    __shared__ __attribute__((aligned(16))) unsigned char ost[4 * 1024];
-    const int wvi = threadIdx.x >> 6;
-    float* const my = stg + wvi * SWAVE;
-    int toff[8];
-#pragma unroll
-    for (int j = 0; j < 8; ++j) {
-        const int k = 8 * g + j, kk = k < 27 ? k : 0;
-        toff[j] = (kk / 9) * SCH + ((kk % 9) / 3) * SROW + (kk % 3) + l15;
-    }
-    int ec[3], er[3], ecol[3], eoff[3];
-    float es[3], eb[3];
-#pragma unroll
-    for (int q = 0; q < 3; ++q) {
-        const int e0 = lane + 64 * q, ee = e0 < 162 ? e0 : 0;
-        ec[q] = ee / 54; er[q] = (ee % 54) / 18; ecol[q] = ee % 18;
-        eoff[q] = e0 < 162 ? ec[q] * SCH + er[q] * SROW + ecol[q] : -1;
-        es[q] = sub_scale[ec[q]]; eb[q] = sub_bias[ec[q]];
-    }
-    const unsigned tpr = (unsigned)(w + 15) >> 4;
-    const unsigned ntiles = (unsigned)N * (unsigned)h * tpr;
-    const unsigned wave0 = __builtin_amdgcn_readfirstlane(blockIdx.x * 4 + (threadIdx.x >> 6)), nwaves = gridDim.x * 4;
-    auto fetch = [&](unsigned tile, float (&raw)[3], unsigned& okmask, unsigned& row_out) __attribute__((always_inline)) {
-        const unsigned row = tile / tpr, xt = tile - row * tpr;
-        const unsigned n = row / (unsigned)h;
-        const int y = (int)(row - n * (unsigned)h), x0 = (int)(16 * xt);
-        const float* const img = x + (size_t)n * 3 * hw;
-        unsigned m = 0;
-#pragma unroll
-        for (int q = 0; q < 3; ++q) {
-            const int yy = y - 1 + er[q], xc = x0 - 1 + ecol[q];
-            const bool ok = yy >= 0 && yy < h && xc >= 0 && xc < w;
-            const int yc = yy < 0 ? 0 : (yy >= h ? h - 1 : yy), xl = xc < 0 ? 0 : (xc >= w ? w - 1 : xc);
-            raw[q] = img[(size_t)ec[q] * hw + (size_t)yc * w + xl];
-            m |= ok ? (1u << q) : 0u;
-        }
-        okmask = m;
-        row_out = row;
-    };
-    float cur[3];
-    unsigned curm = 0, cur_row = 0;
-    if (wave0 < ntiles) fetch(wave0, cur, curm, cur_row);
-    for (unsigned tile = wave0; tile < ntiles; tile += nwaves) {
-        float nxr[3];
-        unsigned nxm, nx_row;
-        const unsigned tnext = tile + nwaves < ntiles ? tile + nwaves : tile;
-        fetch(tnext, nxr, nxm, nx_row);
-        const unsigned xt = tile - cur_row * tpr;
-        const int xx = (int)(16 * xt) + l15;
-#pragma unroll
-        for (int q = 0; q < 3; ++q) {
-            const float t = cur[q] * es[q] + eb[q];
-            if (eoff[q] >= 0) my[eoff[q]] = (curm >> q) & 1u ? t : 0.0f;
-        }
-        asm volatile("" ::: "memory");
-        h8 bfrag;
-#pragma unroll
-        for (int j = 0; j < 8; ++j) bfrag[j] = (_Float16)my[toff[j]];
-        asm volatile("" ::: "memory");
-        unsigned loff = lane * 16, boff = g * 16;
-        asm volatile("" : "+v"(loff), "+v"(boff));
-        const unsigned char* const a1p = reinterpret_cast<const unsigned char*>(&A1s[0][0]) + loff;
-        const unsigned char* const a2p = reinterpret_cast<const unsigned char*>(&A2s[0][0][0]) + loff;
-        const unsigned char* const bp = reinterpret_cast<const unsigned char*>(&bias_in[0]) + boff;
-        f4 acc1[8];
-#pragma unroll
-        for (int mt = 0; mt < 8; ++mt)
-            acc1[mt] = mfma16(*reinterpret_cast<const h8*>(a1p + mt * 1024), bfrag, *reinterpret_cast<const f4*>(bp + mt * 64));
-        f4 acc2[2];
-#pragma unroll
-        for (int mt2 = 0; mt2 < 2; ++mt2)
-#pragma unroll
-            for (int r = 0; r < 4; ++r) acc2[mt2][r] = b_feat[16 * mt2 + 4 * g + r];
-#pragma unroll
-        for (int s4 = 0; s4 < 4; ++s4) {
-            const h8 mid = act_pack(acc1[2 * s4], acc1[2 * s4 + 1], a1, max1);
-#pragma unroll
-            for (int mt2 = 0; mt2 < 2; ++mt2) acc2[mt2] = mfma16(*reinterpret_cast<const h8*>(a2p + (2 * s4 + mt2) * 1024), mid, acc2[mt2]);
-        }
-        {
-            typedef float f2v __attribute__((ext_vector_type(2)));
-            typedef _Float16 h4 __attribute__((ext_vector_type(4)));
-            unsigned char* const o = ost + wvi * 1024;
-            const int sw = (l15 >> 1) & 3;
-#pragma unroll
-            for (int mt2 = 0; mt2 < 2; ++mt2) {
-                const h2 p0 = prelu_h2(__builtin_convertvector(f2v{acc2[mt2][0], acc2[mt2][1]}, h2), a2, max2);
-                const h2 p1 = prelu_h2(__builtin_convertvector(f2v{acc2[mt2][2], acc2[mt2][3]}, h2), a2, max2);
-                *reinterpret_cast<h4*>(o + l15 * 64 + (((2 * mt2 + (g >> 1)) ^ sw) << 4) + ((g & 1) << 3)) = h4{p0[0], p0[1], p1[0], p1[1]};
-            }
-            asm volatile("" ::: "memory");
-            const int opx = lane >> 2, opc = (lane & 3) ^ ((opx >> 1) & 3);
-            const h8 ov = *reinterpret_cast<const h8*>(o + lane * 16);
-            asm volatile("" ::: "memory");
-            const int ox = (int)(16 * xt) + opx;
-            if (ox < w) *reinterpret_cast<h8*>(out + ((size_t)cur_row * w + ox) * NF + 8 * opc) = ov;
-        }
-        (void)xx;
-#pragma unroll
-        for (int q = 0; q < 3; ++q) cur[q] = nxr[q];
-        curm = nxm;
-        cur_row = nx_row;
-    }
-}
-
 #if VSR_X
 template <bool ALLMAX>
 __global__ void __launch_bounds__(512, 2)
@@ -1326,13 +1183,10 @@
                     float slope_in, int nmid, const float* w_feat, const float* b_feat, float slope_feat, void* out_nhwc,
                     int N, int h, int w, vsr_stream_t stream) {
     VSR_REQUIRE(x && sub_scale3 && sub_bias3 && w_in && b_in && w_feat && b_feat && out_nhwc, "sr_head_f16: null pointer");
-    VSR_REQUIRE(N > 0 && h > 0 && w > 0, "sr_head_f16: bad shape");
-    if (nmid != 128) return vsr::fail(VSR_E_UNSUPPORTED, "sr_head_f16: %d mid channels (the reference has 4 x 32)", nmid);
-    VSR_REQUIRE((long long)N * h * ((w + 15) / 16) < (1ll << 31), "sr_head_f16: too many pixels");
-    const size_t tiles = (size_t)N * h * ((w + 15) / 16);
-    const unsigned grid = (unsigned)(tiles / 4 + 1 < 2048 ? tiles / 4 + 1 : 2048);
-    hipLaunchKernelGGL(k_head_h, dim3(grid), dim3(256), 0, vsr::S(stream), x, sub_scale3, sub_bias3, w_in, b_in, slope_in,
-                       nmid, w_feat, b_feat, slope_feat, (_Float16*)out_nhwc, N, h, w);
+    unsigned grid = 0;
+    if (int rc = head_grid("sr_head_f16", N, h, w, nmid, grid)) return rc;
+    hipLaunchKernelGGL(k_head_h<false>, dim3(grid), dim3(256), 0, vsr::S(stream), x, sub_scale3, sub_bias3, w_in, b_in, slope_in,
+                       nmid, w_feat, b_feat, slope_feat, (_Float16*)out_nhwc, N, h, w, (const unsigned char*)nullptr, (_Float16*)nullptr);
     return vsr::launched("sr_head_f16");
 }
 
diff --git a/video_super_resolution_amd/csrc/sr_head.h b/video_super_resolution_amd/csrc/sr_head.h
--- /dev/null
+++ b/video_super_resolution_amd/csrc/sr_head.h
@@ -0,0 +1,198 @@
+#pragma once
+#include "sr_f16_common.h"
+
+namespace {
+
+constexpr int HC_FRAG_BYTES = 3 * 2 * 1024;
+constexpr int HC_PAR_BYTES = 96 * 4;
+constexpr int HC_BLOB_BYTES = HC_FRAG_BYTES + HC_PAR_BYTES;
+
+template <bool CHAIN>
+__global__ void __launch_bounds__(256, 4)
+k_head_h(const float* __restrict__ x, const float* __restrict__ sub_scale, const float* __restrict__ sub_bias,
+         const float* __restrict__ w_in, const float* __restrict__ b_in, float slope_in, int nmid,
+         const float* __restrict__ w_feat, const float* __restrict__ b_feat, float slope_feat, _Float16* __restrict__ out,
+         int N, int h, int w, const unsigned char* __restrict__ cblob, _Float16* __restrict__ out_a) {
+    const int lane = threadIdx.x & 63;
+    const int l15 = lane & 15, g = lane >> 4;
+    const size_t hw = (size_t)h * w;
+    __shared__ __attribute__((aligned(16))) float bias_in[128];
+    if (threadIdx.x < 128) bias_in[threadIdx.x] = b_in[threadIdx.x];
+    __shared__ __attribute__((aligned(16))) h8 A1s[8][64], A2s[4][2][64];
+    __shared__ __attribute__((aligned(16))) h8 Acs[CHAIN ? 3 : 1][2][64];
+    __shared__ __attribute__((aligned(16))) float cbs[2][32];
+    {
+        const int wv = threadIdx.x >> 6;
+#pragma unroll
+        for (int q = 0; q < 2; ++q) {
+            const int mt = 2 * wv + q;
+            h8 a;
+#pragma unroll
+            for (int j = 0; j < 8; ++j) {
+                const int k = 8 * g + j;
+                a[j] = k < 27 ? (_Float16)w_in[(16 * mt + l15) * 27 + k] : (_Float16)0.0f;
+            }
+            A1s[mt][lane] = a;
+        }
+#pragma unroll
+        for (int mt2 = 0; mt2 < 2; ++mt2) {
+            h8 a;
+#pragma unroll
+            for (int j = 0; j < 8; ++j) {
+                const int mid = 32 * wv + (j < 4 ? 4 * g + j : 16 + 4 * g + (j - 4));
+                a[j] = (_Float16)w_feat[(16 * mt2 + l15) * nmid + mid];
+            }
+            A2s[wv][mt2][lane] = a;
+        }
+        if (CHAIN) {
+            for (int q = threadIdx.x; q < HC_FRAG_BYTES / 16; q += 256) (&Acs[0][0][0])[q] = reinterpret_cast<const h8*>(cblob)[q];
+            if (threadIdx.x < 64) (&cbs[0][0])[threadIdx.x] = reinterpret_cast<const float*>(cblob + HC_FRAG_BYTES)[threadIdx.x];
+        }
+    }
+    __syncthreads();
+    const h2 a1 = {(_Float16)slope_in, (_Float16)slope_in}, a2 = {(_Float16)slope_feat, (_Float16)slope_feat};
+    const bool max1 = slope_in <= 1.0f, max2 = slope_feat <= 1.0f;
+    const float slope_ci = CHAIN ? reinterpret_cast<const float*>(cblob + HC_FRAG_BYTES)[64] : 1.0f;
+    const float slope_ut = CHAIN ? reinterpret_cast<const float*>(cblob + HC_FRAG_BYTES)[65] : 1.0f;
+    const h2 aci = {(_Float16)slope_ci, (_Float16)slope_ci}, aut = {(_Float16)slope_ut, (_Float16)slope_ut};
+    const bool maxci = slope_ci <= 1.0f, maxut = slope_ut <= 1.0f;
+    constexpr int SROW = 20, SCH = 3 * SROW, SWAVE = 3 * SCH;
+    __shared__ __attribute__((aligned(16))) float stg[4 * SWAVE];
+    __shared__ __attribute__((aligned(16))) unsigned char ost[4 * 1024];
+    const int wvi = threadIdx.x >> 6;
+    float* const my = stg + wvi * SWAVE;
+    int toff[8];
+#pragma unroll
+    for (int j = 0; j < 8; ++j) {
+        const int k = 8 * g + j, kk = k < 27 ? k : 0;
+        toff[j] = (kk / 9) * SCH + ((kk % 9) / 3) * SROW + (kk % 3) + l15;
+    }
+    int ec[3], er[3], ecol[3], eoff[3];
+    float es[3], eb[3];
+#pragma unroll
+    for (int q = 0; q < 3; ++q) {
+        const int e0 = lane + 64 * q, ee = e0 < 162 ? e0 : 0;
+        ec[q] = ee / 54; er[q] = (ee % 54) / 18; ecol[q] = ee % 18;
+        eoff[q] = e0 < 162 ? ec[q] * SCH + er[q] * SROW + ecol[q] : -1;
+        es[q] = sub_scale[ec[q]]; eb[q] = sub_bias[ec[q]];
+    }
+    const unsigned tpr = (unsigned)(w + 15) >> 4;
+    const unsigned ntiles = (unsigned)N * (unsigned)h * tpr;
+    const unsigned wave0 = __builtin_amdgcn_readfirstlane(blockIdx.x * 4 + (threadIdx.x >> 6)), nwaves = gridDim.x * 4;
+    auto fetch = [&](unsigned tile, float (&raw)[3], unsigned& okmask, unsigned& row_out) __attribute__((always_inline)) {
+        const unsigned row = tile / tpr, xt = tile - row * tpr;
+        const unsigned n = row / (unsigned)h;
+        const int y = (int)(row - n * (unsigned)h), x0 = (int)(16 * xt);
+        const float* const img = x + (size_t)n * 3 * hw;
+        unsigned m = 0;
+#pragma unroll
+        for (int q = 0; q < 3; ++q) {
+            const int yy = y - 1 + er[q], xc = x0 - 1 + ecol[q];
+            const bool ok = yy >= 0 && yy < h && xc >= 0 && xc < w;
+            const int yc = yy < 0 ? 0 : (yy >= h ? h - 1 : yy), xl = xc < 0 ? 0 : (xc >= w ? w - 1 : xc);
+            raw[q] = img[(size_t)ec[q] * hw + (size_t)yc * w + xl];
+            m |= ok ? (1u << q) : 0u;
+        }
+        okmask = m;
+        row_out = row;
+    };
+    float cur[3];
+    unsigned curm = 0, cur_row = 0;
+    if (wave0 < ntiles) fetch(wave0, cur, curm, cur_row);
+    for (unsigned tile = wave0; tile < ntiles; tile += nwaves) {
+        float nxr[3];
+        unsigned nxm, nx_row;
+        const unsigned tnext = tile + nwaves < ntiles ? tile + nwaves : tile;
+        fetch(tnext, nxr, nxm, nx_row);
+        const unsigned xt = tile - cur_row * tpr;
+        const int xx = (int)(16 * xt) + l15;
+#pragma unroll
+        for (int q = 0; q < 3; ++q) {
+            const float t = cur[q] * es[q] + eb[q];
+            if (eoff[q] >= 0) my[eoff[q]] = (curm >> q) & 1u ? t : 0.0f;
+        }
+        asm volatile("" ::: "memory");
+        h8 bfrag;
+#pragma unroll
+        for (int j = 0; j < 8; ++j) bfrag[j] = (_Float16)my[toff[j]];
+        asm volatile("" ::: "memory");
+        unsigned loff = lane * 16, boff = g * 16;
+        asm volatile("" : "+v"(loff), "+v"(boff));
+        const unsigned char* const a1p = reinterpret_cast<const unsigned char*>(&A1s[0][0]) + loff;
+        const unsigned char* const a2p = reinterpret_cast<const unsigned char*>(&A2s[0][0][0]) + loff;
+        const unsigned char* const bp = reinterpret_cast<const unsigned char*>(&bias_in[0]) + boff;
+        f4 acc1[8];
+#pragma unroll
+        for (int mt = 0; mt < 8; ++mt)
+            acc1[mt] = mfma16(*reinterpret_cast<const h8*>(a1p + mt * 1024), bfrag, *reinterpret_cast<const f4*>(bp + mt * 64));
+        f4 acc2[2];
+#pragma unroll
+        for (int mt2 = 0; mt2 < 2; ++mt2)
+#pragma unroll
+            for (int r = 0; r < 4; ++r) acc2[mt2][r] = b_feat[16 * mt2 + 4 * g + r];
+#pragma unroll
+        for (int s4 = 0; s4 < 4; ++s4) {
+            const h8 mid = act_pack(acc1[2 * s4], acc1[2 * s4 + 1], a1, max1);
+#pragma unroll
+            for (int mt2 = 0; mt2 < 2; ++mt2) acc2[mt2] = mfma16(*reinterpret_cast<const h8*>(a2p + (2 * s4 + mt2) * 1024), mid, acc2[mt2]);
+        }
+        {
+            typedef float f2v __attribute__((ext_vector_type(2)));
+            typedef _Float16 h4 __attribute__((ext_vector_type(4)));
+            unsigned char* const o = ost + wvi * 1024;
+            const int sw = (l15 >> 1) & 3;
+#pragma unroll
+            for (int mt2 = 0; mt2 < 2; ++mt2) {
+                const h2 p0 = prelu_h2(__builtin_convertvector(f2v{acc2[mt2][0], acc2[mt2][1]}, h2), a2, max2);
+                const h2 p1 = prelu_h2(__builtin_convertvector(f2v{acc2[mt2][2], acc2[mt2][3]}, h2), a2, max2);
+                *reinterpret_cast<h4*>(o + l15 * 64 + (((2 * mt2 + (g >> 1)) ^ sw) << 4) + ((g & 1) << 3)) = h4{p0[0], p0[1], p1[0], p1[1]};
+            }
+            asm volatile("" ::: "memory");
+            const int opx = lane >> 2, opc = (lane & 3) ^ ((opx >> 1) & 3);
+            const h8 ov = *reinterpret_cast<const h8*>(o + lane * 16);
+            asm volatile("" ::: "memory");
+            const int ox = (int)(16 * xt) + opx;
+            if (ox < w) *reinterpret_cast<h8*>(out + ((size_t)cur_row * w + ox) * NF + 8 * opc) = ov;
+            if (CHAIN) {
+                const h8 fb = *reinterpret_cast<const h8*>(o + l15 * 64 + ((g ^ sw) << 4));
+                asm volatile("" ::: "memory");
+                const unsigned char* const acp = reinterpret_cast<const unsigned char*>(&Acs[0][0][0]) + loff;
+                const unsigned char* const cbp = reinterpret_cast<const unsigned char*>(&cbs[0][0]) + boff;
+                f4 acc[2];
+#pragma unroll
+                for (int mt = 0; mt < 2; ++mt) acc[mt] = *reinterpret_cast<const f4*>(cbp + mt * 64);
+#pragma unroll
+                for (int t = 0; t < 2; ++t)
+#pragma unroll
+                    for (int mt = 0; mt < 2; ++mt) acc[mt] = mfma16(*reinterpret_cast<const h8*>(acp + (t * 2 + mt) * 1024), fb, acc[mt]);
+                h8 prev = act_pack(acc[0], acc[1], aci, maxci);
+#pragma unroll
+                for (int mt = 0; mt < 2; ++mt)
+                    acc[mt] = mfma16(*reinterpret_cast<const h8*>(acp + (4 + mt) * 1024), prev, *reinterpret_cast<const f4*>(cbp + 128 + mt * 64));
+                prev = act_pack(acc[0], acc[1], aut, maxut);
+                *reinterpret_cast<h4*>(o + l15 * 64 + (((g >> 1) ^ sw) << 4) + ((g & 1) << 3)) = h4{prev[0], prev[1], prev[2], prev[3]};
+                *reinterpret_cast<h4*>(o + l15 * 64 + (((2 + (g >> 1)) ^ sw) << 4) + ((g & 1) << 3)) = h4{prev[4], prev[5], prev[6], prev[7]};
+                asm volatile("" ::: "memory");
+                const h8 av = *reinterpret_cast<const h8*>(o + lane * 16);
+                asm volatile("" ::: "memory");
+                if (ox < w) *reinterpret_cast<h8*>(out_a + ((size_t)cur_row * w + ox) * NF + 8 * opc) = av;
+            }
+        }
+        (void)xx;
+#pragma unroll
+        for (int q = 0; q < 3; ++q) cur[q] = nxr[q];
+        curm = nxm;
+        cur_row = nx_row;
+    }
+}
+
+inline int head_grid(const char* what, int N, int h, int w, int nmid, unsigned& grid) {
+    VSR_REQUIRE(N > 0 && h > 0 && w > 0, "%s: bad shape", what);
+    if (nmid != 128) return vsr::fail(VSR_E_UNSUPPORTED, "%s: %d mid channels (the reference has 4 x 32)", what, nmid);
+    VSR_REQUIRE((long long)N * h * ((w + 15) / 16) < (1ll << 31), "%s: too many pixels", what);
+    const size_t tiles = (size_t)N * h * ((w + 15) / 16);
+    grid = (unsigned)(tiles / 4 + 1 < 2048 ? tiles / 4 + 1 : 2048);
+    return VSR_OK;
+}
+
+}
diff --git a/video_super_resolution_amd/csrc/sr_head_x4f.hip b/video_super_resolution_amd/csrc/sr_head_x4f.hip
--- /dev/null
+++ b/video_super_resolution_amd/csrc/sr_head_x4f.hip
@@ -0,0 +1,33 @@
+#include "sr_head.h"
+
+#include "../../include/vsr_hip_x4f.h"
+
+extern "C" {
+
+int vsr_x4f_abi_version(void) { return VSR_X4F_ABI_VERSION; }
+const char* vsr_x4f_last_error(void) { return vsr::err_buf(); }
+
+size_t vsr_x4f_query(int what) {
+    switch (what) {
+        case VSR_X4F_Q_HEAD_CHAIN_BLOB_BYTES: return HC_BLOB_BYTES;
+        default: return 0;
+    }
+}
+
+int vsr_x4f_sr_head_chain_f16(const float* x, const float* sub_scale3, const float* sub_bias3, const float* w_in, const float* b_in,
+                              float slope_in, int nmid, const float* w_feat, const float* b_feat, float slope_feat, const void* chain_blob,
+                              void* feat_nhwc, void* a_nhwc, int N, int h, int w, vsr_stream_t stream) {
+    VSR_REQUIRE(x && sub_scale3 && sub_bias3 && w_in && b_in && w_feat && b_feat && chain_blob && feat_nhwc && a_nhwc,
+                "x4f_sr_head_chain: null pointer");
+    unsigned grid = 0;
+    if (int rc = head_grid("x4f_sr_head_chain", N, h, w, nmid, grid)) return rc;
+    VSR_REQUIRE((reinterpret_cast<uintptr_t>(chain_blob) & 15) == 0 && (reinterpret_cast<uintptr_t>(feat_nhwc) & 15) == 0 &&
+                    (reinterpret_cast<uintptr_t>(a_nhwc) & 15) == 0, "x4f_sr_head_chain: blob and outputs must be 16-byte aligned");
+    const size_t bytes = (size_t)N * h * w * NF * 2;
+    VSR_REQUIRE(!ranges_overlap(feat_nhwc, bytes, a_nhwc, bytes), "x4f_sr_head_chain: feat and a must not overlap");
+    hipLaunchKernelGGL(k_head_h<true>, dim3(grid), dim3(256), 0, vsr::S(stream), x, sub_scale3, sub_bias3, w_in, b_in, slope_in, nmid,
+                       w_feat, b_feat, slope_feat, (_Float16*)feat_nhwc, N, h, w, (const unsigned char*)chain_blob, (_Float16*)a_nhwc);
+    return vsr::launched("x4f_sr_head_chain");
+}
+
+}
diff --git a/video_super_resolution_amd/graph.py b/video_super_resolution_amd/graph.py
--- a/video_super_resolution_amd/graph.py
+++ b/video_super_resolution_amd/graph.py
@@ -31,7 +31,7 @@
         weights = (m.model._weights_key(), m._flow_exec.key(), m._depth_exec.key(), m._vos_exec.key())
         return (tuple(data.shape), data.dtype, data.device.index, None if est is None else (tuple(est.shape), est.dtype),
                 m.precision, m.upscale_factor, m.share_planes, m.share_tail, m.overlap_shared, m.early_planes, m.depth_est_late, tuple(m.early_scales),
-                m.model.fuse_uptran, m.model.fold_chain, tuple(m.model.fold_chain_modes), m.model.fold_tail, m.model.utd_build, m.model.tail_build, weights)
+                m.model.fuse_uptran, m.model.fold_chain, tuple(m.model.fold_chain_modes), m.model._fold_modes(), m.model.fold_tail, m.model.utd_build, m.model.tail_build, weights)
 
     def _capture(self, data, est):
         m = self.model
diff --git a/video_super_resolution_amd/sr.py b/video_super_resolution_amd/sr.py
--- a/video_super_resolution_amd/sr.py
+++ b/video_super_resolution_amd/sr.py
@@ -8,8 +8,8 @@
 import torch.nn as nn
 
 from . import _lib as L
-from .sr_pack import (_append_post_s3, pack_conv_out_frags, pack_conv_out_frags3, pack_dt_frags, pack_tail_s2_blob, pack_tail_s3_blob,
-                      pack_utd_blob, pack_utd_s2_blob, pack_utd_s3_blob, pack_utd_s3_pre_blob)
+from .sr_pack import (_append_post_s3, pack_conv_out_frags, pack_conv_out_frags3, pack_dt_frags, pack_head_chain_blob, pack_tail_s2_blob,
+                      pack_tail_s3_blob, pack_utd_blob, pack_utd_s2_blob, pack_utd_s3_blob, pack_utd_s3_pre_blob)
 
 _NF = 32
 
@@ -547,8 +547,23 @@
     utd_s2_build = int(os.environ.get("VSR_UTD_S2_BUILD", "1"))
     fuse_uptran = os.environ.get("VSR_UTD_POST", "1") != "0"
 
-    fold_chain = os.environ.get("VSR_FOLD_CHAIN", "0") != "0"
+    _fold_chain_env = os.environ.get("VSR_FOLD_CHAIN")
+    fold_chain = (_fold_chain_env or "0") != "0"
     fold_chain_modes = (2, 3)
+    fold_chain_x4_default = (2,)
+
+    def _fold_modes(self):
+        if self.fold_chain:
+            return tuple(self.fold_chain_modes)
+        unset = "fold_chain" not in self.__dict__ and self._fold_chain_env is None
+        if unset and self.upscale_factor == 4:
+            return tuple(m for m in self.fold_chain_x4_default if m in self.fold_chain_modes)
+        return ()
+
+    def _head_chain_blob(self, P):
+        if "head_chain" not in P:
+            P["head_chain"] = (pack_head_chain_blob((P["ci_w"], P["ci_b"], P["ci_a"]), (P["ut_w"][0], _NF, P["ut_b"][0], P["ut_a"][0])),)
+        return P["head_chain"][0]
 
     def _utd_timer_name(self, N):
         return ("sr_utd_f16" if N == 8 else f"sr_utd_f16_p{N}") + ("_side" if getattr(self, "_utd_side", False) else "")
@@ -634,12 +649,20 @@
         hp = h * w
         side = getattr(self, "_utd_side", False)
         feat = torch.empty((N, hp, _NF), dtype=torch.float16, device=dev)
+        modes = self._fold_modes()
+        a_head = None
         if N:
             x = x.contiguous()
+            head = (L.dptr(x), L.dptr(P["sub_s"]), L.dptr(P["sub_b"]), L.dptr(P["w_in"]), L.dptr(P["b_in"]), L.cf(P["a_in"]),
+                    P["w_in"].shape[0], L.dptr(P["w_feat"]), L.dptr(P["b_feat"]), L.cf(P["a_feat"]))
             tok = L.TIMER.start("sr_head_f16") if L.TIMER.enabled else None
-            L.check(lib.vsr_sr_head_f16(L.dptr(x), L.dptr(P["sub_s"]), L.dptr(P["sub_b"]), L.dptr(P["w_in"]), L.dptr(P["b_in"]),
-                                        L.cf(P["a_in"]), P["w_in"].shape[0], L.dptr(P["w_feat"]), L.dptr(P["b_feat"]),
-                                        L.cf(P["a_feat"]), L.dptr(feat, torch.float16), N, h, w, L.stream()), "sr_head_f16")
+            if 2 in modes and S == 4 and G == 6 and taps is None and not L._use_x and self.num_steps > 0:
+                a_head = torch.empty((N, hp, _NF), dtype=torch.float16, device=dev)
+                x4f = L.load_x4f()
+                L.check(x4f.vsr_x4f_sr_head_chain_f16(*head, L.dptr(self._head_chain_blob(P), torch.uint8), L.dptr(feat, torch.float16),
+                                                      L.dptr(a_head, torch.float16), N, h, w, L.stream()), "x4f_sr_head_chain", lib=x4f)
+            else:
+                L.check(lib.vsr_sr_head_f16(*head, L.dptr(feat, torch.float16), N, h, w, L.stream()), "sr_head_f16")
             L.TIMER.stop(tok)
         nchw = lambda t: t.view(N, h, w, _NF).permute(0, 3, 1, 2).float()
         v4 = lambda t: None if t is None else t.view(N, h, w, _NF)
@@ -655,11 +678,13 @@
         stage_post, utd_post = P.get("stage_post", ()), P.get("utd_post", ())
         for step in range(self.num_steps if N else 0):
             last_step = step == self.num_steps - 1
-            fold = (self.fold_chain and S == 3 and G == 6 and taps is None and not L._use_x and 0 in P.get("stage_pre", {})
-                    and (step == 0 or sorted(live) == [3, 6]) and (3 if step > 0 else 2) in self.fold_chain_modes)
+            fold = (S == 3 and G == 6 and taps is None and not L._use_x and 0 in P.get("stage_pre", {})
+                    and (step == 0 or sorted(live) == [3, 6]) and (3 if step > 0 else 2) in modes)
             if fold:
                 prev = (live[3], live[6], cmap_nhwc) if step > 0 else (None, None, None)
                 outs = [None, None]
+            elif step == 0 and a_head is not None:
+                outs = [None, a_head]
             elif step > 0 and len(self._co(P, live, cmap_nhwc)["ins"]) > 2:
                 hid = self._hid(P, live, N, hp, cmap_nhwc)
                 outs = [hid] + self._chain([ci(hid), ut(0)], N, hp, keep=[want_lr0, True])
diff --git a/video_super_resolution_amd/sr_pack.py b/video_super_resolution_amd/sr_pack.py
--- a/video_super_resolution_amd/sr_pack.py
+++ b/video_super_resolution_amd/sr_pack.py
@@ -168,6 +168,21 @@
     return frags.to(torch.float16).contiguous()
 
 
+HEAD_CHAIN_BLOB_BYTES = 6 * 1024 + 96 * 4
+
+
+def pack_head_chain_blob(ci, ut0) -> torch.Tensor:
+    nbytes = int(L.load_x4f().vsr_x4f_query(L.Q_X4F_HEAD_CHAIN_BLOB_BYTES))
+    assert nbytes == HEAD_CHAIN_BLOB_BYTES
+    ci_w, ci_b, ci_a = ci
+    ut_w, ut_col, ut_b, ut_a = ut0
+    frags = torch.stack((_frag_1x1(ci_w, 0, _k16_natural), _frag_1x1(ci_w, _NF, _k16_natural), _frag_1x1(ut_w, ut_col, _k16_acc)))
+    blob = torch.zeros(nbytes, dtype=torch.uint8, device=ci_w.device)
+    off = _put(blob, 0, frags, 6 * 1024)
+    _put(blob, off, _param_block([ci_b, ut_b], [ci_a, ut_a], 96, blob.device), 96 * 4)
+    return blob
+
+
 def _s2_taps(device):
     W, A, B = _lead3(device, 4, 3, 3)
     return (W >> 1) + 2 * A, (W & 1) + 2 * B
```

After: 44.35 (median of 6 runs). Within noise of the previous version (+0.5%).
